# nju-ee/MODE-2022

Measured on AMD Instinct MI355X. Metric: ERP stereo pairs/sec (512x1024, 192 disp) fwd+bwd, higher is better.
Workload: dtype fp32 storage/accumulate; products: 2xfp16 split (22-bit, per-tensor 2^k scale, 3 MFMAs) in the stride-1 3x3x3 / spherical / 3x3 layers incl. gradients (DESIGN 3u/3v); 3xbf16 split (24-bit, 6 MFMAs) in the stride-2 / transposed 3x3x3 layers and the polar spherical tiles (3j-3l); fp32 MFMA in the 32->; 1 GPU; ModeDisparity(192,Sphere,1024x512 Cassini) fwd+bwd+Adam step, batch 2/GPU (BASELINE configs[2]); global_batch=2, conv_arith=bf16x6, init=recipe state, seed 1 (tests/golden/recipe.py), parallelism=dp1

## Files before the change

### include/mode_hip.h

```cpp
#ifndef MODE_HIP_H_
#define MODE_HIP_H_

#include <stddef.h>
#include <stdint.h>

#ifdef __cplusplus
extern "C" {
#endif

typedef void* mode_stream_t;

enum {
  MODE_OK = 0,
  MODE_ERR_BAD_ARG = -1,
  MODE_ERR_UNSUPPORTED = -2,
  MODE_ERR_WORKSPACE = -3
};

typedef struct mode_bn_epilogue {
  const float* gamma;
  const float* beta;
  const float* mean;
  const float* var;
  float eps;
// ... 158 lines not shown

int mode_conv1x1_bwd_weight(const float* gy, const float* x, float* gw, float* workspace, int B, int Ci, int H, int W, int Co,
                            int stride, int accumulate, mode_stream_t stream);

size_t mode_conv_stem_wpack_bytes(int Ci, int Co);

int mode_conv_stem_fwd(const float* x, const float* w, float* y, float* wpack, int B, int Ci, int H, int W, int Co, mode_stream_t stream);

int mode_conv_stem_fwd_bn(const float* x, const float* w, const mode_bn_epilogue* bn, float* y, float* wpack, int B, int Ci, int H,
                          int W, int Co, mode_stream_t stream);

size_t mode_conv_stem_bwd_weight_workspace_bytes(int B, int Ci, int H, int W, int Co);

int mode_conv_stem_bwd_weight(const float* gy, const float* x, float* gw, float* workspace, int B, int Ci, int H, int W, int Co,
                              int accumulate, mode_stream_t stream);
size_t mode_conv2d_bwd_weight_workspace_bytes(int B, int Ci, int H, int W, int Co);
int mode_conv2d_bwd_weight(const float* gy, const float* x, float* gw, float* workspace, int B, int Ci, int H, int W, int Co,
                           int dilation, int accumulate, mode_stream_t stream);

size_t mode_conv3d_wpack_bytes(int Ci, int Co);

int mode_conv3d_fwd(const float* x, const float* w, float* y, float* wpack, int B, int Ci, int D, int H, int W, int Co,
                    int stride, mode_stream_t stream);

int mode_conv3d_bwd_data(const float* gy, const float* w, float* gx, float* wpack, int B, int Ci, int D, int H, int W,
                         int Co, int stride, mode_stream_t stream);

int mode_conv3d_fwd_bn(const float* x, const float* w, const mode_bn_epilogue* bn, float* y, float* wpack, int B, int Ci, int D,
                       int H, int W, int Co, int stride, mode_stream_t stream);

int mode_deconv3d_fwd_bn(const float* x, const float* w, const mode_bn_epilogue* bn, float* y, float* wpack, int B, int Cin, int D,
                         int H, int W, int Cout, mode_stream_t stream);

int mode_conv3d_split_supported(int Ci, int Co, int stride, int which );
int mode_conv3d_split_shape_supported(int Ci, int Co, int D, int H, int W, int stride, int which);
int mode_conv3d_fwd_s2_split(const float* x, const float* w, const mode_bn_epilogue* bn ,
                             float* y, float* wpack, int B, int Ci, int D, int H, int W, int Co, mode_stream_t stream);
int mode_conv3d_fwd_s2_split_amax(const float* x, const float* w, const mode_bn_epilogue* bn, float* y, float* out_absmax, float* wpack, int B,
                                  int Ci, int D, int H, int W, int Co, mode_stream_t stream);

int mode_deconv3d_split_supported(int Cin, int Cout);
int mode_deconv3d_fwd_split(const float* x, const float* w, float* y, float* wpack, int B, int Cin, int D, int H, int W, int Cout,
                            mode_stream_t stream);
int mode_abs_max(const float* x, long long n, float* out_device_buffer, mode_stream_t stream);
int mode_abs_max_batch(const float* const* device_ptrs, const long long* device_sizes, int n, float* out, mode_stream_t stream);
int mode_conv3d_fwd_split_f16(const float* x, const float* w, const float* amax_x, const float* amax_w, float* y, float* wpack, int B, int Ci,
                              int D, int H, int W, int Co, mode_stream_t stream);
int mode_conv3d_bwd_data_split_f16(const float* gy, const float* w, const float* amax_g, const float* amax_w, const float* acc, float* gx,
                                   float* wpack, int B, int Ci, int D, int H, int W, int Co, mode_stream_t stream);
int mode_conv3d_fwd_split_f16_bn(const float* x, const float* w, const float* amax_x, const mode_bn_epilogue* bn, float* y, float* amax_y,
                                 float* wpack, int B, int Ci, int D, int H, int W, int Co, mode_stream_t stream);
int mode_conv3d_bwd_weight_split_f16(const float* gy, const float* x, const float* amax_g, const float* amax_x, float* gw, float* workspace,
                                     int B, int Ci, int D, int H, int W, int Co, int accumulate, mode_stream_t stream);
int mode_conv3d_bwd_data_split_acc_supported(int Ci, int Co, int stride);
int mode_conv3d_bwd_data_split_acc(const float* gy, const float* w, const float* acc, float* gx, float* wpack, int B, int Ci, int D, int H,
                                   int W, int Co, int stride, mode_stream_t stream);
int mode_deconv3d_split_bn_supported(int Cin, int Cout);
int mode_deconv3d_fwd_split_bn(const float* x, const float* w, const mode_bn_epilogue* bn, float* y, float* wpack, int B, int Cin, int D,
                               int H, int W, int Cout, mode_stream_t stream);
int mode_deconv3d_fwd_split_bn_amax(const float* x, const float* w, const mode_bn_epilogue* bn, float* y, float* out_absmax ,
                                    float* wpack, int B, int Cin, int D, int H, int W, int Cout, mode_stream_t stream);
int mode_conv3d_bwd_data_s2_split(const float* gy, const float* w, float* gx, float* wpack, int B, int Ci, int D, int H, int W, int Co,
                                  mode_stream_t stream);
int mode_conv3d_bwd_weight_s2_split(const float* gy, const float* x, float* gw, float* workspace, int B, int Ci, int D, int H, int W,
                                    int Co, int accumulate, mode_stream_t stream);

int mode_conv3d_fwd_split(const float* x, const float* w, const mode_bn_epilogue* bn, float* y, float* wpack, int B, int Ci, int D,
                          int H, int W, int Co, mode_stream_t stream);
int mode_conv3d_bwd_data_split(const float* gy, const float* w, float* gx, float* wpack, int B, int Ci, int D, int H, int W, int Co,
                               mode_stream_t stream);
int mode_conv3d_bwd_weight_split(const float* gy, const float* x, float* gw, float* workspace, int B, int Ci, int D, int H, int W,
                                 int Co, int accumulate, mode_stream_t stream);

int mode_conv2d_split_supported(int Ci, int Co, int dilation, int which );
int mode_conv2d_split_shape_supported(int Ci, int Co, int H, int W, int dilation, int which );
int mode_conv2d_fwd_split(const float* x, const float* w, const mode_bn_epilogue* bn, float* y, float* wpack, int B, int Ci, int H, int W,
                          int Co, int dilation, mode_stream_t stream);
int mode_conv2d_bwd_data_split(const float* gy, const float* w, float* gx, float* wpack, int B, int Ci, int H, int W, int Co, int dilation,
                               mode_stream_t stream);
int mode_conv2d_bwd_data_split_acc(const float* gy, const float* w, const float* acc, float* gx, float* wpack, int B, int Ci, int H, int W,
                                   int Co, int dilation, mode_stream_t stream);
int mode_conv2d_fwd_split_f16(const float* x, const float* w, const float* amax_x, const float* amax_w, float* y, float* wpack, int B, int Ci,
                              int H, int W, int Co, int dilation, mode_stream_t stream);
int mode_conv2d_bwd_data_split_f16(const float* gy, const float* w, const float* amax_g, const float* amax_w, const float* acc, float* gx,
                                   float* wpack, int B, int Ci, int H, int W, int Co, int dilation, mode_stream_t stream);
int mode_conv2d_fwd_split_f16_bn(const float* x, const float* w, const float* amax_x, const mode_bn_epilogue* bn, float* y, float* amax_y,
                                 float* wpack, int B, int Ci, int H, int W, int Co, int dilation, mode_stream_t stream);
int mode_conv2d_bwd_weight_split(const float* gy, const float* x, float* gw, float* workspace, int B, int Ci, int H, int W, int Co,
                                 int dilation, int accumulate, mode_stream_t stream);
int mode_conv2d_bwd_weight_split_f16(const float* gy, const float* x, const float* amax_g, const float* amax_x, float* gw, float* workspace,
                                     int B, int Ci, int H, int W, int Co, int dilation, int accumulate, mode_stream_t stream);

size_t mode_conv3d_bwd_weight_workspace_bytes(int B, int Ci, int D, int H, int W, int Co, int stride);

int mode_conv3d_bwd_weight(const float* gy, const float* x, float* gw, float* workspace, int B, int Ci, int D, int H,
                           int W, int Co, int stride, int accumulate, mode_stream_t stream);

int mode_deconv3d_fwd(const float* x, const float* w, float* y, float* wpack, int B, int Cin, int D, int H, int W,
                      int Cout, mode_stream_t stream);

int mode_head_fwd(const float* logits, float* pred, float* conf, int B, int D4, int H4, int W4, int D, int H, int W,
                  mode_stream_t stream);

size_t mode_head_bwd_workspace_bytes(int B, int D4, int H, int W);

int mode_head_bwd(const float* logits, const float* gpred, float* glogits, float* workspace, int B, int D4, int H4,
// ... 203 lines not shown
```

### mode-2022_amd/csrc/bn_act.hip

```cpp
#include "bn_internal.h"
#include <cstdlib>

namespace {

constexpr int NT = 256;
constexpr int NW = NT / 64;

__device__ __forceinline__ float wave_sum(float v) {
#pragma unroll
  for (int off = 32; off > 0; off >>= 1) v += __shfl_down(v, off, 64);
  return v;
}

__device__ __forceinline__ void block_sum2(float& a, float& b, float* sh ) {
  a = wave_sum(a);
  b = wave_sum(b);
  const int wave = threadIdx.x >> 6, lane = threadIdx.x & 63;
  if (lane == 0) {
    sh[wave] = a;
    sh[NW + wave] = b;
  }
  __syncthreads();
  if (threadIdx.x == 0) {
    a = sh[0];
    b = sh[NW];
#pragma unroll
    for (int w = 1; w < NW; ++w) {
      a += sh[w];
      b += sh[NW + w];
    }
  }
}

__global__ __launch_bounds__(NT) void bn_stats_kernel(const float* __restrict__ y, float* __restrict__ partial, int B, int C,
                                                      long long S, int nsplit, unsigned* __restrict__ zero) {
  __shared__ float sh[2 * NW];
  const int c = blockIdx.y, split = blockIdx.x;
  const int Bg = B / gridDim.z, b0 = blockIdx.z * Bg;
  const long long prow = (long long)blockIdx.z * C + c;
  if (zero && blockIdx.x == 0 && blockIdx.y == 0 && blockIdx.z == 0)
    for (int i = threadIdx.x; i < MODE_BN_ABSMAX_FLOATS; i += NT) zero[i] = 0u;
  const long long S4 = (S & 3) ? 0 : (S >> 2);
  const float K = y[((long long)b0 * C + c) * S];
  float s0 = 0.f, s1 = 0.f;
  for (int b = b0; b < b0 + Bg; ++b) {
    const float4* p = reinterpret_cast<const float4*>(y + ((long long)b * C + c) * S);
    auto acc1 = [&](const float4& v) {
      const float dx = v.x - K, dy = v.y - K, dz = v.z - K, dw = v.w - K;
      s0 += (dx + dy) + (dz + dw);
      s1 += (dx * dx + dy * dy) + (dz * dz + dw * dw);
    };
    const long long st = (long long)nsplit * NT;
    long long i = (long long)split * NT + threadIdx.x;
    for (; i + 3 * st < S4; i += 4 * st) {
      const float4 v0 = p[i], v1 = p[i + st], v2 = p[i + 2 * st], v3 = p[i + 3 * st];
      acc1(v0);
      acc1(v1);
      acc1(v2);
      acc1(v3);
    }
    for (; i < S4; i += st) acc1(p[i]);
    {
      const float* q = y + ((long long)b * C + c) * S;
      for (long long i = (S4 << 2) + (long long)split * NT + threadIdx.x; i < S; i += (long long)nsplit * NT) {
        const float dq = q[i] - K;
        s0 += dq;
        s1 += dq * dq;
      }
    }
  }
  block_sum2(s0, s1, sh);
  if (threadIdx.x == 0) {
    partial[(prow * nsplit + split) * 2] = s0;
    partial[(prow * nsplit + split) * 2 + 1] = s1;
  }
}

__device__ __forceinline__ void reduce_partials(const float* __restrict__ partial, int c, int nsplit, double& s0, double& s1,
                                                double* shd ) {
  double a = 0.0, b = 0.0;
  for (int i = threadIdx.x; i < nsplit; i += NT) {
    const float2 v = reinterpret_cast<const float2*>(partial)[(long long)c * nsplit + i];
    a += (double)v.x;
    b += (double)v.y;
  }
#pragma unroll
  for (int off = 32; off > 0; off >>= 1) {
    a += __shfl_down(a, off, 64);
    b += __shfl_down(b, off, 64);
  }
  const int wave = threadIdx.x >> 6, lane = threadIdx.x & 63;
  if (lane == 0) {
    shd[wave] = a;
    shd[NW + wave] = b;
  }
  __syncthreads();
  s0 = shd[0];
  s1 = shd[NW];
#pragma unroll
  for (int w = 1; w < NW; ++w) {
    s0 += shd[w];
    s1 += shd[NW + w];
  }
  __syncthreads();
}

struct BnCoefArgs {
  const float* partial;
  const float* gamma;
  const float* beta;
  float* running_mean;
  float* running_var;
  long long* num_batches_tracked;
  float* save_mean;
  float* save_invstd;
  float* save_scale;
  float* save_shift;
  float momentum, eps;
  int nsplit;
  double count;
  int groups;
  int Bg;
  const float* pivot;
  unsigned* amax;
};

template <bool RELU, bool ADD, bool TRAIN, bool AMAX = false>
// ... 344 lines not shown
                                      float* save_mean, float* save_invstd, float* save_scale, float* save_shift, float* workspace, int B,
                                      int C, long long S, int groups, float* out_absmax, mode_stream_t stream) {
  return bn_train_fwd_impl(y, add, gamma, beta, running_mean, running_var, num_batches_tracked, momentum, eps, relu, out, save_mean,
                           save_invstd, save_scale, save_shift, workspace, B, C, S, groups, 0, out_absmax, stream);
}

static int check_nsplit(int nsplit) {
  MODE_REQUIRE(nsplit > 0 && nsplit <= 1023, MODE_ERR_BAD_ARG, "mode_bn_train_fwd_prestats: %d partial pairs per channel (1..1023)", nsplit);
  return MODE_OK;
}

extern "C" int mode_bn_train_fwd_prestats(const float* y, const float* add, const float* gamma, const float* beta, float* running_mean,
                                          float* running_var, long long* num_batches_tracked, float momentum, float eps, int relu,
                                          float* out, float* save_mean, float* save_invstd, float* save_scale, float* save_shift,
                                          float* workspace, int nsplit, int B, int C, long long S, mode_stream_t stream) {
  int rc = check_nsplit(nsplit);
  if (rc != MODE_OK) return rc;
  return bn_train_fwd_impl(y, add, gamma, beta, running_mean, running_var, num_batches_tracked, momentum, eps, relu, out, save_mean,
                           save_invstd, save_scale, save_shift, workspace, B, C, S, 1, nsplit, nullptr, stream);
}

extern "C" int mode_bn_train_fwd_prestats_amax(const float* y, const float* add, const float* gamma, const float* beta, float* running_mean,
                                               float* running_var, long long* num_batches_tracked, float momentum, float eps, int relu,
                                               float* out, float* save_mean, float* save_invstd, float* save_scale, float* save_shift,
                                               float* workspace, int nsplit, int B, int C, long long S, float* out_absmax,
                                               mode_stream_t stream) {
  int rc = check_nsplit(nsplit);
  if (rc != MODE_OK) return rc;
  return bn_train_fwd_impl(y, add, gamma, beta, running_mean, running_var, num_batches_tracked, momentum, eps, relu, out, save_mean,
                           save_invstd, save_scale, save_shift, workspace, B, C, S, 1, nsplit, out_absmax, stream);
}

static int bn_train_fwd_impl(const float* y, const float* add, const float* gamma, const float* beta, float* running_mean,
                             float* running_var, long long* num_batches_tracked, float momentum, float eps, int relu, float* out,
                             float* save_mean, float* save_invstd, float* save_scale, float* save_shift, float* workspace, int B,
                             int C, long long S, int groups, int prestats, float* amax, mode_stream_t stream) {
  int rc = check_bn(B, C, S, "mode_bn_train_fwd");
  if (rc != MODE_OK) return rc;
  MODE_REQUIRE(B > 0, MODE_ERR_BAD_ARG, "mode_bn_train_fwd: empty batch has no statistics");
  MODE_REQUIRE(y && gamma && beta && out && save_mean && save_invstd && workspace, MODE_ERR_BAD_ARG, "mode_bn_train_fwd: null pointer");
  MODE_REQUIRE(aligned_rows(y, S) && aligned_rows(out, S) && (!add || aligned_rows(add, S)) && aligned16(workspace), MODE_ERR_UNSUPPORTED,
               "mode_bn_train_fwd: unaligned buffer");
  MODE_REQUIRE((running_mean == nullptr) == (running_var == nullptr), MODE_ERR_BAD_ARG, "mode_bn_train_fwd: running stats must come in pairs");
  MODE_REQUIRE((save_scale == nullptr) == (save_shift == nullptr), MODE_ERR_BAD_ARG, "mode_bn_train_fwd: save_scale / save_shift come in pairs");
  MODE_REQUIRE(groups >= 1 && B % groups == 0, MODE_ERR_BAD_ARG, "mode_bn_train_fwd: batch %d not divisible into %d groups", B, groups);
  MODE_REQUIRE(out != y, MODE_ERR_BAD_ARG, "mode_bn_train_fwd: in-place operation (out == y) is not supported");
  hipStream_t st = mode::as_stream(stream);
  if (amax && prestats > 0) {
    rc = mode::absmax_begin(amax, st, "mode_bn_train_fwd");
    if (rc != MODE_OK) return rc;
  }
  const int nsplit = prestats > 0 ? prestats : pick_nsplit(C * groups, S);
  if (prestats <= 0)
    hipLaunchKernelGGL(bn_stats_kernel, dim3(nsplit, C, groups), dim3(NT), 0, st, y, workspace, B, C, S, nsplit, reinterpret_cast<unsigned*>(amax));
  BnCoefArgs k{workspace, gamma, beta, running_mean, running_var, num_batches_tracked, save_mean, save_invstd, save_scale, save_shift,
               momentum, eps, nsplit,
               (double)(B / groups) * (double)S, groups, B / groups, prestats > 0 ? workspace + 2LL * C * nsplit : nullptr,
               reinterpret_cast<unsigned*>(amax)};
  const int BC = B * C;
  const char* who = "mode_bn_train_fwd";
  if (amax) {
    if (relu)
      rc = add ? launch_apply(bn_apply_kernel<true, true, true, true>, BC, S, st, who, y, add, k, out, C, S)
               : launch_apply(bn_apply_kernel<true, false, true, true>, BC, S, st, who, y, y, k, out, C, S);
    else
      rc = add ? launch_apply(bn_apply_kernel<false, true, true, true>, BC, S, st, who, y, add, k, out, C, S)
               : launch_apply(bn_apply_kernel<false, false, true, true>, BC, S, st, who, y, y, k, out, C, S);
    return rc;
  }
  if (relu) {
    if (add) return launch_apply(bn_apply_kernel<true, true, true>, BC, S, st, who, y, add, k, out, C, S);
    return launch_apply(bn_apply_kernel<true, false, true>, BC, S, st, who, y, y, k, out, C, S);
  }
  if (add) return launch_apply(bn_apply_kernel<false, true, true>, BC, S, st, who, y, add, k, out, C, S);
  return launch_apply(bn_apply_kernel<false, false, true>, BC, S, st, who, y, y, k, out, C, S);
}

namespace {
__global__ __launch_bounds__(NT) void bn_finalize_kernel(const float* __restrict__ y, BnCoefArgs k, int C, long long S) {
  __shared__ double shd[2 * NW];
  const int c = blockIdx.x;
  double s0, s1;
  reduce_partials(k.partial, c, k.nsplit, s0, s1, shd);
  if (threadIdx.x != 0) return;
  const double dm = s0 / k.count;
  const double mean = (double)y[(long long)c * S] + dm;
  double var = s1 / k.count - dm * dm;
  if (var < 0.0) var = 0.0;
  const double invstd = 1.0 / sqrt(var + (double)k.eps);
  const double sc = (double)k.gamma[c] * invstd;
  k.save_mean[c] = (float)mean;
  k.save_invstd[c] = (float)invstd;
  k.save_scale[c] = (float)sc;
  k.save_shift[c] = (float)((double)k.beta[c] - mean * sc);
  if (k.running_mean) {
    const double unbiased = k.count > 1.0 ? var * k.count / (k.count - 1.0) : var;
    k.running_mean[c] = (float)((1.0 - k.momentum) * (double)k.running_mean[c] + k.momentum * mean);
    k.running_var[c] = (float)((1.0 - k.momentum) * (double)k.running_var[c] + k.momentum * unbiased);
  }
  if (c == 0 && k.num_batches_tracked) *k.num_batches_tracked += 1;
}
}

int mode::bn_train_coefficients(const float* y, const float* gamma, const float* beta, float* running_mean, float* running_var,
                                long long* num_batches_tracked, float momentum, float eps, float* save_mean, float* save_invstd,
                                float* save_scale, float* save_shift, float* workspace, int B, int C, long long S, hipStream_t st,
                                const char* who) {
  int rc = ::check_bn(B, C, S, who);
  if (rc != MODE_OK) return rc;
  MODE_REQUIRE(B > 0, MODE_ERR_BAD_ARG, "%s: empty batch has no statistics", who);
  MODE_REQUIRE(y && gamma && beta && save_mean && save_invstd && save_scale && save_shift && workspace, MODE_ERR_BAD_ARG, "%s: null pointer", who);
  MODE_REQUIRE(aligned_rows(y, S) && aligned16(workspace), MODE_ERR_UNSUPPORTED, "%s: unaligned buffer", who);
  MODE_REQUIRE((running_mean == nullptr) == (running_var == nullptr), MODE_ERR_BAD_ARG, "%s: running stats must come in pairs", who);
  const int nsplit = pick_nsplit(C, S);
  hipLaunchKernelGGL(bn_stats_kernel, dim3(nsplit, C, 1), dim3(NT), 0, st, y, workspace, B, C, S, nsplit, (unsigned*)nullptr);
  BnCoefArgs k{workspace, gamma, beta, running_mean, running_var, num_batches_tracked, save_mean, save_invstd, save_scale, save_shift,
               momentum, eps, nsplit, (double)B * (double)S, 1, B, nullptr};
  hipLaunchKernelGGL(bn_finalize_kernel, dim3(C), dim3(NT), 0, st, y, k, C, S);
  return mode::check_launch(who);
}

extern "C" int mode_bn_eval_fwd(const float* y, const float* add, const float* gamma, const float* beta, const float* running_mean,
                                const float* running_var, float eps, int relu, float* out, int B, int C, long long S,
                                mode_stream_t stream) {
  int rc = check_bn(B, C, S, "mode_bn_eval_fwd");
  if (rc != MODE_OK) return rc;
  if (B == 0) return MODE_OK;
  MODE_REQUIRE(y && gamma && beta && running_mean && running_var && out, MODE_ERR_BAD_ARG, "mode_bn_eval_fwd: null pointer");
  MODE_REQUIRE(aligned_rows(y, S) && aligned_rows(out, S) && (!add || aligned_rows(add, S)), MODE_ERR_UNSUPPORTED, "mode_bn_eval_fwd: unaligned buffer");
  hipStream_t st = mode::as_stream(stream);
  BnCoefArgs k{nullptr, gamma, beta, const_cast<float*>(running_mean), const_cast<float*>(running_var), nullptr, nullptr, nullptr, nullptr,
               nullptr, 0.f,
               eps, 0, 0.0, 1, 1, nullptr};
  const int BC = B * C;
  const char* who = "mode_bn_eval_fwd";
  if (relu) {
    if (add) return launch_apply(bn_apply_kernel<true, true, false>, BC, S, st, who, y, add, k, out, C, S);
    return launch_apply(bn_apply_kernel<true, false, false>, BC, S, st, who, y, y, k, out, C, S);
  }
  if (add) return launch_apply(bn_apply_kernel<false, true, false>, BC, S, st, who, y, add, k, out, C, S);
  return launch_apply(bn_apply_kernel<false, false, false>, BC, S, st, who, y, y, k, out, C, S);
}

extern "C" int mode_bn_train_bwd(const float* gout, const float* y, const float* out, const float* gamma, const float* save_mean,
                                 const float* save_invstd, const float* save_scale, const float* save_shift, int relu, float* gy,
                                 float* gadd, float* ggamma, float* gbeta, int accumulate, float* workspace, int B, int C, long long S,
                                 int groups, mode_stream_t stream) {
  return mode_bn_train_bwd_amax(gout, y, out, gamma, save_mean, save_invstd, save_scale, save_shift, relu, gy, gadd, ggamma, gbeta,
                                accumulate, workspace, B, C, S, groups, nullptr, stream);
}

extern "C" int mode_bn_train_bwd_amax(const float* gout, const float* y, const float* out, const float* gamma, const float* save_mean,
                                      const float* save_invstd, const float* save_scale, const float* save_shift, int relu, float* gy,
                                      float* gadd, float* ggamma, float* gbeta, int accumulate, float* workspace, int B, int C,
                                      long long S, int groups, float* gy_absmax, mode_stream_t stream) {
  float* amax = gy_absmax;
  int rc = check_bn(B, C, S, "mode_bn_train_bwd");
  if (rc != MODE_OK) return rc;
  MODE_REQUIRE(B > 0, MODE_ERR_BAD_ARG, "mode_bn_train_bwd: empty batch");
  MODE_REQUIRE(gout && y && gamma && save_mean && save_invstd && gy && ggamma && gbeta && workspace, MODE_ERR_BAD_ARG,
               "mode_bn_train_bwd: null pointer");
  MODE_REQUIRE((save_scale == nullptr) == (save_shift == nullptr), MODE_ERR_BAD_ARG, "mode_bn_train_bwd: save_scale / save_shift come in pairs");
  MODE_REQUIRE(!relu || out || save_scale, MODE_ERR_BAD_ARG,
               "mode_bn_train_bwd: the ReLU mask needs the forward output, or (no residual add) the forward's scale / shift");
  MODE_REQUIRE(aligned_rows(gout, S) && aligned_rows(y, S) && aligned_rows(gy, S) && (!out || aligned_rows(out, S)) &&
                   (!gadd || aligned_rows(gadd, S)) && aligned16(workspace),
               MODE_ERR_UNSUPPORTED, "mode_bn_train_bwd: unaligned buffer");
  MODE_REQUIRE(groups >= 1 && B % groups == 0, MODE_ERR_BAD_ARG, "mode_bn_train_bwd: batch %d not divisible into %d groups", B, groups);
  if (gadd) {
    const long long n = (long long)B * C * S;
    auto overlaps = [&](const float* p) { return p && p < gadd + n && gadd < p + n; };
// ... 79 lines not shown
```

### mode-2022_amd/csrc/conv3d.hip

```cpp
#include "common.h"
#include <cstdlib>

#include "conv3d_internal.h"
#include "bn_internal.h"

namespace {

typedef float f32x16 __attribute__((ext_vector_type(16)));

constexpr int NT = 256;
constexpr int CCH = 8;

struct CDims {
  int B, Ci, Co, D, H, W;
  int Do, Ho, Wo;
  int nWt, nHt, nDt;
  int MT, NCHUNK;
  int ntiles;
};

__device__ __forceinline__ f32x16 mfma32(float a, float b, f32x16 c) {
  return __builtin_amdgcn_mfma_f32_32x32x2f32(a, b, c, 0, 0, 0);
}

// ... 554 lines not shown
extern "C" int mode_conv3d_fwd_split_stats_partials(void) { return mode::conv3d_split_stat_partials(); }

extern "C" int mode_conv3d_fwd_split_stats(const float* x, const float* w, float* y, float* wpack, float* stats, int B, int Ci, int D, int H,
                                           int W, int Co, mode_stream_t stream) {
  const char* who = "mode_conv3d_fwd_split_stats";
  int rc = check_split_args(x, w, y, wpack, B, Ci, D, H, W, Co, 1, 0, who);
  if (rc != MODE_OK) return rc;
  MODE_REQUIRE(stats, MODE_ERR_WORKSPACE, "%s: statistics workspace required", who);
  MODE_REQUIRE(B > 0, MODE_ERR_BAD_ARG, "%s: empty batch has no statistics", who);
  return mode::conv3d_s1_split(x, w, y, wpack, B, Ci, Co, D, H, W, 0, mode::as_stream(stream), who, nullptr, stats);
}

extern "C" int mode_conv3d_fwd_s2_split_amax(const float* x, const float* w, const mode_bn_epilogue* bn, float* y, float* out_absmax, float* wpack,
                                             int B, int Ci, int D, int H, int W, int Co, mode_stream_t stream) {
  const char* who = "mode_conv3d_fwd_s2_split";
  int rc = check_split_args(x, w, y, wpack, B, Ci, D, H, W, Co, 2, 0, who);
  if (rc == MODE_OK && bn) rc = mode::check_bn(bn, who);
  if (rc != MODE_OK) return rc;
  MODE_REQUIRE(!out_absmax || bn, MODE_ERR_BAD_ARG, "%s: the output maximum comes out of the eval epilogue (bn is NULL)", who);
  if (B == 0) return out_absmax ? mode::absmax_begin(out_absmax, mode::as_stream(stream), who) : MODE_OK;
  return mode::conv3d_s2_split(x, w, y, wpack, B, Ci, Co, D, H, W, mode::as_stream(stream), who, bn, out_absmax);
}

extern "C" int mode_conv3d_fwd_s2_split(const float* x, const float* w, const mode_bn_epilogue* bn, float* y, float* wpack, int B, int Ci,
                                        int D, int H, int W, int Co, mode_stream_t stream) {
  return mode_conv3d_fwd_s2_split_amax(x, w, bn, y, nullptr, wpack, B, Ci, D, H, W, Co, stream);
}

extern "C" int mode_conv3d_bwd_data_s2_split(const float* gy, const float* w, float* gx, float* wpack, int B, int Ci, int D, int H, int W,
                                             int Co, mode_stream_t stream) {
  const char* who = "mode_conv3d_bwd_data_s2_split";
  int rc = check_split_args(gy, w, gx, wpack, B, Ci, D, H, W, Co, 2, 1, who);
  if (rc != MODE_OK || B == 0) return rc;
  return mode::deconv3d_split(gy, w, gx, wpack, B, Co, Ci, D / 2, H / 2, W / 2, mode::as_stream(stream), who);
}

extern "C" int mode_abs_max(const float* x, long long n, float* out, mode_stream_t stream) {
  return mode::abs_max(x, n, out, mode::as_stream(stream), "mode_abs_max");
}

extern "C" int mode_abs_max_batch(const float* const* device_ptrs, const long long* device_sizes, int n, float* out, mode_stream_t stream) {
  return mode::abs_max_batch(device_ptrs, device_sizes, n, out, mode::as_stream(stream), "mode_abs_max_batch");
}

extern "C" int mode_conv3d_fwd_split_f16(const float* x, const float* w, const float* amax_x, const float* amax_w, float* y, float* wpack, int B,
                                         int Ci, int D, int H, int W, int Co, mode_stream_t stream) {
  const char* who = "mode_conv3d_fwd_split_f16";
  int rc = check_split_args(x, w, y, wpack, B, Ci, D, H, W, Co, 1, 0, who);
  if (rc != MODE_OK || B == 0) return rc;
  MODE_REQUIRE(amax_x && amax_w, MODE_ERR_BAD_ARG, "%s: null operand maximum", who);
  return mode::conv3d_s1_split(x, w, y, wpack, B, Ci, Co, D, H, W, 0, mode::as_stream(stream), who, nullptr, nullptr, nullptr, amax_x, amax_w);
}

extern "C" int mode_conv3d_fwd_split_f16_bn(const float* x, const float* w, const float* amax_x, const mode_bn_epilogue* bn, float* y,
                                            float* amax_y, float* wpack, int B, int Ci, int D, int H, int W, int Co, mode_stream_t stream) {
  const char* who = "mode_conv3d_fwd_split_f16_bn";
  int rc = check_split_args(x, w, y, wpack, B, Ci, D, H, W, Co, 1, 0, who);
  if (rc == MODE_OK) {
    MODE_REQUIRE(bn, MODE_ERR_BAD_ARG, "%s: null BatchNorm epilogue", who);
    rc = mode::check_bn(bn, who);
  }
  if (rc != MODE_OK) return rc;
  MODE_REQUIRE(amax_x && amax_y, MODE_ERR_BAD_ARG, "%s: null maximum buffer", who);
  if (B == 0) return mode::absmax_begin(amax_y, mode::as_stream(stream), who);
  return mode::conv3d_s1_split(x, w, y, wpack, B, Ci, Co, D, H, W, 0, mode::as_stream(stream), who, bn, nullptr, nullptr, amax_x, nullptr, amax_y);
}

extern "C" int mode_conv3d_bwd_data_split_f16(const float* gy, const float* w, const float* amax_g, const float* amax_w, const float* acc, float* gx,
                                              float* wpack, int B, int Ci, int D, int H, int W, int Co, mode_stream_t stream) {
  const char* who = "mode_conv3d_bwd_data_split_f16";
  int rc = check_split_args(gy, w, gx, wpack, B, Ci, D, H, W, Co, 1, 1, who);
  if (rc != MODE_OK || B == 0) return rc;
  MODE_REQUIRE(amax_g && amax_w && acc != gx, MODE_ERR_BAD_ARG, "%s: null operand maximum, or acc is the output tensor", who);
  return mode::conv3d_s1_split(gy, w, gx, wpack, B, Co, Ci, D, H, W, 1, mode::as_stream(stream), who, nullptr, nullptr, acc, amax_g, amax_w);
}

extern "C" int mode_conv3d_bwd_data_split_acc_supported(int Ci, int Co, int stride) {
  if (Ci <= 0 || Co <= 0) return 0;
  if (stride == 1) return mode::conv3d_split_supported(Co, Ci) ? 1 : 0;
  return (stride == 2 && mode::deconv3d_split_bn_supported(Co, Ci)) ? 1 : 0;
}

extern "C" int mode_conv3d_bwd_data_split_acc(const float* gy, const float* w, const float* acc, float* gx, float* wpack, int B, int Ci, int D,
                                              int H, int W, int Co, int stride, mode_stream_t stream) {
  const char* who = "mode_conv3d_bwd_data_split_acc";
  MODE_REQUIRE(stride == 1 || stride == 2, MODE_ERR_UNSUPPORTED, "%s: stride %d not implemented", who, stride);
  int rc = check_split_args(gy, w, gx, wpack, B, Ci, D, H, W, Co, stride, 1, who);
  if (rc != MODE_OK || B == 0) return rc;
  MODE_REQUIRE(acc && acc != gx, MODE_ERR_BAD_ARG, "%s: acc must be a tensor of gx's shape that is not gx", who);
  if (stride == 1) return mode::conv3d_s1_split(gy, w, gx, wpack, B, Co, Ci, D, H, W, 1, mode::as_stream(stream), who, nullptr, nullptr, acc);
  return mode::deconv3d_split(gy, w, gx, wpack, B, Co, Ci, D / 2, H / 2, W / 2, mode::as_stream(stream), who, nullptr, acc);
}

extern "C" int mode_deconv3d_split_supported(int Cin, int Cout) { return mode::deconv3d_split_supported(Cin, Cout) ? 1 : 0; }

extern "C" int mode_deconv3d_fwd_split(const float* x, const float* w, float* y, float* wpack, int B, int Cin, int D, int H, int W, int Cout,
                                       mode_stream_t stream) {
  const char* who = "mode_deconv3d_fwd_split";
  int rc = check_deconv_split_args(x, w, y, wpack, B, Cin, D, H, W, Cout, who);
  if (rc != MODE_OK || B == 0) return rc;
  return mode::deconv3d_split(x, w, y, wpack, B, Cin, Cout, D, H, W, mode::as_stream(stream), who);
}

extern "C" int mode_deconv3d_split_bn_supported(int Cin, int Cout) { return mode::deconv3d_split_bn_supported(Cin, Cout) ? 1 : 0; }

extern "C" int mode_deconv3d_fwd_split_bn_amax(const float* x, const float* w, const mode_bn_epilogue* bn, float* y, float* out_absmax,
// ... 586 lines not shown
  if (B == 0) {
    if (!accumulate) return mode::zero_floats(gw, (size_t)Co * Ci * 27, st, "mode_conv3d_bwd_weight");
    return MODE_OK;
  }
  if (Co == 1 && stride == 1)
    return mode::conv3d_co1_bwd_weight(gy, x, gw, workspace, B, Ci, D, H, W, accumulate, st, "mode_conv3d_bwd_weight");
  WDims d;
  make_wdims(d, B, Ci, D, H, W, Co, stride);
  if (stride == 1) {
    const size_t lds = WGeom<1, WTH1>::LDS;
    if ((long long)std::max(Ci, Co) * D * H * W < (1ll << 29)) {
      rc = mode::allow_lds(conv3d_bwd_weight_ring_kernel, lds, "mode_conv3d_bwd_weight");
      if (rc != MODE_OK) return rc;
      int ring_dc = D;
      while (ring_dc > 6 && (long long)B * d.nHt * d.nWt * mode::cdiv(D, ring_dc) < 2ll * d.S) ring_dc = mode::cdiv(ring_dc, 2);
      static const char* dc_env = getenv("MODE_RING_DC");
      if (dc_env && atoi(dc_env) > 0) ring_dc = atoi(dc_env);
      const int nDc = mode::cdiv(D, ring_dc);
      const int units = B * d.nHt * d.nWt * nDc;
      if (d.S > units) d.S = units;
      hipLaunchKernelGGL(conv3d_bwd_weight_ring_kernel, dim3(d.S, d.MTo, d.MTc), dim3(NT), lds, st, gy, x, workspace, d, nDc, units,
                         ring_dc);
    } else {
      rc = mode::allow_lds(conv3d_bwd_weight_kernel<1, WTH1>, lds, "mode_conv3d_bwd_weight");
      if (rc != MODE_OK) return rc;
      hipLaunchKernelGGL((conv3d_bwd_weight_kernel<1, WTH1>), dim3(d.S, d.MTo, d.MTc), dim3(NT), lds, st, gy, x, workspace, d);
    }
  } else {
    const size_t lds = WGeom<2, WTH2>::LDS;
    if (std::max((long long)Ci * D * H * W, (long long)Co * d.Do * d.Ho * d.Wo) < (1ll << 29)) {
      if (d.MTo >= 2) {
        const size_t lds2 = lds + (size_t)32 * WGeom<2, WTH2>::GPLANE * sizeof(float);
        rc = mode::allow_lds(conv3d_bwd_weight_s2_kernel<2>, lds2, "mode_conv3d_bwd_weight");
        if (rc != MODE_OK) return rc;
        hipLaunchKernelGGL(conv3d_bwd_weight_s2_kernel<2>, dim3(d.S, mode::cdiv(d.MTo, 2), d.MTc), dim3(2 * NT), lds2, st, gy, x, workspace, d);
      } else {
        rc = mode::allow_lds(conv3d_bwd_weight_s2_kernel<1>, lds, "mode_conv3d_bwd_weight");
        if (rc != MODE_OK) return rc;
        hipLaunchKernelGGL(conv3d_bwd_weight_s2_kernel<1>, dim3(d.S, d.MTo, d.MTc), dim3(NT), lds, st, gy, x, workspace, d);
      }
    } else {
      rc = mode::allow_lds(conv3d_bwd_weight_kernel<2, WTH2>, lds, "mode_conv3d_bwd_weight");
      if (rc != MODE_OK) return rc;
      hipLaunchKernelGGL((conv3d_bwd_weight_kernel<2, WTH2>), dim3(d.S, d.MTo, d.MTc), dim3(NT), lds, st, gy, x, workspace, d);
    }
  }
  rc = mode::check_launch("mode_conv3d_bwd_weight");
  if (rc != MODE_OK) return rc;
  hipLaunchKernelGGL(reduce_gw3d, dim3(mode::cdiv((long long)d.MTo * d.MTc * 27 * 1024, 32)), dim3(256), 0, st, workspace, gw, d, accumulate);
  return mode::check_launch("mode_conv3d_bwd_weight(reduce)");
}

static int bwd_weight_split(const float* gy, const float* x, const float* amax_g, const float* amax_x, float* gw, float* workspace, int B, int Ci,
                            int D, int H, int W, int Co, int accumulate, mode_stream_t stream, const char* who);

extern "C" int mode_conv3d_bwd_weight_split(const float* gy, const float* x, float* gw, float* workspace, int B, int Ci, int D, int H,
                                            int W, int Co, int accumulate, mode_stream_t stream) {
  return bwd_weight_split(gy, x, nullptr, nullptr, gw, workspace, B, Ci, D, H, W, Co, accumulate, stream, "mode_conv3d_bwd_weight_split");
}

extern "C" int mode_conv3d_bwd_weight_split_f16(const float* gy, const float* x, const float* amax_g, const float* amax_x, float* gw, float* workspace,
                                                int B, int Ci, int D, int H, int W, int Co, int accumulate, mode_stream_t stream) {
  MODE_REQUIRE(amax_g && amax_x, MODE_ERR_BAD_ARG, "mode_conv3d_bwd_weight_split_f16: null operand maximum");
  return bwd_weight_split(gy, x, amax_g, amax_x, gw, workspace, B, Ci, D, H, W, Co, accumulate, stream, "mode_conv3d_bwd_weight_split_f16");
}

static int bwd_weight_split(const float* gy, const float* x, const float* amax_g, const float* amax_x, float* gw, float* workspace, int B, int Ci,
                            int D, int H, int W, int Co, int accumulate, mode_stream_t stream, const char* who) {
  int rc = check_split_args(gy, x, gw, workspace, B, Ci, D, H, W, Co, 1, 2, who);
  if (rc != MODE_OK) return rc;
  hipStream_t st = mode::as_stream(stream);
  if (B == 0) {
    if (!accumulate) return mode::zero_floats(gw, (size_t)Co * Ci * 27, st, "mode_conv3d_bwd_weight");
    return MODE_OK;
  }
  WDims d;
  make_wdims(d, B, Ci, D, H, W, Co, 1);
  mode::WgradSplitDims q;
  q.Ci = Ci; q.Co = Co; q.D = D; q.H = H; q.W = W;
  q.nWt = d.nWt; q.nHt = d.nHt; q.MTo = d.MTo; q.MTc = d.MTc;
  int S = mode::cdiv(kNumCU, d.MTo * d.MTc);
  int ring_dc = D;
  while (ring_dc > 6 && (long long)B * d.nHt * d.nWt * mode::cdiv(D, ring_dc) < 2ll * S) ring_dc = mode::cdiv(ring_dc, 2);
  q.ring_dc = ring_dc;
  q.nDc = mode::cdiv(D, ring_dc);
  q.units = B * d.nHt * d.nWt * q.nDc;
  if (S > q.units) S = q.units;
  q.S = d.S = S;
  rc = mode::conv3d_bww_split_launch(gy, x, workspace, q, st, who, amax_g, amax_x);
  if (rc != MODE_OK) return rc;
  hipLaunchKernelGGL(reduce_gw3d, dim3(mode::cdiv((long long)d.MTo * d.MTc * 27 * 1024, 32)), dim3(256), 0, st, workspace, gw, d, accumulate);
  return mode::check_launch("mode_conv3d_bwd_weight_split(reduce)");
}

extern "C" int mode_conv3d_bwd_weight_s2_split(const float* gy, const float* x, float* gw, float* workspace, int B, int Ci, int D, int H,
                                               int W, int Co, int accumulate, mode_stream_t stream) {
  const char* who = "mode_conv3d_bwd_weight_s2_split";
  int rc = check_split_args(gy, x, gw, workspace, B, Ci, D, H, W, Co, 2, 2, who);
  if (rc != MODE_OK) return rc;
  hipStream_t st = mode::as_stream(stream);
  if (B == 0) {
    if (!accumulate) return mode::zero_floats(gw, (size_t)Co * Ci * 27, st, "mode_conv3d_bwd_weight");
    return MODE_OK;
  }
  WDims d;
  make_wdims(d, B, Ci, D, H, W, Co, 2);
  mode::WgradS2SplitDims q;
  q.Ci = Ci; q.Co = Co; q.D = D; q.H = H; q.W = W; q.Do = d.Do; q.Ho = d.Ho; q.Wo = d.Wo;
  q.nWt = mode::cdiv(d.Wo, 16); q.MTo = d.MTo; q.MTc = d.MTc;
  int S = std::max(1, kNumCU / (mode::cdiv(d.MTo, 2) * d.MTc));
  int ring_dc = d.Do;
  while (ring_dc > 3 && (long long)B * d.Ho * q.nWt * mode::cdiv(d.Do, ring_dc) < 2ll * S) ring_dc = mode::cdiv(ring_dc, 2);
  q.ring_dc = ring_dc;
  q.nDc = mode::cdiv(d.Do, ring_dc);
  q.units = B * d.Ho * q.nWt * q.nDc;
  q.S = std::min(std::min(S, q.units), d.S);
  d.S = q.S;
  rc = mode::conv3d_bww_s2_split_launch(gy, x, workspace, q, st, who);
  if (rc != MODE_OK) return rc;
  hipLaunchKernelGGL(reduce_gw3d, dim3(mode::cdiv((long long)d.MTo * d.MTc * 27 * 1024, 32)), dim3(256), 0, st, workspace, gw, d, accumulate);
  return mode::check_launch("mode_conv3d_bwd_weight_s2_split(reduce)");
}

extern "C" int mode_deconv3d_fwd(const float* x, const float* w, float* y, float* wpack, int B, int Cin, int D, int H, int W,
                                 int Cout, mode_stream_t stream) {
  int rc = check_conv_args(x, w, y, wpack, B, Cin, D, H, W, Cout, 1, "mode_deconv3d_fwd");
  if (rc != MODE_OK || B == 0) return rc;
  MODE_REQUIRE((long long)Cout * D * H * W * 8 < (1ll << 31), MODE_ERR_UNSUPPORTED, "mode_deconv3d_fwd: output sample too large");
  return deconv3d(x, w, y, wpack, B, Cin, Cout, D, H, W, mode::as_stream(stream), "mode_deconv3d_fwd");
}

extern "C" int mode_deconv3d_fwd_bn(const float* x, const float* w, const mode_bn_epilogue* bn, float* y, float* wpack, int B, int Cin,
                                    int D, int H, int W, int Cout, mode_stream_t stream) {
  const char* who = "mode_deconv3d_fwd_bn";
  int rc = check_conv_args(x, w, y, wpack, B, Cin, D, H, W, Cout, 1, who);
  if (rc == MODE_OK) rc = mode::check_bn(bn, who);
  if (rc != MODE_OK || B == 0) return rc;
  MODE_REQUIRE((long long)Cout * D * H * W * 8 < (1ll << 31), MODE_ERR_UNSUPPORTED, "%s: output sample too large", who);
  return deconv3d(x, w, y, wpack, B, Cin, Cout, D, H, W, mode::as_stream(stream), who, bn);
}
```

### mode-2022_amd/csrc/conv3d_internal.h

```cpp
#pragma once
#include "common.h"
#include "size_contracts.h"

namespace mode {

int conv3d_co1_fwd(const float* x, const float* w, float* y, int B, int Ci, int D, int H, int W, hipStream_t st, const char* who);

int conv3d_co1_fwd_small(const float* x, const float* w, float* y, int B, int Ci, int D, int H, int W, hipStream_t st, const char* who);

int conv3d_co1_bwd_data(const float* gy, const float* w, float* gx, int B, int Ci, int D, int H, int W, hipStream_t st, const char* who);

size_t conv3d_co1_bwd_weight_workspace_floats(int B, int Ci, int D, int H, int W);
int conv3d_co1_bwd_weight(const float* gy, const float* x, float* gw, float* workspace, int B, int Ci, int D, int H, int W,
                          int accumulate, hipStream_t st, const char* who);

bool conv3d_split_supported(int K, int rows);
size_t conv3d_split_wpack_floats(int K, int rows);
int conv3d_split_stat_partials();
int conv3d_s1_split(const float* x, const float* w, float* y, float* wpack, int B, int K, int rows, int D, int H, int W, int flip,
                    hipStream_t st, const char* who, const mode_bn_epilogue* bn, float* stats = nullptr, const float* acc_in = nullptr,
                    const float* amax_x = nullptr, const float* amax_w = nullptr, float* amax_y = nullptr);

int abs_max(const float* x, long long n, float* out, hipStream_t st, const char* who);
int abs_max_batch(const float* const* ptrs, const long long* sizes, int n, float* out, hipStream_t st, const char* who);

bool conv3d_s2_split_supported(int K, int rows);
size_t conv3d_s2_split_wpack_floats(int K, int rows);
int conv3d_s2_split(const float* x, const float* w, float* y, float* wpack, int B, int K, int rows, int D, int H, int W, hipStream_t st,
                    const char* who, const mode_bn_epilogue* bn = nullptr, float* amax_y = nullptr);

bool deconv3d_split_supported(int K, int Co);
bool deconv3d_split_bn_supported(int K, int Co);
size_t deconv3d_split_wpack_floats(int K, int Co);
int deconv3d_split(const float* x, const float* w, float* y, float* wpack, int B, int K, int Co, int D, int H, int W, hipStream_t st,
                   const char* who, const mode_bn_epilogue* bn = nullptr, const float* acc_in = nullptr, float* amax_y = nullptr);

struct WgradSplitDims {
  int Ci, Co, D, H, W;
  int nWt, nHt, nDc, ring_dc, units;
  int S, MTo, MTc;
};
int conv3d_bww_split_launch(const float* gy, const float* x, float* part, const WgradSplitDims& d, hipStream_t st, const char* who,
                            const float* amax_g = nullptr, const float* amax_x = nullptr);

struct WgradS2SplitDims {
  int Ci, Co, D, H, W, Do, Ho, Wo;
  int nWt, nDc, ring_dc, units;
  int S, MTo, MTc;
};
int conv3d_bww_s2_split_launch(const float* gy, const float* x, float* part, const WgradS2SplitDims& d, hipStream_t st, const char* who);

bool conv2d_split_supported(int K, int rows, int dilation);
size_t conv2d_split_wpack_floats(int K, int rows);
int conv2d_split_run(const float* x, const float* w, float* y, float* wpack, int B, int K, int rows, int H, int W, int dilation, int flip,
                     hipStream_t st, const char* who, const mode_bn_epilogue* bn, const float* acc_in = nullptr,
                     const float* amax_x = nullptr, const float* amax_w = nullptr, float* amax_y = nullptr);

struct Wgrad2SplitDims {
  int Ci, Co, H, W;
  int nWt, nGroups, run_groups, nRun, units;
  int S, MTo, MTc;
};
int conv2d_bww_split_launch(const float* gy, const float* x, float* part, const Wgrad2SplitDims& d, int dilation, hipStream_t st,
                            const char* who, const float* amax_g = nullptr, const float* amax_x = nullptr);

}
```

### mode-2022_amd/csrc/conv3d_split.hip

```cpp
#include "common.h"

#include "bn_internal.h"
#include "conv3d_internal.h"
#include "split_arith.h"

namespace {

using namespace mode::split;

#ifndef MODE_SPLIT_NT
#define MODE_SPLIT_NT 256
#endif
constexpr int NT = MODE_SPLIT_NT;
constexpr int TD = 2, ID = TD + 2, IW = 34;
template <int TH_>
struct Geo {
  static constexpr int TH = TH_, IH = TH_ + 2;
  static constexpr int ROWS = ID * IH;
  static constexpr int ITEMS = ROWS * IW;
  static constexpr int KIT = (ITEMS + NT - 1) / NT;
  static constexpr int PIECE = KIT * NT;
  static constexpr int R = TD * TH_ / (NT / 64);
  static constexpr int RB = R / 4;
};
// ... 30 lines not shown
  if (fold && blockIdx.x == 0) {
    float* shifts = reinterpret_cast<float*>(wp + total * NP);
    for (int o = threadIdx.x; o < rows; o += blockDim.x) shifts[o] = fold == 1 ? fold_shift(bn, o) : 0.f;
  }
  for (long long idx = (long long)blockIdx.x * blockDim.x + threadIdx.x; idx < total; idx += (long long)gridDim.x * blockDim.x) {
    const int lane = (int)(idx & 63);
    long long r = idx >> 6;
    const int pair = (int)(r % NPAIR);
    r /= NPAIR;
    const int ch = (int)(r % NCHUNK);
    const int m = (int)(r / NCHUNK);
    const int o = m * 32 + (lane & 31);
    const int tap = 2 * pair + (lane >> 5);
    float v[8];
#pragma unroll
    for (int j = 0; j < 8; ++j) {
      const int c = ch * 8 + j;
      v[j] = 0.f;
      if (o < rows && c < K && tap < 27)
        v[j] = flip == 0 ? w[((long long)o * K + c) * 27 + tap] : w[((long long)c * rows + o) * 27 + (26 - tap)];
      if (fold == 1 && o < rows) v[j] *= fold_scale(bn, o);
      if (F16) v[j] *= sw;
    }
    uint32_t q1[4], q2[4], q3[4];
#pragma unroll
    for (int j = 0; j < 4; ++j) split2<F16>(v[2 * j], v[2 * j + 1], q1[j], q2[j], q3[j]);
    uint4* dst = wp + (idx - lane) * NP + lane;
    dst[0] = make_uint4(q1[0], q1[1], q1[2], q1[3]);
    dst[64] = make_uint4(q2[0], q2[1], q2[2], q2[3]);
    if (NP == 3) dst[128] = make_uint4(q3[0], q3[1], q3[2], q3[3]);
  }
}

__host__ __device__ constexpr int tap_off(int tap, int IH) {
  return (tap / 9) * (IH * IW) + ((tap / 3) % 3) * IW + tap % 3;
}

__global__ __launch_bounds__(64) void first_voxel_kernel(const float* __restrict__ x, const float* __restrict__ w, float* __restrict__ pivot,
                                                         int K, int Co, int D, int H, int W) {
  const int o = blockIdx.x, lane = threadIdx.x;
  const long long HW = (long long)H * W, DHW = (long long)D * HW;
  float acc = 0.f;
  for (int item = lane; item < K * 8; item += 64) {
    const int c = item >> 3, t = item & 7;
    const int kd = 1 + (t >> 2), kh = 1 + ((t >> 1) & 1), kw = 1 + (t & 1);
    if (kd - 1 < D && kh - 1 < H && kw - 1 < W)
      acc = __builtin_fmaf(w[((long long)o * K + c) * 27 + kd * 9 + kh * 3 + kw], x[c * DHW + (kd - 1) * HW + (kh - 1) * W + (kw - 1)], acc);
  }
#pragma unroll
  for (int off = 32; off > 0; off >>= 1) acc += __shfl_xor(acc, off, 64);
  if (lane == 0) pivot[o] = acc;
}

template <int MT, int EPI, bool F16 = false, int TH_ = 8, bool AMAX = false>
__global__ __launch_bounds__(NT) void conv3d_split_kernel(const float* __restrict__ x, const uint4* __restrict__ wp,
                                                          float* __restrict__ y, SDims d, Epi epi, float* __restrict__ stats,
                                                          const float* __restrict__ stat_pivot, const float* __restrict__ amax_x,
                                                          const float* __restrict__ amax_w, unsigned* __restrict__ amax_y) {
  constexpr int NP = Arith<F16>::NP, NTERM = Arith<F16>::NTERM, BUF = buf_of<F16, TH_>();
  using Ge = Geo<TH_>;
  constexpr int TH = Ge::TH, IH = Ge::IH, ITEMS = Ge::ITEMS, KIT = Ge::KIT, PIECE = Ge::PIECE, R = Ge::R, RB = Ge::RB;
  static_assert(EPI == 0 || EPI == 1 || TH_ == 8, "the tall tile exists for the plain store and the shift epilogue (a residual's values do not fit)");
  const float sx = F16 ? f16_scale_of(mode::absmax_load(amax_x)) : 1.f;
  const float unscale = F16 ? (1.f / sx) * (1.f / f16_scale_of(mode::absmax_load(amax_w))) : 1.f;
  extern __shared__ __attribute__((aligned(16))) uint4 sm[];
  const int tid = threadIdx.x, wave = tid >> 6, lane = tid & 63;
  d.o0 += 32 * MT * (int)blockIdx.y;
  wp += (long long)blockIdx.y * MT * d.NCHUNK * NPAIR * (64 * NP);

  const int nwx = gridDim.x / kNumXCD;
  const int xcd = blockIdx.x % kNumXCD, slot = blockIdx.x / kNumXCD;
  const int q = d.ntiles / kNumXCD, rr = d.ntiles % kNumXCD;
  const int t_begin = xcd < rr ? xcd * (q + 1) : rr * (q + 1) + (xcd - rr) * q;
  const int t_count = xcd < rr ? q + 1 : q;
  const int mine = slot < t_count ? (t_count - slot + nwx - 1) / nwx : 0;
  const int G = mine * d.NCHUNK;

  const long long HW = (long long)d.H * d.W;
  const long long DHW = (long long)d.D * HW;

  auto tile_of = [&](int k, int& b, int& d0, int& h0, int& w0) {
    int t = t_begin + slot + k * nwx;
    w0 = (t % d.nWt) * 32;
    t /= d.nWt;
    h0 = (t % d.nHt) * TH;
    t /= d.nHt;
    d0 = (t % d.nDt) * TD;
    b = t / d.nDt;
  };

  int pdz[KIT], phy[KIT], pwi[KIT], poff[KIT];
#pragma unroll
  for (int k = 0; k < KIT; ++k) {
    const int item = min(tid + k * NT, ITEMS - 1);
    const int row = item / IW;
    pwi[k] = item - row * IW;
    pdz[k] = row / IH;
    phy[k] = row - pdz[k] * IH;
    poff[k] = pdz[k] * (int)HW + phy[k] * d.W + pwi[k];
  }
  float raw[KIT][8];
  int jw, jh, jd, jb, sw, sh, sd, sb, s_ch = 0;
  {
    int t = nwx;
    jw = t % d.nWt;
    t /= d.nWt;
    jh = t % d.nHt;
    t /= d.nHt;
    jd = t % d.nDt;
    jb = t / d.nDt;
    t = t_begin + slot;
    sw = t % d.nWt;
    t /= d.nWt;
    sh = t % d.nHt;
    t /= d.nHt;
    sd = t % d.nDt;
    sb = t / d.nDt;
  }
  unsigned soff[8];
#pragma unroll
  for (int c = 0; c < 8; ++c) soff[c] = (unsigned)c * (unsigned)DHW * 4u;
  __amdgpu_buffer_rsrc_t st_rs = buf_rsrc(x, 0);
  int st_base = 0, st_d0 = 0, st_h0 = 0, st_w0 = 0;
  auto stage_advance = [&](int step) {
    s_ch += step;
    const int wrap = s_ch >= d.NCHUNK ? 1 : 0;
    s_ch = wrap ? 0 : s_ch;
    sw += wrap ? jw : 0;
    int c = sw >= d.nWt ? 1 : 0;
    sw -= c ? d.nWt : 0;
    sh += (wrap ? jh : 0) + c;
    c = sh >= d.nHt ? 1 : 0;
    sh -= c ? d.nHt : 0;
    sd += (wrap ? jd : 0) + c;
    c = sd >= d.nDt ? 1 : 0;
    sd -= c ? d.nDt : 0;
    sb += (wrap ? jb : 0) + c;
  };
  auto stage_begin = [&]() {
    st_d0 = sd * TD;
    st_h0 = sh * TH;
    st_w0 = sw * 32;
    st_rs = buf_rsrc(x + ((long long)sb * d.K + s_ch * 8) * DHW, (unsigned)DHW * 32u);
    st_base = (st_d0 - 1) * (int)HW + (st_h0 - 1) * d.W + (st_w0 - 1);
  };
  auto stage_load = [&](int k) {
    const unsigned ok = (unsigned)((unsigned)(st_d0 + pdz[k] - 1) < (unsigned)d.D) & (unsigned)((unsigned)(st_h0 + phy[k] - 1) < (unsigned)d.H) &
                        (unsigned)((unsigned)(st_w0 + pwi[k] - 1) < (unsigned)d.W);
    const unsigned off = ok ? (unsigned)(st_base + poff[k]) * 4u : kBufOOB;
#pragma unroll
    for (int c = 0; c < 8; ++c) raw[k][c] = buf_load_f32(st_rs, off, soff[c]);
  };
  uint32_t sq[3][4];
  auto stage_commit = [&](int buf, int k, int h) {
#pragma unroll
    for (int j = 2 * h; j < 2 * h + 2; ++j) {
      float v0 = raw[k][2 * j], v1 = raw[k][2 * j + 1];
      if (F16) {
        v0 *= sx;
        v1 *= sx;
      }
      split2<F16>(v0, v1, sq[0][j], sq[1][j], sq[2][j]);
    }
    if (h == 1) {
      uint4* dst = sm + buf * BUF + tid + k * NT;
#pragma unroll
      for (int p = 0; p < NP; ++p) dst[p * PIECE] = make_uint4(sq[p][0], sq[p][1], sq[p][2], sq[p][3]);
    }
  };

  f32x16 acc[MT][R];
#pragma unroll
  for (int m = 0; m < MT; ++m)
#pragma unroll
    for (int r = 0; r < R; ++r) acc[m][r] = (f32x16){0};
  int rowpos[R];
#pragma unroll
  for (int r = 0; r < R; ++r) {
    const int row = wave * R + r;
    rowpos[r] = (row / TH) * (IH * IW) + (row % TH) * IW + (lane & 31);
  }
  const int half = lane >> 5;
  float shiftv[MT][16], addv[MT][R][16];
  float st0[MT][16], st1[MT][16], stK[MT][16];
  if (EPI == 3) {
#pragma unroll
    for (int m = 0; m < MT; ++m)
#pragma unroll
      for (int qq = 0; qq < 16; ++qq) {
        st0[m][qq] = st1[m][qq] = 0.f;
        stK[m][qq] = stat_pivot ? stat_pivot[min(d.o0 + m * 32 + (qq & 3) + 8 * (qq >> 2) + 4 * half, d.Co - 1)] : 0.f;
      }
  }
  unsigned out_mag = 0;
  const float relu_floor = (EPI == 1 || EPI == 2) && epi.relu ? 0.f : -__builtin_inff();
  if (EPI == 1 || EPI == 2) {
#pragma unroll
    for (int m = 0; m < MT; ++m)
#pragma unroll
      for (int qq = 0; qq < 16; ++qq) shiftv[m][qq] = epi.shift[min(d.o0 + m * 32 + (qq & 3) + 8 * (qq >> 2) + 4 * half, d.Co - 1)];
  }
  unsigned ep_off[R], ep_chan[MT][16];
  int ep_b = 0;
  auto ep_tile = [&](int k) {
    int b, d0, h0, w0;
    tile_of(k, b, d0, h0, w0);
    ep_b = __builtin_amdgcn_readfirstlane(b);
#pragma unroll
    for (int r = 0; r < R; ++r) {
      const int row = wave * R + r;
      const int gd = d0 + row / TH, gh = h0 + row % TH, gw = w0 + (lane & 31);
// ... 52 lines not shown
#pragma unroll
    for (int r = 0; r < 4; ++r)
#pragma unroll
      for (int p = 0; p < NP; ++p) bq[0][r][p] = src[p * PIECE + rowpos[r] + (half ? tap_off(1, IH) : tap_off(0, IH))];
#pragma unroll
    for (int idx = 0; idx < NPAIR * RB; ++idx) {
      const int pair = idx / RB, rb = idx % RB;
      if (idx + 1 < NPAIR * RB) {
        const int npair = (idx + 1) / RB, nrb = (idx + 1) % RB;
        const int t0 = 2 * npair, t1 = t0 + 1 < 27 ? t0 + 1 : 26;
        const int toff = half ? tap_off(t1, IH) : tap_off(t0, IH);
#pragma unroll
        for (int r = 0; r < 4; ++r)
#pragma unroll
          for (int p = 0; p < NP; ++p) bq[(idx + 1) & 1][r][p] = src[p * PIECE + rowpos[4 * nrb + r] + toff];
      }
      if (rb == 0) {
        if (pair + WAHEAD < NPAIR)
          load_a((pair + WAHEAD) % 7, ch, pair + WAHEAD);
        else
          load_a((pair + WAHEAD) % 7, ch_next, pair + WAHEAD - NPAIR);
        if (pair < KIT) stage_load(pair);
      }
      if (EPI == 2 && pair >= NPAIR - 2 * R) {
        const int r = (pair - (NPAIR - 2 * R)) / 2;
#pragma unroll
        for (int m = 0; m < MT; ++m)
#pragma unroll
          for (int qq = 8 * (pair & 1); qq < 8 * (pair & 1) + 8; ++qq) addv[m][r][qq] = ep_base[ep_cur[r] + ep_chan[m][qq]];
      }
      if (pair >= NPAIR - KIT) {
        if (RB == 1 || rb == 0) stage_commit((g + 1) & 1, pair - (NPAIR - KIT), 0);
        if (RB == 1 || rb == 1) stage_commit((g + 1) & 1, pair - (NPAIR - KIT), 1);
      }
#define MODE_SPLIT_TERM(PA, PB)                                                      \
  _Pragma("unroll") for (int m = 0; m < MT; ++m) _Pragma("unroll") for (int r = 0; r < 4; ++r) \
      acc[m][4 * rb + r] = mfma_split<F16>(aring[pair % 7][m][PA], bq[idx & 1][r][PB], acc[m][4 * rb + r]);
      if constexpr (F16) {
        MODE_SPLIT_TERM(1, 0)
        MODE_SPLIT_TERM(0, 1)
        MODE_SPLIT_TERM(0, 0)
      } else {
        MODE_SPLIT_TERM(2, 0)
        MODE_SPLIT_TERM(0, 2)
        MODE_SPLIT_TERM(1, 1)
        MODE_SPLIT_TERM(1, 0)
        MODE_SPLIT_TERM(0, 1)
        MODE_SPLIT_TERM(0, 0)
      }
#undef MODE_SPLIT_TERM
#pragma unroll
      for (int i = 0; i < MT * 4 * NTERM; ++i) {
        __builtin_amdgcn_sched_group_barrier(0x008, 1, 0);
        __builtin_amdgcn_sched_group_barrier(0x002, 3, 0);
        if (F16) {
          __builtin_amdgcn_sched_group_barrier(0x080, 1, 0);
          __builtin_amdgcn_sched_group_barrier(0x020, 1, 0);
        } else {
          __builtin_amdgcn_sched_group_barrier(0x100, 1, 0);
        }
      }
      __builtin_amdgcn_sched_barrier(0);
    }
    if (ch == d.NCHUNK - 1) {
      int b, d0, h0, w0;
      tile_of(k_tile, b, d0, h0, w0);
      float* yb = y + (long long)b * d.Co * DHW;
      const int gw = w0 + (lane & 31);
#pragma unroll
      for (int r = 0; r < R; ++r) {
        const int row = wave * R + r;
        const int gd = d0 + row / TH, gh = h0 + row % TH;
        if (gd < d.D && gh < d.H && gw < d.W) {
          const long long sp = gd * HW + (long long)gh * d.W + gw;
#pragma unroll
          for (int m = 0; m < MT; ++m)
#pragma unroll
            for (int qq = 0; qq < 16; ++qq) {
              const int o = d.o0 + m * 32 + (qq & 3) + 8 * (qq >> 2) + 4 * half;
              if (o < d.Co) {
                const long long idx = o * DHW + sp;
                float v = acc[m][r][qq];
                if (F16) v *= unscale;
                if (EPI == 1 || EPI == 2) v += shiftv[m][qq];
                if (EPI == 2) v += addv[m][r][qq];
                if (EPI == 3) {
                  const float dv = v - stK[m][qq];
                  st0[m][qq] += dv;
                  st1[m][qq] = __builtin_fmaf(dv, dv, st1[m][qq]);
                }
                const float vo = ((EPI == 1 || EPI == 2) && v < relu_floor) ? relu_floor : v;
                if (AMAX) out_mag = max(out_mag, mode::absmax_mag(vo));
                yb[idx] = vo;
              }
            }
        }
#pragma unroll
        for (int m = 0; m < MT; ++m) acc[m][r] = (f32x16){0};
      }
      ++k_tile;
      if (EPI == 2) ep_tile(min(k_tile, max(mine - 1, 0)));
    }
    ch = ch_next;
    lds_barrier();
  }
  if (AMAX) {
    __syncthreads();
    mode::absmax_block_commit(out_mag, amax_y, reinterpret_cast<unsigned*>(sm));
  }
  if (EPI == 3) {
    float* red = reinterpret_cast<float*>(sm);
    __syncthreads();
#pragma unroll
    for (int m = 0; m < MT; ++m)
#pragma unroll
      for (int qq = 0; qq < 16; ++qq) {
        float a = st0[m][qq], b = st1[m][qq];
#pragma unroll
        for (int off = 16; off > 0; off >>= 1) {
          a += __shfl_xor(a, off, 64);
          b += __shfl_xor(b, off, 64);
        }
        if ((lane & 31) == 0) {
          const int c = m * 32 + (qq & 3) + 8 * (qq >> 2) + 4 * half;
          red[(wave * MT * 32 + c) * 2] = a;
          red[(wave * MT * 32 + c) * 2 + 1] = b;
        }
      }
    __syncthreads();
    if (tid < MT * 32) {
      const int o = d.o0 + tid;
      if (o < d.Co) {
        float a = 0.f, b = 0.f;
#pragma unroll
        for (int wv = 0; wv < NT / 64; ++wv) {
          a += red[(wv * MT * 32 + tid) * 2];
          b += red[(wv * MT * 32 + tid) * 2 + 1];
        }
        stats[((long long)o * gridDim.x + blockIdx.x) * 2] = a;
        stats[((long long)o * gridDim.x + blockIdx.x) * 2 + 1] = b;
      }
    }
  }
}

template <int MT>
int launch_split(const float* x, const float* wpack, float* y, SDims d, int nblocks, hipStream_t st, const char* who, Epi epi,
                 float* stats = nullptr, const float* stat_pivot = nullptr, const float* amax_x = nullptr, const float* amax_w = nullptr,
                 float* amax_y = nullptr) {
  const uint4* wp = reinterpret_cast<const uint4*>(wpack);
  const int grid = kNumCU;
#define MODE_SPLIT_LAUNCH_TH(EPIV, F16V, THV, AMAXV, STATS, PIVOT)                                                           \
  {                                                                                                                          \
    int rc = mode::allow_lds(conv3d_split_kernel<MT, EPIV, F16V, THV, AMAXV>, lds_bytes<F16V, THV>(), who);                  \
    if (rc != MODE_OK) return rc;                                                                                            \
    hipLaunchKernelGGL((conv3d_split_kernel<MT, EPIV, F16V, THV, AMAXV>), dim3(grid, nblocks), dim3(NT), (lds_bytes<F16V, THV>()), st, x, wp, \
                       y, d, epi, STATS, PIVOT, amax_x, amax_w, reinterpret_cast<unsigned*>(amax_y));                        \
    return mode::check_launch(who);                                                                                          \
  }
#define MODE_SPLIT_LAUNCH(EPIV, F16V, STATS, PIVOT) MODE_SPLIT_LAUNCH_TH(EPIV, F16V, 8, false, STATS, PIVOT)
  if (amax_x && amax_y) {
    MODE_REQUIRE(!stats && epi.shift, MODE_ERR_BAD_ARG, "%s: the output maximum belongs to the eval epilogues", who);
    if (epi.add) MODE_SPLIT_LAUNCH_TH(2, true, 8, true, nullptr, nullptr)
    if (d.TH == 16) MODE_SPLIT_LAUNCH_TH(1, true, 16, true, nullptr, nullptr)
    MODE_SPLIT_LAUNCH_TH(1, true, 8, true, nullptr, nullptr)
  }
  if (amax_x) {
    MODE_REQUIRE(!stats && (!epi.shift || epi.add), MODE_ERR_UNSUPPORTED, "%s: the fp16 arithmetic has no BatchNorm epilogues", who);
    if (epi.shift && epi.add) MODE_SPLIT_LAUNCH(2, true, nullptr, nullptr)
    if (d.TH == 16) MODE_SPLIT_LAUNCH_TH(0, true, 16, false, nullptr, nullptr)
    MODE_SPLIT_LAUNCH(0, true, nullptr, nullptr)
  }
  if (stats) MODE_SPLIT_LAUNCH(3, false, stats, stat_pivot)
  if (epi.shift && epi.add) MODE_SPLIT_LAUNCH(2, false, nullptr, nullptr)
  if (epi.shift) MODE_SPLIT_LAUNCH(1, false, nullptr, nullptr)
  MODE_SPLIT_LAUNCH(0, false, nullptr, nullptr)
#undef MODE_SPLIT_LAUNCH
#undef MODE_SPLIT_LAUNCH_TH
}

__device__ __forceinline__ unsigned finite_mag(unsigned bits) {
  const unsigned v = bits & 0x7fffffffu;
  return v < 0x7f800000u ? v : 0u;
}
__global__ __launch_bounds__(256) void abs_max_kernel(const float* __restrict__ x, long long n, unsigned* __restrict__ out) {
  unsigned m = 0;
  const long long n4 = n >> 2, stride = (long long)gridDim.x * blockDim.x;
  const uint4* x4 = reinterpret_cast<const uint4*>(x);
  long long i = (long long)blockIdx.x * blockDim.x + threadIdx.x;
  for (; i + 3 * stride < n4; i += 4 * stride) {
    const uint4 v0 = x4[i], v1 = x4[i + stride], v2 = x4[i + 2 * stride], v3 = x4[i + 3 * stride];
    m = max(max(m, finite_mag(v0.x)), max(max(finite_mag(v0.y), finite_mag(v0.z)), finite_mag(v0.w)));
    m = max(max(m, finite_mag(v1.x)), max(max(finite_mag(v1.y), finite_mag(v1.z)), finite_mag(v1.w)));
    m = max(max(m, finite_mag(v2.x)), max(max(finite_mag(v2.y), finite_mag(v2.z)), finite_mag(v2.w)));
    m = max(max(m, finite_mag(v3.x)), max(max(finite_mag(v3.y), finite_mag(v3.z)), finite_mag(v3.w)));
  }
  for (; i < n4; i += stride) {
    const uint4 v = x4[i];
    m = max(max(m, finite_mag(v.x)), max(max(finite_mag(v.y), finite_mag(v.z)), finite_mag(v.w)));
  }
  for (long long i = (n4 << 2) + (long long)blockIdx.x * blockDim.x + threadIdx.x; i < n; i += stride)
    m = max(m, finite_mag(__builtin_bit_cast(unsigned, x[i])));
#pragma unroll
  for (int off = 32; off > 0; off >>= 1) m = max(m, (unsigned)__shfl_xor((int)m, off, 64));
  __shared__ unsigned sh[4];
  mode::absmax_block_commit(m, out, sh);
}

__global__ __launch_bounds__(1024) void abs_max_batch_kernel(const float* const* __restrict__ ptrs, const long long* __restrict__ sizes,
                                                             unsigned* __restrict__ out) {
  const int j = blockIdx.x;
  const float* x = ptrs[j];
  const long long n = sizes[j];
  unsigned m = 0;
  long long i = threadIdx.x;
  for (; i + 3072 < n; i += 4096) {
    const float a = x[i], b = x[i + 1024], c = x[i + 2048], e = x[i + 3072];
    m = max(max(m, finite_mag(__builtin_bit_cast(unsigned, a))), finite_mag(__builtin_bit_cast(unsigned, b)));
    m = max(max(m, finite_mag(__builtin_bit_cast(unsigned, c))), finite_mag(__builtin_bit_cast(unsigned, e)));
  }
  for (; i < n; i += 1024) m = max(m, finite_mag(__builtin_bit_cast(unsigned, x[i])));
#pragma unroll
  for (int off = 32; off > 0; off >>= 1) m = max(m, (unsigned)__shfl_xor((int)m, off, 64));
  __shared__ unsigned sh[16];
  if ((threadIdx.x & 63) == 0) sh[threadIdx.x >> 6] = m;
  unsigned* o = out + (long long)j * MODE_BN_ABSMAX_FLOATS;
  for (int k = threadIdx.x + 1; k < MODE_BN_ABSMAX_FLOATS; k += 1024) o[k] = 0u;
  __syncthreads();
  if (threadIdx.x == 0) {
    unsigned r = 0;
#pragma unroll
// ... 2 lines not shown
  }
}

__global__ __launch_bounds__(1024) void abs_max_folded_kernel(const float* __restrict__ w, mode_bn_epilogue bn, int rows, int n,
                                                              unsigned* __restrict__ out) {
  unsigned m = 0;
  for (int i = threadIdx.x; i < rows * n; i += 1024) m = max(m, finite_mag(__builtin_bit_cast(unsigned, w[i] * fold_scale(bn, i / n))));
#pragma unroll
  for (int off = 32; off > 0; off >>= 1) m = max(m, (unsigned)__shfl_xor((int)m, off, 64));
  __shared__ unsigned sh[16];
  if ((threadIdx.x & 63) == 0) sh[threadIdx.x >> 6] = m;
  for (int k = threadIdx.x + 1; k < MODE_BN_ABSMAX_FLOATS; k += 1024) out[k] = 0u;
  __syncthreads();
  if (threadIdx.x == 0) {
    unsigned r = 0;
#pragma unroll
    for (int k = 0; k < 16; ++k) r = max(r, sh[k]);
    out[0] = r;
  }
}

}

namespace mode {

int abs_max_batch(const float* const* ptrs, const long long* sizes, int n, float* out, hipStream_t st, const char* who) {
  MODE_REQUIRE(n >= 0, MODE_ERR_BAD_ARG, "%s: negative count", who);
  if (n == 0) return MODE_OK;
  MODE_REQUIRE(ptrs && sizes && out, MODE_ERR_BAD_ARG, "%s: null pointer", who);
  hipLaunchKernelGGL(abs_max_batch_kernel, dim3(n), dim3(1024), 0, st, ptrs, sizes, reinterpret_cast<unsigned*>(out));
  return mode::check_launch(who);
}

int abs_max(const float* x, long long n, float* out, hipStream_t st, const char* who) {
  MODE_REQUIRE(n >= 0 && out && (n == 0 || x), MODE_ERR_BAD_ARG, "%s: bad argument", who);
  MODE_REQUIRE((reinterpret_cast<size_t>(x) & 15) == 0, MODE_ERR_BAD_ARG, "%s: the tensor must be 16-byte aligned", who);
  int rc = mode::fill_words(out, 0u, MODE_BN_ABSMAX_FLOATS, st, who);
  if (rc != MODE_OK || n == 0) return rc;
  const int blocks = (int)std::min<long long>(cdiv(n, 256 * 16), 16 * kNumCU);
  hipLaunchKernelGGL(abs_max_kernel, dim3(std::max(blocks, 1)), dim3(256), 0, st, x, n, reinterpret_cast<unsigned*>(out));
  return mode::check_launch(who);
}

size_t conv3d_split_wpack_floats(int K, int rows) {
  return (size_t)cdiv(rows, 32) * cdiv(K, 8) * NPAIR * 3 * 64 * 4 + 32 * (size_t)cdiv(rows, 32);
}

bool conv3d_split_supported(int K, int rows) { return rows > 1 && rows <= 64 && K % 8 == 0; }

int conv3d_split_stat_partials() { return kNumCU; }

int conv3d_s1_split(const float* x, const float* w, float* y, float* wpack, int B, int K, int rows, int D, int H, int W, int flip,
                    hipStream_t st, const char* who, const mode_bn_epilogue* bn, float* stats, const float* acc_in, const float* amax_x,
                    const float* amax_w, float* amax_y) {
  const float* absmax = amax_x;
  const bool eval16 = absmax && bn;
  MODE_REQUIRE(eval16 ? (!amax_w && amax_y && !stats && !acc_in) : ((amax_x == nullptr) == (amax_w == nullptr) && !amax_y), MODE_ERR_BAD_ARG,
               "%s: both operand maxima, or neither (eval epilogue: the input's and the output's)", who);
  MODE_REQUIRE(!(acc_in && (bn || stats)), MODE_ERR_BAD_ARG, "%s: the accumulate form takes no BatchNorm epilogue and no statistics", who);
  MODE_REQUIRE(!(absmax && stats), MODE_ERR_UNSUPPORTED, "%s: the fp16 arithmetic has no statistics epilogue", who);
  SDims d;
  d.B = B; d.K = K; d.Co = rows; d.D = D; d.H = H; d.W = W;
  d.MT = cdiv(rows, 32);
  d.NCHUNK = cdiv(K, 8);
  MODE_REQUIRE(conv3d_split_supported(K, rows), MODE_ERR_UNSUPPORTED, "%s: %d output / %d reduction channels not supported by the split kernel", who,
               rows, K);
  MODE_REQUIRE(conv3d_s1_split_fits(rows, (long long)D * H * W), MODE_ERR_UNSUPPORTED,
               "%s: volume beyond the 32-bit offsets of the split kernel (8 planes of 2^31 bytes or more, or an output sample of 2^31 elements)", who);
  static const char* tall_env = getenv("MODE_SPLIT_TALL");
  const bool tall_ok = !tall_env || tall_env[0] != '0';
  d.TH = 8;
  if (absmax && !acc_in && !(bn && bn->add) && H % 16 == 0 && (long long)B * cdiv(D, TD) * (H / 8) * cdiv(W, 32) >= 4ll * kNumCU && tall_ok)
    d.TH = 16;
  d.nWt = cdiv(W, 32);
  d.nHt = cdiv(H, d.TH);
  d.nDt = cdiv(D, TD);
  d.ntiles = B * d.nDt * d.nHt * d.nWt;
  const long long npack = (long long)d.MT * d.NCHUNK * NPAIR * 64;
  const int NP = absmax ? 2 : 3;
  if (eval16) {
    float* wmax = wpack + npack * NP * 4 + 32 * d.MT;
    static_assert(NPAIR * 64 * 4 >= MODE_BN_ABSMAX_FLOATS + 64, "the folded weights' maximum does not fit behind the shifts");
    if (mode::pack_needed()) {
      hipLaunchKernelGGL(abs_max_folded_kernel, dim3(1), dim3(1024), 0, st, w, *bn, rows, K * 27, reinterpret_cast<unsigned*>(wmax));
      hipLaunchKernelGGL(pack_w3d_split<true>, dim3(cdiv(npack, 256)), dim3(256), 0, st, w, reinterpret_cast<uint4*>(wpack), rows, K, d.MT, d.NCHUNK,
                         flip, 1, *bn, wmax);
    }
    int rc = mode::absmax_begin(amax_y, st, who);
    if (rc != MODE_OK) return rc;
    d.o0 = 0;
    return launch_split<1>(x, wpack, y, d, d.MT, st, who, make_epi(bn, wpack + npack * NP * 4), nullptr, nullptr, amax_x, wmax, amax_y);
  }
  if (mode::pack_needed()) {
    if (absmax)
      hipLaunchKernelGGL(pack_w3d_split<true>, dim3(cdiv(npack, 256)), dim3(256), 0, st, w, reinterpret_cast<uint4*>(wpack), rows, K, d.MT, d.NCHUNK,
                         flip, acc_in ? 2 : 0, mode_bn_epilogue(), amax_w);
    else
      hipLaunchKernelGGL(pack_w3d_split<false>, dim3(cdiv(npack, 256)), dim3(256), 0, st, w, reinterpret_cast<uint4*>(wpack), rows, K, d.MT, d.NCHUNK,
                         flip, bn ? 1 : acc_in ? 2 : 0, bn ? *bn : mode_bn_epilogue(), nullptr);
  }
  Epi epi = make_epi(bn, wpack + npack * NP * 4);
  if (acc_in) {
    epi.shift = wpack + npack * NP * 4;
    epi.add = acc_in;
    epi.relu = 0;
  }
  d.o0 = 0;
  if (stats && !bn) {
    float* pivot = stats + 2LL * rows * conv3d_split_stat_partials();
    hipLaunchKernelGGL(first_voxel_kernel, dim3(rows), dim3(64), 0, st, x, w, pivot, K, rows, D, H, W);
    return launch_split<1>(x, wpack, y, d, d.MT, st, who, epi, stats, pivot);
  }
  return launch_split<1>(x, wpack, y, d, d.MT, st, who, epi, nullptr, nullptr, amax_x, amax_w);
}

}
```

### mode-2022_amd/csrc/conv3d_split_wgrad.hip

```cpp
#include "common.h"

#include "bn_internal.h"
#include "conv3d_internal.h"
#include "split_arith.h"

namespace {

using namespace mode::split;

constexpr int NT = 256;
constexpr int WTH = 2, XR = WTH + 2;
constexpr int XROWP = 40;
constexpr int XPLANE = XR * XROWP;
constexpr int XPIECE = 4 * XPLANE;
constexpr int XCS = 3 * XPIECE + 8;
constexpr int GPIECE = WTH * 32;
constexpr int GCS = 3 * GPIECE + 8;
constexpr int GBUF = 32 * GCS;
constexpr int XALL = 32 * XCS;
constexpr size_t LDS_BYTES = (size_t)(XALL + 2 * GBUF) * 2;
constexpr int XIT = (32 * XR * 17 + NT - 1) / NT;
constexpr int GIT = 32 * WTH * 16 / NT;

template <bool F16>
__device__ __forceinline__ void split2(float a, float b, uint32_t& p1, uint32_t& p2, uint32_t& p3) {
  if constexpr (F16) {
    split2_f16_subfma(a, b, p1, p2);
    p3 = 0;
  } else {
    split3_bf16_subfma(a, b, p1, p2, p3);
  }
}

template <bool F16>
__global__ __launch_bounds__(NT) void conv3d_bww_split_kernel(const float* __restrict__ gy, const float* __restrict__ x,
                                                              float* __restrict__ part, mode::WgradSplitDims d,
                                                              const float* __restrict__ amax_g, const float* __restrict__ amax_x) {
  constexpr int NP = Arith<F16>::NP;
  const float sg = F16 ? f16_scale_of(mode::absmax_load(amax_g)) : 1.f, sx = F16 ? f16_scale_of(mode::absmax_load(amax_x)) : 1.f;
  const float unscale = F16 ? (1.f / sg) * (1.f / sx) : 1.f;
  extern __shared__ __attribute__((aligned(16))) uint16_t lds[];
  uint16_t* xl = lds;
  uint16_t* gl = lds + XALL;
  const int s = blockIdx.x, ob = blockIdx.y, cb = blockIdx.z;
  const int tid = threadIdx.x, wave = tid >> 6, lane = tid & 63, half = lane >> 5;
  const int HWi = d.H * d.W, DHWi = d.D * HWi;

  int tkd[7], tkh[7];
#pragma unroll
  for (int t = 0; t < 6; ++t) {
    const int g = wave + 4 * (t / 3);
    tkd[t] = g / 3;
    tkh[t] = g % 3;
  }
  tkd[6] = 2;
  tkh[6] = 2;
  const int kw6 = min(wave, 2);
  const uint32_t sel6 = kw6 == 0 ? 0x03020100u : kw6 == 1 ? 0x05040302u : 0x07060504u;

  f32x16 acc[7], acs[7];
#pragma unroll
  for (int t = 0; t < 7; ++t) {
    acc[t] = (f32x16){0};
    acs[t] = (f32x16){0};
  }

  int x_c[XIT], x_row[XIT], x_wp[XIT], g_o[GIT], g_row[GIT], g_wp[GIT];
#pragma unroll
  for (int k = 0; k < XIT; ++k) {
    const int item = min(tid + k * NT, 32 * XR * 17 - 1);
    x_wp[k] = item % 17;
    x_row[k] = (item / 17) % XR;
    x_c[k] = item / (17 * XR);
  }
#pragma unroll
  for (int k = 0; k < GIT; ++k) {
    const int item = tid + k * NT;
    g_wp[k] = item % 16;
    g_row[k] = (item / 16) % WTH;
    g_o[k] = item / (16 * WTH);
  }

  float xr[XIT][2], gr[GIT][2];
  unsigned xo0[XIT], xo1[XIT], go0[GIT], go1[GIT];
  int xdst[XIT], gdst[GIT];
#pragma unroll
  for (int k = 0; k < XIT; ++k) xdst[k] = x_c[k] * XCS + x_row[k] * XROWP + 2 * x_wp[k];
#pragma unroll
  for (int k = 0; k < GIT; ++k) gdst[k] = g_o[k] * GCS + g_row[k] * 32 + 2 * g_wp[k];
  auto unit_begin = [&](int h0, int w0) {
#pragma unroll
    for (int k = 0; k < XIT; ++k) {
      const int gh = h0 - 1 + x_row[k], gw = w0 - 1 + 2 * x_wp[k];
      const unsigned rowok = (unsigned)((unsigned)gh < (unsigned)d.H) & (unsigned)(cb * 32 + x_c[k] < d.Ci);
      const unsigned base = 4u * (unsigned)(x_c[k] * DHWi + gh * d.W + gw);
      xo0[k] = (rowok & (unsigned)((unsigned)gw < (unsigned)d.W)) ? base : kBufOOB;
      xo1[k] = (rowok & (unsigned)((unsigned)(gw + 1) < (unsigned)d.W)) ? base + 4u : kBufOOB;
    }
#pragma unroll
    for (int k = 0; k < GIT; ++k) {
      const int gh = h0 + g_row[k], gw = w0 + 2 * g_wp[k];
      const unsigned rowok = (unsigned)(gh < d.H) & (unsigned)(ob * 32 + g_o[k] < d.Co);
      const unsigned base = 4u * (unsigned)(g_o[k] * DHWi + gh * d.W + gw);
      go0[k] = (rowok & (unsigned)(gw < d.W)) ? base : kBufOOB;
      go1[k] = (rowok & (unsigned)(gw + 1 < d.W)) ? base + 4u : kBufOOB;
    }
  };
  const unsigned block_bytes = 128u * (unsigned)DHWi;
  const float* xb = x;
  const float* gb = gy;
  auto load_x = [&](int k, int z) {
    const __amdgpu_buffer_rsrc_t rs = buf_rsrc(xb, (unsigned)z < (unsigned)d.D ? block_bytes : 0u);
    const unsigned zo = 4u * (unsigned)(min(max(z, 0), d.D - 1) * HWi);
    xr[k][0] = buf_load_f32(rs, xo0[k], zo);
    xr[k][1] = buf_load_f32(rs, xo1[k], zo);
  };
  auto commit_x = [&](int k, int z) {
    uint32_t p1, p2, p3;
    float v0 = xr[k][0], v1 = xr[k][1];
    if (F16) {
      v0 *= sx;
      v1 *= sx;
    }
    split2<F16>(v0, v1, p1, p2, p3);
    uint32_t* dst = reinterpret_cast<uint32_t*>(xl + xdst[k] + ((z + 4) & 3) * XPLANE);
    dst[0] = p1;
    dst[XPIECE / 2] = p2;
    if (!F16) dst[XPIECE] = p3;
  };
  auto load_g = [&](int k, int z) {
    const __amdgpu_buffer_rsrc_t rs = buf_rsrc(gb, z < d.D ? block_bytes : 0u);
    const unsigned zo = 4u * (unsigned)(min(z, d.D - 1) * HWi);
    gr[k][0] = buf_load_f32(rs, go0[k], zo);
    gr[k][1] = buf_load_f32(rs, go1[k], zo);
  };
  auto commit_g = [&](int k, int z) {
    uint32_t p1, p2, p3;
    float v0 = gr[k][0], v1 = gr[k][1];
    if (F16) {
      v0 *= sg;
      v1 *= sg;
    }
    split2<F16>(v0, v1, p1, p2, p3);
    uint32_t* dst = reinterpret_cast<uint32_t*>(gl + gdst[k] + (z & 1) * GBUF);
    dst[0] = p1;
    dst[GPIECE / 2] = p2;
    if (!F16) dst[GPIECE] = p3;
  };

  for (int u = xcd_remap(s, d.S); u < d.units; u += d.S) {
    int t = u;
    const int dc = t % d.nDc;
    t /= d.nDc;
    const int wt = t % d.nWt;
    t /= d.nWt;
    const int ht = t % d.nHt;
    const int b = t / d.nHt;
    unit_begin(ht * WTH, wt * 32);
    const int dlo = dc * d.ring_dc, dhi = min(d.D, dlo + d.ring_dc);
    xb = x + ((long long)b * d.Ci + cb * 32) * DHWi;
    gb = gy + ((long long)b * d.Co + ob * 32) * DHWi;

#pragma unroll 1
    for (int z = dlo - 1; z <= dlo + 1; ++z) {
#pragma unroll
      for (int k = 0; k < XIT; ++k) load_x(k, z);
#pragma unroll
      for (int k = 0; k < XIT; ++k) commit_x(k, z);
    }
#pragma unroll
    for (int k = 0; k < GIT; ++k) load_g(k, dlo);
#pragma unroll
    for (int k = 0; k < GIT; ++k) commit_g(k, dlo);
// ... 81 lines not shown
          }
        } else {
          MODE_SPLIT_TERM(acs, 2, 0)
          MODE_SPLIT_TERM(acs, 0, 2)
          MODE_SPLIT_TERM(acs, 1, 1)
          MODE_SPLIT_TERM(acs, 1, 0)
          MODE_SPLIT_TERM(acs, 0, 1)
          MODE_SPLIT_TERM(acc, 0, 0)
        }
#undef MODE_SPLIT_TERM
#pragma unroll
        for (int i = 0; i < (F16 ? 21 : 42); ++i) {
          __builtin_amdgcn_sched_group_barrier(0x008, 1, 0);
          if (F16) {
            if (ks < 2) {
              __builtin_amdgcn_sched_group_barrier(0x002, 3, 0);
              __builtin_amdgcn_sched_group_barrier(0x080, 1, 0);
              __builtin_amdgcn_sched_group_barrier(0x020, 1, 0);
            } else {
              __builtin_amdgcn_sched_group_barrier(0x002, 4, 0);
              __builtin_amdgcn_sched_group_barrier(0x080, 2, 0);
            }
          } else {
            __builtin_amdgcn_sched_group_barrier(0x002, 5, 0);
            __builtin_amdgcn_sched_group_barrier(0x100, 1, 0);
            __builtin_amdgcn_sched_group_barrier(0x200, 1, 0);
          }
        }
        __builtin_amdgcn_sched_barrier(0);
      }
      lds_barrier();
    }
  }

  float* pb = part + (((long long)s * d.MTo + ob) * d.MTc + cb) * (27 * 1024);
#pragma unroll
  for (int t7 = 0; t7 < 7; ++t7) {
    const int tap = t7 < 6 ? 3 * (wave + 4 * (t7 / 3)) + t7 % 3 : 24 + wave;
    if (tap < 27) {
#pragma unroll
      for (int q = 0; q < 16; ++q) {
        const int i = (q & 3) + 8 * (q >> 2) + 4 * half;
        pb[tap * 1024 + i * 32 + (lane & 31)] = F16 ? (acc[t7][q] + acs[t7][q]) * unscale : acc[t7][q] + acs[t7][q];
      }
    }
  }
}

}

namespace mode {

int conv3d_bww_split_launch(const float* gy, const float* x, float* part, const WgradSplitDims& d, hipStream_t st, const char* who,
                            const float* amax_g, const float* amax_x) {
  if (amax_g) {
    int rc = allow_lds(conv3d_bww_split_kernel<true>, LDS_BYTES, who);
    if (rc != MODE_OK) return rc;
    hipLaunchKernelGGL(conv3d_bww_split_kernel<true>, dim3(d.S, d.MTo, d.MTc), dim3(NT), LDS_BYTES, st, gy, x, part, d, amax_g, amax_x);
    return check_launch(who);
  }
  int rc = allow_lds(conv3d_bww_split_kernel<false>, LDS_BYTES, who);
  if (rc != MODE_OK) return rc;
  hipLaunchKernelGGL(conv3d_bww_split_kernel<false>, dim3(d.S, d.MTo, d.MTc), dim3(NT), LDS_BYTES, st, gy, x, part, d, nullptr, nullptr);
  return check_launch(who);
}

}
```

### mode-2022_amd/csrc/split_arith.h

```cpp
#pragma once
#ifdef __HIPCC__
#include <hip/hip_runtime.h>

#include <cstdint>

namespace mode {
namespace split {

typedef float f32x2 __attribute__((ext_vector_type(2)));
typedef float f32x16 __attribute__((ext_vector_type(16)));
typedef __bf16 bf16x2 __attribute__((ext_vector_type(2)));
typedef __bf16 bf16x8 __attribute__((ext_vector_type(8)));
typedef _Float16 f16x2 __attribute__((ext_vector_type(2)));
typedef _Float16 f16x8 __attribute__((ext_vector_type(8)));

template <bool F16> struct Arith {
  static constexpr int NP = F16 ? 2 : 3;
  static constexpr int NTERM = F16 ? 3 : 6;
};

__device__ __forceinline__ uint32_t pack2(float a, float b) {
  const f32x2 v = {a, b};
  return __builtin_bit_cast(uint32_t, __builtin_convertvector(v, bf16x2));
}
// ... 7 lines not shown
  return p;
}
__device__ __forceinline__ void split3_bf16_pinned(float a, float b, uint32_t& p1, uint32_t& p2, uint32_t& p3) {
  p1 = split_step_bf16_pinned(a, b);
  p2 = split_step_bf16_pinned(a, b);
  p3 = pack2(a, b);
}

__device__ __forceinline__ void split3_bf16_subfma(float a, float b, uint32_t& p1, uint32_t& p2, uint32_t& p3) {
  p1 = pack2(a, b);
  const float ra = a - __builtin_bit_cast(float, p1 << 16), rb = __builtin_fmaf(-1.f, __builtin_bit_cast(float, p1 & 0xffff0000u), b);
  p2 = pack2(ra, rb);
  const float sa = ra - __builtin_bit_cast(float, p2 << 16), sb = __builtin_fmaf(-1.f, __builtin_bit_cast(float, p2 & 0xffff0000u), rb);
  p3 = pack2(sa, sb);
}


__device__ __forceinline__ void split2_f16_subfma(float a, float b, uint32_t& p1, uint32_t& p2) {
  const f32x2 v = {a, b};
  const f16x2 h1 = __builtin_convertvector(v, f16x2);
  p1 = __builtin_bit_cast(uint32_t, h1);
  const f32x2 r = {a - (float)h1[0], __builtin_fmaf(-1.f, (float)h1[1], b)};
  p2 = __builtin_bit_cast(uint32_t, __builtin_convertvector(r, f16x2));
}

__device__ __forceinline__ void split2_f16_pinned(float a, float b, uint32_t& p1, uint32_t& p2) {
  const f32x2 v = {a, b};
  const f16x2 h1 = __builtin_convertvector(v, f16x2);
  p1 = __builtin_bit_cast(uint32_t, h1);
  float ra = a - (float)h1[0], rb = b - (float)h1[1];
  asm("" : "+v"(ra), "+v"(rb));
  const f32x2 r = {ra, rb};
  p2 = __builtin_bit_cast(uint32_t, __builtin_convertvector(r, f16x2));
}

__device__ __forceinline__ void split2_f16_mix(float a, float b, uint32_t& p1, uint32_t& p2) {
  const f32x2 v = {a, b};
  const f16x2 h1 = __builtin_convertvector(v, f16x2);
  p1 = __builtin_bit_cast(uint32_t, h1);
  float ra, rb;
  asm("v_fma_mix_f32 %0, 1.0, %3, -%2 op_sel_hi:[0,0,1]\n\t"
      "v_fma_mix_f32 %1, 1.0, %4, -%2 op_sel:[0,0,1] op_sel_hi:[0,0,1]"
      : "=&v"(ra), "=&v"(rb)
      : "v"(p1), "v"(a), "v"(b));
  const f32x2 r = {ra, rb};
  p2 = __builtin_bit_cast(uint32_t, __builtin_convertvector(r, f16x2));
}

__device__ __forceinline__ float f16_scale_of(float m) {
  const unsigned e = min(max((__builtin_bit_cast(unsigned, m) >> 23) & 0xffu, 64u), 254u);
  return m == 0.f ? 1.f : __builtin_bit_cast(float, (268u - e) << 23);
}

__device__ __forceinline__ f32x16 mfma_bf16(uint4 a, uint4 b, f32x16 c) {
  return __builtin_amdgcn_mfma_f32_32x32x16_bf16(__builtin_bit_cast(bf16x8, a), __builtin_bit_cast(bf16x8, b), c, 0, 0, 0);
}
__device__ __forceinline__ f32x16 mfma_f16(uint4 a, uint4 b, f32x16 c) {
  return __builtin_amdgcn_mfma_f32_32x32x16_f16(__builtin_bit_cast(f16x8, a), __builtin_bit_cast(f16x8, b), c, 0, 0, 0);
}
template <bool F16>
__device__ __forceinline__ f32x16 mfma_split(uint4 a, uint4 b, f32x16 c) {
  if constexpr (F16)
    return mfma_f16(a, b, c);
  else
    return mfma_bf16(a, b, c);
}

__device__ __forceinline__ void lds_barrier() { asm volatile("s_waitcnt lgkmcnt(0)\n\ts_barrier" ::: "memory"); }

}
}
#endif
```

### mode-2022_amd/mode_hip/__init__.py

```python
import ctypes
import os
import threading

import torch

HERE = os.path.dirname(os.path.abspath(__file__))
LIB_PATH = os.path.join(HERE, 'libmode_hip.so')

_c_int = ctypes.c_int
_c_ptr = ctypes.c_void_p
_c_size = ctypes.c_size_t

SIGNATURES = {
    'mode_hip_abi_version': (_c_int, []),
    'mode_last_error': (ctypes.c_char_p, []),
    'mode_debug_poison': (_c_int, [ctypes.c_uint, _c_ptr]),
    'mode_weight_pack_reuse': (_c_int, [_c_int]),
    'mode_sum_n': (_c_int, [_c_ptr] * 5 + [ctypes.c_longlong, _c_ptr]),
    'mode_conv3d_fwd_split_stats_partials': (_c_int, []),
    'mode_conv3d_fwd_split_stats': (_c_int, [_c_ptr] * 5 + [_c_int] * 6 + [_c_ptr]),
    'mode_bn_train_fwd_prestats': (_c_int, [_c_ptr] * 7 + [ctypes.c_float] * 2 + [_c_int] + [_c_ptr] * 6 + [_c_int] * 3 +
                                   [ctypes.c_longlong, _c_ptr]),
    'mode_sphere_conv_wpack_bytes': (_c_size, [_c_int] * 5),
    'mode_sphere_conv_fwd': (_c_int, [_c_ptr] * 5 + [_c_int] * 12 + [_c_ptr]),
# ... 34 lines not shown
    'mode_cost_volume_bwd': (_c_int, [_c_ptr] * 3 + [_c_int] * 5 + [_c_ptr]),
    'mode_conv2d_wpack_bytes': (_c_size, [_c_int] * 2),
    'mode_conv2d_fwd': (_c_int, [_c_ptr] * 4 + [_c_int] * 6 + [_c_ptr]),
    'mode_conv2d_fwd_bn': (_c_int, [_c_ptr] * 5 + [_c_int] * 6 + [_c_ptr]),
    'mode_zero_insert2': (_c_int, [_c_ptr] * 2 + [ctypes.c_longlong] + [_c_int] * 2 + [_c_ptr]),
    'mode_conv2d_bwd_data': (_c_int, [_c_ptr] * 4 + [_c_int] * 6 + [_c_ptr]),
    'mode_conv2d_bwd_weight_workspace_bytes': (_c_size, [_c_int] * 5),
    'mode_conv2d_bwd_weight': (_c_int, [_c_ptr] * 4 + [_c_int] * 7 + [_c_ptr]),
    'mode_conv1x1_wpack_bytes': (_c_size, [_c_int] * 2),
    'mode_conv1x1_fwd': (_c_int, [_c_ptr] * 4 + [_c_int] * 6 + [_c_ptr]),
    'mode_conv1x1_fwd_bn': (_c_int, [_c_ptr] * 5 + [_c_int] * 6 + [_c_ptr]),
    'mode_conv1x1_bwd_data': (_c_int, [_c_ptr] * 4 + [_c_int] * 6 + [_c_ptr]),
    'mode_conv1x1_bwd_weight_workspace_bytes': (_c_size, [_c_int] * 6),
    'mode_conv1x1_bwd_weight': (_c_int, [_c_ptr] * 4 + [_c_int] * 7 + [_c_ptr]),
    'mode_conv_stem_wpack_bytes': (_c_size, [_c_int] * 2),
    'mode_conv_stem_fwd': (_c_int, [_c_ptr] * 4 + [_c_int] * 5 + [_c_ptr]),
    'mode_conv_stem_fwd_bn': (_c_int, [_c_ptr] * 5 + [_c_int] * 5 + [_c_ptr]),
    'mode_conv_stem_bwd_weight_workspace_bytes': (_c_size, [_c_int] * 5),
    'mode_conv_stem_bwd_weight': (_c_int, [_c_ptr] * 4 + [_c_int] * 6 + [_c_ptr]),
    'mode_cost_conv_assemble_fwd': (_c_int, [_c_ptr] * 3 + [_c_int] * 5 + [_c_ptr]),
    'mode_cost_conv_assemble_fwd_bn': (_c_int, [_c_ptr] * 4 + [_c_int] * 5 + [_c_ptr]),
    'mode_cost_conv_assemble_fwd_bn_amax': (_c_int, [_c_ptr] * 5 + [_c_int] * 5 + [_c_ptr]),
    'mode_cost_conv_assemble_bwd': (_c_int, [_c_ptr] * 3 + [_c_int] * 5 + [_c_ptr]),
    'mode_conv3d_wpack_bytes': (_c_size, [_c_int] * 2),
    'mode_conv3d_fwd': (_c_int, [_c_ptr] * 4 + [_c_int] * 7 + [_c_ptr]),
    'mode_conv3d_fwd_bn': (_c_int, [_c_ptr] * 5 + [_c_int] * 7 + [_c_ptr]),
    'mode_deconv3d_fwd_bn': (_c_int, [_c_ptr] * 5 + [_c_int] * 6 + [_c_ptr]),
    'mode_conv3d_bwd_data': (_c_int, [_c_ptr] * 4 + [_c_int] * 7 + [_c_ptr]),
    'mode_conv2d_split_supported': (_c_int, [_c_int] * 4),
    'mode_conv2d_split_shape_supported': (_c_int, [_c_int] * 6),
    'mode_conv2d_fwd_split': (_c_int, [_c_ptr] * 5 + [_c_int] * 6 + [_c_ptr]),
    'mode_conv2d_bwd_data_split': (_c_int, [_c_ptr] * 4 + [_c_int] * 6 + [_c_ptr]),
    'mode_conv2d_bwd_data_split_acc': (_c_int, [_c_ptr] * 5 + [_c_int] * 6 + [_c_ptr]),
    'mode_conv2d_fwd_split_f16': (_c_int, [_c_ptr] * 6 + [_c_int] * 6 + [_c_ptr]),
    'mode_conv2d_fwd_split_f16_bn': (_c_int, [_c_ptr] * 7 + [_c_int] * 6 + [_c_ptr]),
    'mode_conv2d_bwd_data_split_f16': (_c_int, [_c_ptr] * 7 + [_c_int] * 6 + [_c_ptr]),
    'mode_conv2d_bwd_weight_split': (_c_int, [_c_ptr] * 4 + [_c_int] * 7 + [_c_ptr]),
    'mode_conv2d_bwd_weight_split_f16': (_c_int, [_c_ptr] * 6 + [_c_int] * 7 + [_c_ptr]),
    'mode_conv3d_split_supported': (_c_int, [_c_int] * 4),
    'mode_conv3d_split_shape_supported': (_c_int, [_c_int] * 7),
    'mode_conv3d_fwd_split': (_c_int, [_c_ptr] * 5 + [_c_int] * 6 + [_c_ptr]),
    'mode_conv3d_fwd_s2_split': (_c_int, [_c_ptr] * 5 + [_c_int] * 6 + [_c_ptr]),
    'mode_conv3d_fwd_s2_split_amax': (_c_int, [_c_ptr] * 6 + [_c_int] * 6 + [_c_ptr]),
    'mode_deconv3d_split_supported': (_c_int, [_c_int] * 2),
    'mode_deconv3d_fwd_split': (_c_int, [_c_ptr] * 4 + [_c_int] * 6 + [_c_ptr]),
    'mode_deconv3d_split_bn_supported': (_c_int, [_c_int] * 2),
    'mode_conv3d_bwd_data_split_acc_supported': (_c_int, [_c_int] * 3),
    'mode_abs_max': (_c_int, [_c_ptr, ctypes.c_longlong, _c_ptr, _c_ptr]),
    'mode_abs_max_batch': (_c_int, [_c_ptr, _c_ptr, _c_int, _c_ptr, _c_ptr]),
    'mode_conv3d_fwd_split_f16': (_c_int, [_c_ptr] * 6 + [_c_int] * 6 + [_c_ptr]),
    'mode_conv3d_fwd_split_f16_bn': (_c_int, [_c_ptr] * 7 + [_c_int] * 6 + [_c_ptr]),
    'mode_conv3d_bwd_data_split_f16': (_c_int, [_c_ptr] * 7 + [_c_int] * 6 + [_c_ptr]),
    'mode_conv3d_bwd_weight_split_f16': (_c_int, [_c_ptr] * 6 + [_c_int] * 7 + [_c_ptr]),
    'mode_conv3d_bwd_data_split_acc': (_c_int, [_c_ptr] * 5 + [_c_int] * 7 + [_c_ptr]),
    'mode_deconv3d_fwd_split_bn': (_c_int, [_c_ptr] * 5 + [_c_int] * 6 + [_c_ptr]),
    'mode_deconv3d_fwd_split_bn_amax': (_c_int, [_c_ptr] * 6 + [_c_int] * 6 + [_c_ptr]),
    'mode_conv3d_bwd_data_s2_split': (_c_int, [_c_ptr] * 4 + [_c_int] * 6 + [_c_ptr]),
    'mode_conv3d_bwd_data_split': (_c_int, [_c_ptr] * 4 + [_c_int] * 6 + [_c_ptr]),
    'mode_conv3d_bwd_weight_split': (_c_int, [_c_ptr] * 4 + [_c_int] * 7 + [_c_ptr]),
    'mode_conv3d_bwd_weight_s2_split': (_c_int, [_c_ptr] * 4 + [_c_int] * 7 + [_c_ptr]),
    'mode_conv3d_bwd_weight_workspace_bytes': (_c_size, [_c_int] * 7),
    'mode_deconv3d_fwd': (_c_int, [_c_ptr] * 4 + [_c_int] * 6 + [_c_ptr]),
    'mode_conv3d_bwd_weight': (_c_int, [_c_ptr] * 4 + [_c_int] * 8 + [_c_ptr]),
    'mode_head_fwd': (_c_int, [_c_ptr] * 3 + [_c_int] * 7 + [_c_ptr]),
    'mode_head_bwd_workspace_bytes': (_c_size, [_c_int] * 4),
    'mode_head_bwd': (_c_int, [_c_ptr] * 4 + [_c_int] * 7 + [_c_ptr]),
    'mode_head_bwd_conf': (_c_int, [_c_ptr] * 7 + [_c_int] * 7 + [_c_ptr]),
    'mode_smooth_l1_workspace_bytes': (_c_size, [ctypes.c_longlong]),
    'mode_smooth_l1_masked': (_c_int, [_c_ptr] * 4 + [ctypes.c_float] * 3 + [_c_ptr] * 3 + [ctypes.c_longlong, _c_ptr]),
    'mode_head_loss_supported': (_c_int, [_c_int] * 7),
    'mode_head_bwd_loss': (_c_int, [_c_ptr] * 3 + [ctypes.c_float] + [_c_ptr] * 3 + [_c_int] * 7 + [_c_ptr]),
    'mode_disp2depth': (_c_int, [_c_ptr] * 2 + [_c_int] * 2 + [ctypes.c_float, _c_ptr]),
    'mode_grid_sample_border': (_c_int, [_c_ptr] * 3 + [_c_int] * 7 + [_c_ptr]),
    'mode_depth_view_trans_workspace_bytes': (_c_size, [_c_int] * 2),
    'mode_depth_view_trans': (_c_int, [_c_ptr] * 8 + [_c_int] * 2 + [_c_ptr]),
    'mode_depth_view_project': (_c_int, [_c_ptr] * 6 + [_c_int] * 2 + [_c_ptr]),
    'mode_zbuffer': (_c_int, [_c_ptr] * 6 + [ctypes.c_longlong, _c_ptr]),
    'mode_multiview_handoff_workspace_bytes': (_c_size, [_c_int] * 3),
    'mode_multiview_handoff': (_c_int, [_c_ptr] * 2 + [_c_int] * 3 + [_c_ptr] * 4 + [_c_int] + [_c_ptr] * 3),
    'mode_multiview_handoff_bwd': (_c_int, [_c_ptr] * 3 + [_c_int] * 3 + [_c_ptr] * 6 + [_c_int] * 2 + [_c_ptr] * 2),
    'mode_multiview_handoff_bwd_full': (_c_int, [_c_ptr] * 3 + [_c_int] * 3 + [_c_ptr] * 6 + [_c_int] * 2 + [_c_ptr] * 3),
    'mode_classif_workspace_bytes': (_c_size, [_c_int] * 5),
    'mode_classif_train_fwd': (_c_int, [_c_ptr] * 6 + [ctypes.c_float] * 2 + [_c_ptr] * 8 + [_c_int] * 5 + [_c_ptr]),
    'mode_classif_train_bwd': (_c_int, [_c_ptr] * 13 + [_c_int] + [_c_ptr] + [_c_int] * 5 + [_c_ptr]),
    'mode_bn_workspace_bytes': (_c_size, [_c_int]),
    'mode_bn_train_fwd': (_c_int, [_c_ptr] * 7 + [ctypes.c_float] * 2 + [_c_int] + [_c_ptr] * 6 + [_c_int] * 2 +
                          [ctypes.c_longlong, _c_int, _c_ptr]),
    'mode_bn_eval_fwd': (_c_int, [_c_ptr] * 6 + [ctypes.c_float, _c_int] + [_c_ptr] + [_c_int] * 2 + [ctypes.c_longlong, _c_ptr]),
    'mode_bn_train_bwd': (_c_int, [_c_ptr] * 8 + [_c_int] + [_c_ptr] * 4 + [_c_int] + [_c_ptr] + [_c_int] * 2 +
                          [ctypes.c_longlong, _c_int, _c_ptr]),
    'mode_bn_train_fwd_amax': (_c_int, [_c_ptr] * 7 + [ctypes.c_float] * 2 + [_c_int] + [_c_ptr] * 6 + [_c_int] * 2 +
                               [ctypes.c_longlong, _c_int, _c_ptr, _c_ptr]),
    'mode_bn_train_fwd_prestats_amax': (_c_int, [_c_ptr] * 7 + [ctypes.c_float] * 2 + [_c_int] + [_c_ptr] * 6 + [_c_int] * 3 +
                                        [ctypes.c_longlong, _c_ptr, _c_ptr]),
    'mode_bn_train_bwd_amax': (_c_int, [_c_ptr] * 8 + [_c_int] + [_c_ptr] * 4 + [_c_int] + [_c_ptr] + [_c_int] * 2 +
                               [ctypes.c_longlong, _c_int, _c_ptr, _c_ptr]),
    'mode_classif_train_bwd_amax': (_c_int, [_c_ptr] * 13 + [_c_int] + [_c_ptr] + [_c_int] * 5 + [_c_ptr, _c_ptr]),
    'mode_maxpool2x2_fwd': (_c_int, [_c_ptr] * 2 + [ctypes.c_longlong, _c_int, _c_int, _c_ptr]),
    'mode_maxpool2x2_bwd': (_c_int, [_c_ptr] * 3 + [ctypes.c_longlong, _c_int, _c_int, _c_ptr]),
    'mode_depth_to_space2': (_c_int, [_c_ptr] * 4 + [_c_int] * 5 + [_c_ptr]),
    'mode_space_to_depth2': (_c_int, [_c_ptr] * 2 + [_c_int] * 4 + [_c_ptr]),
    'mode_conv1x1_sigmoid_fwd': (_c_int, [_c_ptr] * 4 + [_c_int] * 2 + [ctypes.c_longlong, _c_ptr]),
    'mode_conv1x1_sigmoid_bwd_workspace_bytes': (_c_size, [_c_int, ctypes.c_longlong]),
    'mode_conv1x1_sigmoid_bwd': (_c_int, [_c_ptr] * 7 + [_c_int] + [_c_ptr] + [_c_int] * 2 + [ctypes.c_longlong, _c_ptr]),
    'mode_masked_metrics_workspace_bytes': (_c_size, [ctypes.c_longlong]),
    'mode_masked_metrics': (_c_int, [_c_ptr] * 3 + [ctypes.c_longlong] + [_c_ptr] * 2 + [_c_size] + [_c_ptr] * 2),
# ... 92 lines not shown
```

### mode-2022_amd/mode_hip/functional.py

```python
import collections
import ctypes
import threading

import torch

from . import METRICS_COUNT, METRICS_MAX_THRESHOLDS, BnEpilogue, MetricsParams, check, lib, profiling, ptr, require_f32c, require_gpu, stream_of


def _stream_capturing():
  return torch.cuda.is_initialized() and torch.cuda.is_current_stream_capturing()


class _LRU(object):
  capturing = staticmethod(_stream_capturing)

  def __init__(self, maxsize):
    self.maxsize = maxsize
    self.d = collections.OrderedDict()
    self.pinned = {}

  def _touch(self, key):
    if key in self.pinned:
      return self.pinned[key]
    value = self.d[key]
# ... 1905 lines not shown
_bn_tls = threading.local()


def known_abs_max(t):
  tag = getattr(t, '_mode_amax', None)
  return tag[0] if tag is not None and tag[1] == t._version and tag[2] == t.data_ptr() else None


class BnActFunction(torch.autograd.Function):

  @staticmethod
  def forward(ctx, y, add, gamma, beta, running_mean, running_var, momentum, eps, relu, num_batches_tracked=None, groups=1, prestats_ws=None,
              add_carrier=None):
    ctx.add_carrier = add_carrier
    require_gpu(y, add, gamma, beta)
    y = y.contiguous()
    add = add.contiguous() if add is not None else None
    require_f32c(y, gamma, beta)
    B, C, S = _bcs(y)
    out = torch.empty_like(y)
    if B % groups:
      raise RuntimeError('BatchNorm statistics groups: batch %d is not divisible by %d' % (B, groups))
    mean = torch.empty(groups * C, dtype=torch.float32, device=y.device)
    invstd = torch.empty_like(mean)
    from_y = bool(relu) and add is None
    coef = torch.empty((2, groups * C), dtype=torch.float32, device=y.device) if from_y else None
    nbytes = 4 * y.numel() * (3 + (1 if add is not None else 0))
    with torch.cuda.device_of(y), profiling.region(_tag_bn('bn_train_fwd', y), nbytes, 0, y.device):
      common = (ptr(y), ptr(add) if add is not None else None, ptr(gamma), ptr(beta), ptr(running_mean) if running_mean is not None else None,
                ptr(running_var) if running_var is not None else None, ptr(num_batches_tracked) if num_batches_tracked is not None else None,
                float(momentum), float(eps), int(relu), ptr(out), ptr(mean), ptr(invstd), ptr(coef[0]) if from_y else None,
                ptr(coef[1]) if from_y else None)
      _bn_tls.out_amax = out_amax = None
      if CONV_ARITH == 'bf16x6' and ((CONV3D_S1_F16 and y.dim() == 5) or (SPHERE_FWD_F16 and y.dim() == 4 and C % 16 == 0)):
        _bn_tls.out_amax = out_amax = torch.empty(BN_ABSMAX_FLOATS, dtype=torch.float32, device=y.device)
      if prestats_ws is not None:
        if groups != 1:
          raise RuntimeError('BatchNorm with precomputed statistics takes one statistics group')
        check(lib().mode_bn_train_fwd_prestats_amax(*common, ptr(prestats_ws), lib().mode_conv3d_fwd_split_stats_partials(), B, C, S,
                                                    ptr(out_amax) if out_amax is not None else None, stream_of(y)),
              'mode_bn_train_fwd_prestats_amax')
      else:
        ws = _bn_ws(C * groups, y.device)
        check(lib().mode_bn_train_fwd_amax(*common, ptr(ws), B, C, S, groups, ptr(out_amax) if out_amax is not None else None, stream_of(y)),
              'mode_bn_train_fwd_amax')
    _written_by_kernel(running_mean, running_var, num_batches_tracked)
    ctx.save_for_backward(y, out if (relu and not from_y) else None, gamma, beta, mean, invstd, coef)
    ctx.relu, ctx.has_add, ctx.groups = bool(relu), add is not None, groups
    return out

  @staticmethod
  def backward(ctx, gout):
    y, out, gamma, beta, mean, invstd, coef = ctx.saved_tensors
    gout = gout.contiguous()
    B, C, S = _bcs(y)
    gy = torch.empty_like(y)
    need_gadd = ctx.has_add and ctx.relu and ctx.needs_input_grad[1]
    gadd = torch.empty_like(y) if need_gadd else None
    sink_g, sink_b = grad_sink(gamma), grad_sink(beta)
    fused = sink_g is not None and sink_b is not None and ctx.needs_input_grad[2] and ctx.needs_input_grad[3]
    ggamma = sink_g if fused else torch.empty_like(gamma)
    gbeta = sink_b if fused else torch.empty_like(gamma)
    if need_gadd and out is not None:
      nbytes = 4 * y.numel() * 7
    else:
      nbytes = 4 * y.numel() * (2 * (2 + (1 if out is not None else 0)) + 1 + (1 if need_gadd else 0))
    gy_amax = None
    if CONV_ARITH == 'bf16x6' and ((CONV3D_S1_F16 and y.dim() == 5) or (SPHERE_BWD_F16 and y.dim() == 4 and C % 16 == 0)):
      gy_amax = torch.empty(BN_ABSMAX_FLOATS, dtype=torch.float32, device=y.device)
    with torch.cuda.device_of(y), profiling.region(_tag_bn('bn_train_bwd', y), nbytes, 0, y.device):
      ws = _bn_ws(C * ctx.groups, y.device)
      check(lib().mode_bn_train_bwd_amax(ptr(gout), ptr(y), ptr(out) if out is not None else None, ptr(gamma), ptr(mean), ptr(invstd),
                                         ptr(coef[0]) if coef is not None else None, ptr(coef[1]) if coef is not None else None, int(ctx.relu),
                                         ptr(gy), ptr(gadd) if gadd is not None else None, ptr(ggamma), ptr(gbeta),
                                         int(fused), ptr(ws), B, C, S, ctx.groups, ptr(gy_amax) if gy_amax is not None else None,
                                         stream_of(y)), 'mode_bn_train_bwd_amax')
    if gy_amax is not None:
      gy._mode_amax = (gy_amax, gy._version, gy.data_ptr())
    if fused:
      ggamma = gbeta = None
    if ctx.has_add and not ctx.relu:
      gadd = gout
    if gadd is not None and ctx.add_carrier is not None:
      prev = ctx.add_carrier.take(ctx)
      if prev is not None:
        gadd = gadd + prev
      elif ctx.add_carrier.leave(gadd, ctx):
        gadd = None
    return gy, gadd, ggamma, gbeta, None, None, None, None, None, None, None, None, None


def bn_eval(y, add, gamma, beta, running_mean, running_var, eps, relu):
  require_gpu(y, add, gamma, beta, running_mean, running_var)
  y = y.contiguous()
  add = add.contiguous() if add is not None else None
  require_f32c(y, gamma, beta, running_mean, running_var)
  B, C, S = _bcs(y)
  out = torch.empty_like(y)
  nbytes = 4 * y.numel() * (2 + (1 if add is not None else 0))
  with torch.cuda.device_of(y), profiling.region('bn_eval_fwd', nbytes, 0, y.device):
    check(lib().mode_bn_eval_fwd(ptr(y), ptr(add) if add is not None else None, ptr(gamma), ptr(beta), ptr(running_mean),
                                 ptr(running_var), float(eps), int(relu), ptr(out), B, C, S, stream_of(y)), 'mode_bn_eval_fwd')
  return out


def bn_act(bn, y, add=None, relu=False, groups=1, add_carrier=None):
  use_batch_stats = bn.training or bn.running_mean is None
  if use_batch_stats:
    momentum = bn.momentum
    update = bn.training and bn.track_running_stats
    nbt = bn.num_batches_tracked if update else None
    if groups > 1 and momentum is None:
      raise NotImplementedError('grouped BatchNorm statistics need a fixed momentum')
    if nbt is not None and (momentum is None or not (nbt.is_cuda and nbt.dtype == torch.int64)):
      nbt.add_(groups)
      if momentum is None:
        momentum = 1.0 / float(nbt)
      nbt = None
    if add_carrier is not None:
      add_carrier.arm(add is not None and add.requires_grad and torch.is_grad_enabled())
    out = BnActFunction.apply(y, add, bn.weight, bn.bias, bn.running_mean if update else None, bn.running_var if update else None,
                              momentum if momentum is not None else 0.0, bn.eps, relu, nbt, groups, None, add_carrier)
    am = getattr(_bn_tls, 'out_amax', None)
    if am is not None:
      _bn_tls.out_amax = None
      out._mode_amax = (am, out._version, out.data_ptr())
    return out
  if torch.is_grad_enabled() and (y.requires_grad or bn.weight.requires_grad):
    out = torch.nn.functional.batch_norm(y, bn.running_mean, bn.running_var, bn.weight, bn.bias, False, 0.0, bn.eps)
    out = out + add if add is not None else out
    return torch.relu(out) if relu else out
  return bn_eval(y, add, bn.weight, bn.bias, bn.running_mean, bn.running_var, bn.eps, relu)


CLASSIF_FUSED = True


def classif_fused_supported(y, bn, conv):
  return (CLASSIF_FUSED and y.is_cuda and y.dtype == torch.float32 and y.dim() == 5 and y.shape[0] > 0 and y.shape[1] <= 32 and
          bn.training and bn.momentum is not None and bn.weight is not None and bn.bias is not None and
          type(conv) is torch.nn.Conv3d and conv.out_channels == 1 and conv.in_channels == y.shape[1] and conv.bias is None and
          tuple(conv.kernel_size) == (3, 3, 3) and tuple(conv.stride) == (1, 1, 1) and tuple(conv.padding) == (1, 1, 1) and
          tuple(conv.dilation) == (1, 1, 1) and conv.groups == 1 and conv.padding_mode == 'zeros' and
          y.shape[1] * y.shape[2] * y.shape[3] * y.shape[4] < 2**30)


class ClassifHeadFunction(torch.autograd.Function):

  @staticmethod
  def forward(ctx, y, w, gamma, beta, add, running_mean, running_var, momentum, eps, num_batches_tracked):
    require_gpu(y, w, gamma, beta, add)
    y, w = y.contiguous(), w.contiguous()
    add = add.contiguous() if add is not None else None
    require_f32c(y, w, gamma, beta)
    B, C, D, H, W = y.shape
    cost = torch.empty((B, 1, D, H, W), dtype=y.dtype, device=y.device)
    if add is not None:
      require_f32c(add)
      if tuple(add.shape) != tuple(cost.shape):
        raise RuntimeError('classifier head: residual %s does not match the output %s' % (tuple(add.shape), tuple(cost.shape)))
    saved = torch.empty((4, C), dtype=torch.float32, device=y.device)
    with torch.cuda.device_of(y), profiling.region(_tag3('classif_fwd', C, 1, 1, D, H, W), 4 * (2 * y.numel() + cost.numel() * (2 if add is not None else 1)),
                                                   2 * cost.numel() * C * 27, y.device):
      ws = torch.empty(max(lib().mode_classif_workspace_bytes(B, C, D, H, W) // 4, 1), dtype=torch.float32, device=y.device)
      check(lib().mode_classif_train_fwd(ptr(y), ptr(gamma), ptr(beta), ptr(running_mean) if running_mean is not None else None,
                                         ptr(running_var) if running_var is not None else None,
                                         ptr(num_batches_tracked) if num_batches_tracked is not None else None, float(momentum), float(eps),
                                         ptr(w), ptr(add) if add is not None else None, ptr(cost), ptr(saved[0]), ptr(saved[1]), ptr(saved[2]),
                                         ptr(saved[3]), ptr(ws), B, C, D, H, W, stream_of(y)), 'mode_classif_train_fwd')
    _written_by_kernel(running_mean, running_var, num_batches_tracked)
    ctx.save_for_backward(y, w, gamma, beta, saved)
    ctx.has_add = add is not None
    return cost

  @staticmethod
  def backward(ctx, gcost):
    y, w, gamma, beta, saved = ctx.saved_tensors
    gcost = gcost.contiguous()
    B, C, D, H, W = y.shape
    gy = torch.empty_like(y)
    sink_w = grad_sink(w) if ctx.needs_input_grad[1] else None
    sink_g, sink_b = grad_sink(gamma), grad_sink(beta)
    fused = sink_w is not None and sink_g is not None and sink_b is not None and ctx.needs_input_grad[2] and ctx.needs_input_grad[3]
    gw = sink_w if fused else torch.empty_like(w)
    ggamma = sink_g if fused else torch.empty_like(gamma)
# ... 597 lines not shown
```

### mode-2022_amd/models/mode_disparity.py

```python
from __future__ import print_function

import math

import torch
import torch.nn as nn
import torch.nn.functional as F

from mode_hip import functional as HF

from . import stage3d
from .submodule import convbn_3d, feature_extraction, sphere_feature_extraction


class hourglass(nn.Module):

  def __init__(self, inplanes):
    super(hourglass, self).__init__()
    c2 = inplanes * 2
    self.conv1 = nn.Sequential(convbn_3d(inplanes, c2, kernel_size=3, stride=2, pad=1), nn.ReLU(inplace=True))
    self.conv2 = convbn_3d(c2, c2, kernel_size=3, stride=1, pad=1)
    self.conv3 = nn.Sequential(convbn_3d(c2, c2, kernel_size=3, stride=2, pad=1), nn.ReLU(inplace=True))
    self.conv4 = nn.Sequential(convbn_3d(c2, c2, kernel_size=3, stride=1, pad=1), nn.ReLU(inplace=True))
    self.conv5 = nn.Sequential(nn.ConvTranspose3d(c2, c2, kernel_size=3, padding=1, output_padding=1, stride=2, bias=False),
                               nn.BatchNorm3d(c2))
    self.conv6 = nn.Sequential(nn.ConvTranspose3d(c2, inplanes, kernel_size=3, padding=1, output_padding=1, stride=2, bias=False),
                               nn.BatchNorm3d(inplanes))

  def forward(self, x, presqu, postsqu, *, residual=None, pre_consumers=1, x_carrier=None):
    out = stage3d.conv_bn(self.conv1[0], x, relu=True) if x_carrier is None else stage3d.conv_bn(self.conv1[0], x, relu=True, x_carrier=x_carrier)
    pre = stage3d.conv_bn(self.conv2, out, relu=True, add=postsqu)
    inner = 1 + (1 if presqu is None else 0)
    alias = HF.fan_out(pre, inner + pre_consumers) if inner + pre_consumers > 2 else (pre,) * (inner + pre_consumers)
    out = stage3d.conv_bn(self.conv3[0], alias[0], relu=True)
    out = stage3d.conv_bn(self.conv4[0], out, relu=True)
    post = stage3d.conv_bn(self.conv5, out, relu=True, add=presqu if presqu is not None else alias[1])
    out = stage3d.conv_bn(self.conv6, post, add=residual)
    return out, (alias[inner] if pre_consumers == 1 else tuple(alias[inner:])), post


def _cumulative_bn(module):
  return any(isinstance(m, nn.modules.batchnorm._BatchNorm) and m.momentum is None for m in module.modules())


class ModeDisparity(nn.Module):
  pair_extractor = True
  fold_cost_volume = True

  def __init__(self, maxdisp, conv='Sphere', in_height=1024, in_width=512, sphereType='Cassini', out_conf=False):
    super(ModeDisparity, self).__init__()
    print("MODE stereo matching network!")
    self.maxdisp = maxdisp
    self.out_conf = out_conf
    if conv == 'Regular':
      self.feature_extraction = feature_extraction()
      print("using Regular feature extraction!")
    elif conv == 'Sphere':
      self.feature_extraction = sphere_feature_extraction(in_height, in_width, sphereType)
      print("using Spherical feature extraction!")
    else:
      raise NotImplementedError("Convolution Type must be Regular or Sphere!")

    relu = lambda: nn.ReLU(inplace=True)
    self.dres0 = nn.Sequential(convbn_3d(64, 32, 3, 1, 1), relu(), convbn_3d(32, 32, 3, 1, 1), relu())
    self.dres1 = nn.Sequential(convbn_3d(32, 32, 3, 1, 1), relu(), convbn_3d(32, 32, 3, 1, 1))
    self.dres2 = hourglass(32)
    self.dres3 = hourglass(32)
    self.dres4 = hourglass(32)
    for i in (1, 2, 3):
      setattr(self, 'classif%d' % i,
              nn.Sequential(convbn_3d(32, 32, 3, 1, 1), relu(), nn.Conv3d(32, 1, kernel_size=3, padding=1, stride=1, bias=False)))
    self._psmnet_init()

  def _psmnet_init(self):
    for m in self.modules():
      if isinstance(m, (nn.Conv2d, nn.Conv3d)):
        n = m.out_channels
        for k in m.kernel_size:
          n *= k
        m.weight.data.normal_(0, math.sqrt(2. / n))
      elif isinstance(m, (nn.BatchNorm2d, nn.BatchNorm3d)):
        m.weight.data.fill_(1)
        m.bias.data.zero_()
      elif isinstance(m, nn.Linear):
        m.bias.data.zero_()

  def forward(self, left, right):
    cost1, cost2, cost3 = self._logits(left, right)
    size = (self.maxdisp, left.size(2), left.size(3))
    if self.training:
      return stage3d.head(cost1, size), stage3d.head(cost2, size), stage3d.head(cost3, size)
    if self.out_conf:
      return stage3d.head(cost3, size, with_confidence=True)
    return stage3d.head(cost3, size)

  def forward_loss(self, left, right, disp_true, count=None, weights=(0.5, 0.7, 1.0)):
    if not self.training:
      raise RuntimeError('forward_loss() is the training step; call the module itself for inference')
    costs = self._logits(left, right)
    size = (self.maxdisp, left.size(2), left.size(3))
    gt = disp_true.reshape(left.size(0), 1, left.size(2), left.size(3))
    if count is None:
      count = (~torch.isnan(gt)).sum().to(torch.float32).clamp(min=1)
    if HF.head_loss_supported(costs[0], size):
      return HF.head_loss(costs, size, gt, count.reciprocal(), weights)
    preds = tuple(stage3d.head(c, size) for c in costs)
    mask = ~torch.isnan(gt)
    gt0 = torch.nan_to_num(gt)
    loss = 0
    for wgt, o in zip(weights, preds):
      per = F.smooth_l1_loss(o, gt0, reduction='none')
      loss = loss + wgt * torch.where(mask, per, torch.zeros((), dtype=per.dtype, device=per.device)).sum() / count
    return loss, tuple(p.detach() for p in preds)

  def _logits(self, left, right):
    if left.is_cuda:
      with HF.weight_maxima(self):
        return self._logits_body(left, right)
    return self._logits_body(left, right)

  def _logits_body(self, left, right):
    if self.pair_extractor and left.shape == right.shape and not _cumulative_bn(self.feature_extraction):
      with stage3d.bn_groups(2):
        fea = self.feature_extraction(torch.cat((left, right), 0))
      ref_fea, tgt_fea = fea[:left.shape[0]], fea[left.shape[0]:]
    else:
      ref_fea = self.feature_extraction(left)
      tgt_fea = self.feature_extraction(right)

    conv0 = self.dres0[0][0]
    if (self.fold_cost_volume and ref_fea.is_cuda and conv0.bias is None and tuple(conv0.kernel_size) == (3, 3, 3) and
        tuple(conv0.stride) == (1, 1, 1) and tuple(conv0.padding) == (1, 1, 1) and conv0.in_channels == 2 * ref_fea.shape[1] and
        HF.cost_conv_supported(ref_fea, self.maxdisp // 4, conv0.out_channels)):
      if HF.bn_foldable(self.dres0[0][1]):
        cost0 = HF.cost_conv_bn_eval(ref_fea, tgt_fea, conv0.weight, self.maxdisp // 4, self.dres0[0][1], relu=True)
      else:
        y0 = HF.cost_conv(ref_fea, tgt_fea, conv0.weight, self.maxdisp // 4)
        cost0 = stage3d.bn_act(self.dres0[0][1], y0, None, True)
    else:
      cost = HF.cost_volume(ref_fea, tgt_fea, self.maxdisp // 4)
      cost0 = stage3d.conv_bn(self.dres0[0], cost, relu=True)
    cost0 = stage3d.conv_bn(self.dres0[2], cost0, relu=True)
    car = HF.grad_carrier(cost0)
    if car is None:
      t = stage3d.conv_bn(self.dres1[0], cost0, relu=True)
      cost0 = stage3d.conv_bn(self.dres1[2], t, add=cost0)
    else:
      t = stage3d.conv_bn(self.dres1[0], cost0, relu=True, x_carrier=car)
      cost0 = stage3d.conv_bn(self.dres1[2], t, add=cost0, add_carrier=car)

    c0 = HF.fan_out(cost0, 4)
    out1, pre1, post1 = self.dres2(c0[0], None, None, residual=c0[1], pre_consumers=2)
    car1 = HF.grad_carrier(out1)
    kw1 = {} if car1 is None else {'x_carrier': car1}
    out2, pre2, post2 = self.dres3(out1, pre1[0], post1, residual=c0[2], **kw1)
    car2 = HF.grad_carrier(out2)
    kw2 = {} if car2 is None else {'x_carrier': car2}
    out3, pre3, post3 = self.dres4(out2, pre1[1], post2, residual=c0[3], **kw2)

    cost1 = stage3d.classify(self.classif1, out1, **kw1)
    cost2 = stage3d.classify(self.classif2, out2, add=cost1, **kw2)
    cost3 = stage3d.classify(self.classif3, out3, add=cost2)
    return cost1, cost2, cost3
```

### mode-2022_amd/models/stage3d.py

```python
import contextlib
import threading

import torch
import torch.nn as nn
import torch.nn.functional as F

from mode_hip import functional as HF



def _hip_kind(conv, x):
  if conv.kernel_size != (3, 3, 3) or conv.padding != (1, 1, 1) or conv.dilation != (1, 1, 1) or \
      conv.groups != 1 or conv.bias is not None or conv.in_channels > 64 or conv.out_channels > 64:
    return None
  if type(conv) is nn.Conv3d:
    if conv.stride == (1, 1, 1):
      return 'conv1'
    if conv.stride == (2, 2, 2) and all(s % 2 == 0 for s in x.shape[2:]):
      return 'conv2'
  if type(conv) is nn.ConvTranspose3d and conv.stride == (2, 2, 2) and conv.output_padding == (1, 1, 1):
    return 'deconv'
  return None


def conv3(conv, x, carrier=None):
  if not x.is_cuda:
    raise NotImplementedError('Only support cuda tensor!')
  kind = _hip_kind(conv, x)
  if kind == 'conv1':
    return HF.conv3d(x, conv.weight, 1, carrier)
  if kind == 'conv2':
    return HF.conv3d(x, conv.weight, 2, carrier)
  if kind == 'deconv':
    return HF.deconv3d(x, conv.weight)
  if type(conv) is nn.Conv2d and conv.kernel_size == (3, 3) and conv.stride == (1, 1) and conv.groups == 1 and \
      conv.bias is None and conv.padding == conv.dilation and conv.dilation in ((1, 1), (2, 2)) and conv.padding_mode == 'zeros' and \
      x.dtype == torch.float32 and x.is_cuda:
    if torch.is_grad_enabled() and (conv.weight.requires_grad or x.requires_grad):
      if HF.conv2d_wgrad_supported(x, conv.weight):
        return HF.conv2d_3x3(x.contiguous(), conv.weight, conv.dilation[0], carrier)
    elif HF._conv2d_own(x, conv.weight):
      return HF.conv2d_fwd(x.contiguous(), conv.weight.detach().contiguous(), conv.dilation[0])
  if type(conv) is nn.Conv2d and HF.conv2d_3x3_s2_supported(x, conv) and torch.is_grad_enabled() and (conv.weight.requires_grad or x.requires_grad):
    return HF.conv2d_3x3_s2(x, conv)
  if type(conv) is nn.Conv2d and HF.conv_stem_supported(x, conv):
    return HF.conv_stem(x, conv)
  if type(conv) is nn.Conv2d and HF.conv1x1_supported(x, conv):
    return HF.conv1x1(x, conv)
  if type(conv) is nn.Conv2d and HF.conv2d_tabled_supported(x, conv):
    return HF.conv2d_tabled(x, conv)
  return conv(x)


def conv_bn(seq, x, relu=False, add=None, x_carrier=None, add_carrier=None):
  conv, bn = seq[0], seq[1]
  if x.is_cuda and x.dtype == torch.float32 and HF.bn_foldable(bn):
    y = _conv_bn_folded(conv, bn, x, add, relu)
    if y is not None:
      return y
  if (x.is_cuda and bn.training and current_bn_groups() == 1 and _hip_kind(conv, x) == 'conv1' and conv.out_channels > 1 and
      torch.is_grad_enabled() and HF.conv3d_stats_supported(x, conv.weight, bn)):
    return HF.conv3d_bn_train(x, conv.weight, bn, add, relu)
  y = conv3(conv, x) if x_carrier is None else conv3(conv, x, x_carrier)
  return bn_act(bn, y, add, relu) if add_carrier is None else bn_act(bn, y, add, relu, add_carrier)


def _conv_bn_folded(conv, bn, x, add, relu):
  kind = _hip_kind(conv, x)
  if kind == 'conv1' and conv.out_channels > 1:
    return HF.conv3d_bn_eval(x, conv.weight, bn, 1, add, relu)
  if kind == 'conv2':
    return HF.conv3d_bn_eval(x, conv.weight, bn, 2, add, relu)
  if kind == 'deconv':
    return HF.deconv3d_bn_eval(x, conv.weight, bn, add, relu)
  if hasattr(conv, 'forward_bn'):
    return conv.forward_bn(x, bn, add, relu)
  if type(conv) is nn.Conv2d and conv.groups == 1 and conv.bias is None and conv.padding_mode == 'zeros':
    if conv.kernel_size == (3, 3) and conv.stride == (1, 1) and conv.padding == conv.dilation and conv.dilation in ((1, 1), (2, 2)) and \
        HF._conv2d_own(x, conv.weight):
      return HF.conv2d_bn_eval(x, conv.weight, bn, conv.dilation[0], add, relu)
    if HF.conv_stem_supported(x, conv):
      return HF.conv_stem_fwd(x, conv.weight, bn, add, relu)
    if HF.conv1x1_supported(x, conv):
      return HF.conv1x1_fwd(x, conv.weight, conv.stride[0], bn, add, relu)
    if HF.conv2d_tabled_supported(x, conv):
      return HF.conv2d_tabled_bn_eval(x, conv, bn, add, relu)
  return None


_tls = threading.local()


def current_bn_groups():
  return getattr(_tls, 'bn_groups', 1)


@contextlib.contextmanager
def bn_groups(n):
  prev = current_bn_groups()
  _tls.bn_groups = n
  try:
    yield
  finally:
    _tls.bn_groups = prev


def bn_act(bn, y, add=None, relu=False, add_carrier=None):
  if not y.is_cuda:
    raise NotImplementedError('Only support cuda tensor!')
  if not HF.bn_supported(y):
    return bn_act_torch(bn, y, add, relu)
  return HF.bn_act(bn, y, add, relu, groups=current_bn_groups() if bn.training else 1, add_carrier=add_carrier)


def bn_act_torch(bn, y, add=None, relu=False, add_carrier=None):
  groups = current_bn_groups()
  if groups > 1 and bn.training:
    y = torch.cat([bn(part) for part in y.chunk(groups, 0)], 0)
  else:
    y = bn(y)
  if add is not None:
    y = y + add
  return F.relu(y, inplace=True) if relu else y


def classify(seq, x, *, add=None, x_carrier=None):
  conv0, bn = seq[0][0], seq[0][1]
  if (x.is_cuda and bn.training and torch.is_grad_enabled() and current_bn_groups() == 1 and _hip_kind(conv0, x) == 'conv1' and
      conv0.out_channels > 1):
    y = conv3(conv0, x) if x_carrier is None else conv3(conv0, x, x_carrier)
    if HF.classif_fused_supported(y, bn, seq[2]):
      return HF.classif_head_train(y, bn, seq[2], add)
    cost = conv3(seq[2], bn_act(bn, y, None, True))
  else:
    cost = conv3(seq[2], conv_bn(seq[0], x, relu=True) if x_carrier is None else conv_bn(seq[0], x, relu=True, x_carrier=x_carrier))
  return cost if add is None else cost + add


def head(cost, size, with_confidence=False):
  if not cost.is_cuda:
    raise NotImplementedError('Only support cuda tensor!')
  if with_confidence:
    return HF.head_fwd(cost, size, with_confidence=True)
  return HF.head(cost, size)
```

Before: 38.05 pairs/s.

## Defer BN+ReLU into the next conv3d prologue in training hourglass layers

Adds a deferred-activation path: after a conv whose BN+ReLU output only feeds another stride-1 3x3x3 conv, the raw conv output is kept and BN statistics, scale/shift and the activation's abs-max are computed in one stats pass that also tracks per-channel min/max. The next conv's forward and weight-gradient kernels apply scale/shift/ReLU in their input prologue, so the normalized activation tensor is never written or re-read. Backward recomputes the BN-ReLU gradient from the saved pre-activation. This trades materialisation traffic for extra per-element work in the conv prologues and more kernel variants.

```diff
diff --git a/include/mode_hip.h b/include/mode_hip.h
--- a/include/mode_hip.h
+++ b/include/mode_hip.h
@@ -234,6 +234,17 @@
                                  float* wpack, int B, int Ci, int D, int H, int W, int Co, mode_stream_t stream);
 int mode_conv3d_bwd_weight_split_f16(const float* gy, const float* x, const float* amax_g, const float* amax_x, float* gw, float* workspace,
                                      int B, int Ci, int D, int H, int W, int Co, int accumulate, mode_stream_t stream);
+size_t mode_bn_coef_amax_workspace_bytes(int C);
+int mode_bn_train_coef_amax(const float* y, const float* gamma, const float* beta, float* running_mean, float* running_var,
+                            long long* num_batches_tracked, float momentum, float eps, float* save_mean, float* save_invstd, float* scale,
+                            float* shift, float* act_absmax, float* workspace, int B, int C, long long S, int groups, mode_stream_t stream);
+int mode_conv3d_bnrelu_prologue_supported(int Ci, int Co, int D, int H, int W);
+int mode_conv3d_fwd_split_f16_bnrelu(const float* x, const float* scale, const float* shift, const float* w, const float* amax_a,
+                                     const float* amax_w, float* y, float* wpack, int B, int Ci, int D, int H, int W, int Co,
+                                     mode_stream_t stream);
+int mode_conv3d_bwd_weight_split_f16_bnrelu(const float* gy, const float* x, const float* scale, const float* shift, const float* amax_g,
+                                            const float* amax_a, float* gw, float* workspace, int B, int Ci, int D, int H, int W, int Co,
+                                            int accumulate, mode_stream_t stream);
 int mode_conv3d_bwd_data_split_acc_supported(int Ci, int Co, int stride);
 int mode_conv3d_bwd_data_split_acc(const float* gy, const float* w, const float* acc, float* gx, float* wpack, int B, int Ci, int D, int H,
                                    int W, int Co, int stride, mode_stream_t stream);
diff --git a/mode-2022_amd/csrc/bn_act.hip b/mode-2022_amd/csrc/bn_act.hip
--- a/mode-2022_amd/csrc/bn_act.hip
+++ b/mode-2022_amd/csrc/bn_act.hip
@@ -32,9 +32,17 @@
   }
 }
 
+template <bool MINMAX = false>
 __global__ __launch_bounds__(NT) void bn_stats_kernel(const float* __restrict__ y, float* __restrict__ partial, int B, int C,
-                                                      long long S, int nsplit, unsigned* __restrict__ zero) {
+                                                      long long S, int nsplit, unsigned* __restrict__ zero,
+                                                      float* __restrict__ minmax = nullptr) {
   __shared__ float sh[2 * NW];
+  float lo = __builtin_inff(), hi = -__builtin_inff();
+  auto track = [&](float v) {
+    const bool finite = __builtin_fabsf(v) < __builtin_inff();
+    lo = finite ? fminf(lo, v) : lo;
+    hi = finite ? fmaxf(hi, v) : hi;
+  };
   const int c = blockIdx.y, split = blockIdx.x;
   const int Bg = B / gridDim.z, b0 = blockIdx.z * Bg;
   const long long prow = (long long)blockIdx.z * C + c;
@@ -49,6 +57,9 @@
       const float dx = v.x - K, dy = v.y - K, dz = v.z - K, dw = v.w - K;
       s0 += (dx + dy) + (dz + dw);
       s1 += (dx * dx + dy * dy) + (dz * dz + dw * dw);
+      if (MINMAX) {
+        track(v.x); track(v.y); track(v.z); track(v.w);
+      }
     };
     const long long st = (long long)nsplit * NT;
     long long i = (long long)split * NT + threadIdx.x;
@@ -66,6 +77,7 @@
         const float dq = q[i] - K;
         s0 += dq;
         s1 += dq * dq;
+        if (MINMAX) track(q[i]);
       }
     }
   }
@@ -73,6 +85,29 @@
   if (threadIdx.x == 0) {
     partial[(prow * nsplit + split) * 2] = s0;
     partial[(prow * nsplit + split) * 2 + 1] = s1;
+  }
+  if (MINMAX) {
+#pragma unroll
+    for (int off = 32; off > 0; off >>= 1) {
+      lo = fminf(lo, __shfl_down(lo, off, 64));
+      hi = fmaxf(hi, __shfl_down(hi, off, 64));
+    }
+    __syncthreads();
+    const int wave = threadIdx.x >> 6;
+    if ((threadIdx.x & 63) == 0) {
+      sh[wave] = lo;
+      sh[NW + wave] = hi;
+    }
+    __syncthreads();
+    if (threadIdx.x == 0) {
+#pragma unroll
+      for (int w = 1; w < NW; ++w) {
+        lo = fminf(lo, sh[w]);
+        hi = fmaxf(hi, sh[NW + w]);
+      }
+      minmax[(prow * nsplit + split) * 2] = lo;
+      minmax[(prow * nsplit + split) * 2 + 1] = hi;
+    }
   }
 }
 
@@ -523,7 +558,8 @@
   }
   const int nsplit = prestats > 0 ? prestats : pick_nsplit(C * groups, S);
   if (prestats <= 0)
-    hipLaunchKernelGGL(bn_stats_kernel, dim3(nsplit, C, groups), dim3(NT), 0, st, y, workspace, B, C, S, nsplit, reinterpret_cast<unsigned*>(amax));
+    hipLaunchKernelGGL(bn_stats_kernel<false>, dim3(nsplit, C, groups), dim3(NT), 0, st, y, workspace, B, C, S, nsplit, reinterpret_cast<unsigned*>(amax),
+                       (float*)nullptr);
   BnCoefArgs k{workspace, gamma, beta, running_mean, running_var, num_batches_tracked, save_mean, save_invstd, save_scale, save_shift,
                momentum, eps, nsplit,
                (double)(B / groups) * (double)S, groups, B / groups, prestats > 0 ? workspace + 2LL * C * nsplit : nullptr,
@@ -584,10 +620,95 @@
   MODE_REQUIRE(aligned_rows(y, S) && aligned16(workspace), MODE_ERR_UNSUPPORTED, "%s: unaligned buffer", who);
   MODE_REQUIRE((running_mean == nullptr) == (running_var == nullptr), MODE_ERR_BAD_ARG, "%s: running stats must come in pairs", who);
   const int nsplit = pick_nsplit(C, S);
-  hipLaunchKernelGGL(bn_stats_kernel, dim3(nsplit, C, 1), dim3(NT), 0, st, y, workspace, B, C, S, nsplit, (unsigned*)nullptr);
+  hipLaunchKernelGGL(bn_stats_kernel<false>, dim3(nsplit, C, 1), dim3(NT), 0, st, y, workspace, B, C, S, nsplit, (unsigned*)nullptr, (float*)nullptr);
   BnCoefArgs k{workspace, gamma, beta, running_mean, running_var, num_batches_tracked, save_mean, save_invstd, save_scale, save_shift,
                momentum, eps, nsplit, (double)B * (double)S, 1, B, nullptr};
   hipLaunchKernelGGL(bn_finalize_kernel, dim3(C), dim3(NT), 0, st, y, k, C, S);
+  return mode::check_launch(who);
+}
+
+namespace {
+__global__ __launch_bounds__(NT) void bn_coef_amax_kernel(const float* __restrict__ y, BnCoefArgs k, const float* __restrict__ minmax, int C,
+                                                          long long S) {
+  __shared__ double shd[2 * NW];
+  __shared__ float shm[2 * NW];
+  const int c = blockIdx.x;
+  unsigned mag = 0;
+  for (int g = 0; g < k.groups; ++g) {
+    double s0, s1;
+    reduce_partials(k.partial, g * C + c, k.nsplit, s0, s1, shd);
+    float lo = __builtin_inff(), hi = -__builtin_inff();
+    for (int i = threadIdx.x; i < k.nsplit; i += NT) {
+      const float2 v = reinterpret_cast<const float2*>(minmax)[(long long)(g * C + c) * k.nsplit + i];
+      lo = fminf(lo, v.x);
+      hi = fmaxf(hi, v.y);
+    }
+#pragma unroll
+    for (int off = 32; off > 0; off >>= 1) {
+      lo = fminf(lo, __shfl_down(lo, off, 64));
+      hi = fmaxf(hi, __shfl_down(hi, off, 64));
+    }
+    if ((threadIdx.x & 63) == 0) {
+      shm[threadIdx.x >> 6] = lo;
+      shm[NW + (threadIdx.x >> 6)] = hi;
+    }
+    __syncthreads();
+    if (threadIdx.x == 0) {
+#pragma unroll
+      for (int w = 1; w < NW; ++w) {
+        lo = fminf(lo, shm[w]);
+        hi = fmaxf(hi, shm[NW + w]);
+      }
+      const double dm = s0 / k.count;
+      const double mean = (double)y[((long long)(g * k.Bg) * C + c) * S] + dm;
+      double var = s1 / k.count - dm * dm;
+      if (var < 0.0) var = 0.0;
+      const double invstd = 1.0 / sqrt(var + (double)k.eps);
+      const double sc = (double)k.gamma[c] * invstd;
+      const float fsc = (float)sc, fsh = (float)((double)k.beta[c] - mean * sc);
+      k.save_mean[g * C + c] = (float)mean;
+      k.save_invstd[g * C + c] = (float)invstd;
+      k.save_scale[g * C + c] = fsc;
+      k.save_shift[g * C + c] = fsh;
+      if (k.running_mean) {
+        const double unbiased = k.count > 1.0 ? var * k.count / (k.count - 1.0) : var;
+        k.running_mean[c] = (float)((1.0 - k.momentum) * (double)k.running_mean[c] + k.momentum * mean);
+        k.running_var[c] = (float)((1.0 - k.momentum) * (double)k.running_var[c] + k.momentum * unbiased);
+      }
+      if (lo <= hi)
+        mag = max(mag, max(mode::absmax_mag(relu_nan(__builtin_fmaf(lo, fsc, fsh))), mode::absmax_mag(relu_nan(__builtin_fmaf(hi, fsc, fsh)))));
+    }
+    __syncthreads();
+  }
+  if (threadIdx.x == 0) {
+    if (c == 0 && k.num_batches_tracked) *k.num_batches_tracked += k.groups;
+    if (mag) atomicMax(k.amax + 16 * (1 + c % mode::ABSMAX_SLOTS), mag);
+  }
+}
+}
+
+extern "C" size_t mode_bn_coef_amax_workspace_bytes(int C) { return 2 * mode_bn_workspace_bytes(C); }
+
+extern "C" int mode_bn_train_coef_amax(const float* y, const float* gamma, const float* beta, float* running_mean, float* running_var,
+                                       long long* num_batches_tracked, float momentum, float eps, float* save_mean, float* save_invstd,
+                                       float* scale, float* shift, float* act_absmax, float* workspace, int B, int C, long long S, int groups,
+                                       mode_stream_t stream) {
+  const char* who = "mode_bn_train_coef_amax";
+  int rc = check_bn(B, C, S, who);
+  if (rc != MODE_OK) return rc;
+  MODE_REQUIRE(B > 0, MODE_ERR_BAD_ARG, "%s: empty batch has no statistics", who);
+  MODE_REQUIRE(y && gamma && beta && save_mean && save_invstd && scale && shift && act_absmax && workspace, MODE_ERR_BAD_ARG, "%s: null pointer", who);
+  MODE_REQUIRE(aligned_rows(y, S) && aligned16(workspace), MODE_ERR_UNSUPPORTED, "%s: unaligned buffer", who);
+  MODE_REQUIRE((running_mean == nullptr) == (running_var == nullptr), MODE_ERR_BAD_ARG, "%s: running stats must come in pairs", who);
+  MODE_REQUIRE(groups >= 1 && B % groups == 0, MODE_ERR_BAD_ARG, "%s: batch %d not divisible into %d groups", who, B, groups);
+  hipStream_t st = mode::as_stream(stream);
+  const int nsplit = pick_nsplit(C * groups, S);
+  float* minmax = workspace + mode_bn_workspace_bytes(C * groups) / sizeof(float);
+  hipLaunchKernelGGL(bn_stats_kernel<true>, dim3(nsplit, C, groups), dim3(NT), 0, st, y, workspace, B, C, S, nsplit,
+                     reinterpret_cast<unsigned*>(act_absmax), minmax);
+  BnCoefArgs k{workspace, gamma, beta, running_mean, running_var, num_batches_tracked, save_mean, save_invstd, scale, shift,
+               momentum, eps, nsplit, (double)(B / groups) * (double)S, groups, B / groups, nullptr, reinterpret_cast<unsigned*>(act_absmax)};
+  hipLaunchKernelGGL(bn_coef_amax_kernel, dim3(C), dim3(NT), 0, st, y, k, minmax, C, S);
   return mode::check_launch(who);
 }
 
diff --git a/mode-2022_amd/csrc/conv3d.hip b/mode-2022_amd/csrc/conv3d.hip
--- a/mode-2022_amd/csrc/conv3d.hip
+++ b/mode-2022_amd/csrc/conv3d.hip
@@ -630,6 +630,22 @@
   return mode::conv3d_s1_split(x, w, y, wpack, B, Ci, Co, D, H, W, 0, mode::as_stream(stream), who, nullptr, nullptr, nullptr, amax_x, amax_w);
 }
 
+extern "C" int mode_conv3d_fwd_split_f16_bnrelu(const float* x, const float* scale, const float* shift, const float* w, const float* amax_a,
+                                                const float* amax_w, float* y, float* wpack, int B, int Ci, int D, int H, int W, int Co,
+                                                mode_stream_t stream) {
+  const char* who = "mode_conv3d_fwd_split_f16_bnrelu";
+  int rc = check_split_args(x, w, y, wpack, B, Ci, D, H, W, Co, 1, 0, who);
+  if (rc != MODE_OK || B == 0) return rc;
+  MODE_REQUIRE(amax_a && amax_w, MODE_ERR_BAD_ARG, "%s: null operand maximum", who);
+  MODE_REQUIRE(scale && shift, MODE_ERR_BAD_ARG, "%s: null BatchNorm coefficients", who);
+  return mode::conv3d_s1_split(x, w, y, wpack, B, Ci, Co, D, H, W, 0, mode::as_stream(stream), who, nullptr, nullptr, nullptr, amax_a, amax_w,
+                               nullptr, scale, shift);
+}
+
+extern "C" int mode_conv3d_bnrelu_prologue_supported(int Ci, int Co, int D, int H, int W) {
+  return (mode_conv3d_split_shape_supported(Ci, Co, D, H, W, 1, 0) == 1 && mode_conv3d_split_shape_supported(Ci, Co, D, H, W, 1, 2) == 1) ? 1 : 0;
+}
+
 extern "C" int mode_conv3d_fwd_split_f16_bn(const float* x, const float* w, const float* amax_x, const mode_bn_epilogue* bn, float* y,
                                             float* amax_y, float* wpack, int B, int Ci, int D, int H, int W, int Co, mode_stream_t stream) {
   const char* who = "mode_conv3d_fwd_split_f16_bn";
@@ -1322,7 +1338,8 @@
 }
 
 static int bwd_weight_split(const float* gy, const float* x, const float* amax_g, const float* amax_x, float* gw, float* workspace, int B, int Ci,
-                            int D, int H, int W, int Co, int accumulate, mode_stream_t stream, const char* who);
+                            int D, int H, int W, int Co, int accumulate, mode_stream_t stream, const char* who, const float* pro_scale = nullptr,
+                            const float* pro_shift = nullptr);
 
 extern "C" int mode_conv3d_bwd_weight_split(const float* gy, const float* x, float* gw, float* workspace, int B, int Ci, int D, int H,
                                             int W, int Co, int accumulate, mode_stream_t stream) {
@@ -1335,8 +1352,20 @@
   return bwd_weight_split(gy, x, amax_g, amax_x, gw, workspace, B, Ci, D, H, W, Co, accumulate, stream, "mode_conv3d_bwd_weight_split_f16");
 }
 
+extern "C" int mode_conv3d_bwd_weight_split_f16_bnrelu(const float* gy, const float* x, const float* scale, const float* shift,
+                                                       const float* amax_g, const float* amax_a, float* gw, float* workspace, int B, int Ci, int D,
+                                                       int H, int W, int Co, int accumulate, mode_stream_t stream) {
+  const char* who = "mode_conv3d_bwd_weight_split_f16_bnrelu";
+  int rc = check_split_args(gy, x, gw, workspace, B, Ci, D, H, W, Co, 1, 2, who);
+  if (rc != MODE_OK) return rc;
+  MODE_REQUIRE(amax_g && amax_a, MODE_ERR_BAD_ARG, "%s: null operand maximum", who);
+  MODE_REQUIRE(scale && shift, MODE_ERR_BAD_ARG, "%s: null BatchNorm coefficients", who);
+  return bwd_weight_split(gy, x, amax_g, amax_a, gw, workspace, B, Ci, D, H, W, Co, accumulate, stream, who, scale, shift);
+}
+
 static int bwd_weight_split(const float* gy, const float* x, const float* amax_g, const float* amax_x, float* gw, float* workspace, int B, int Ci,
-                            int D, int H, int W, int Co, int accumulate, mode_stream_t stream, const char* who) {
+                            int D, int H, int W, int Co, int accumulate, mode_stream_t stream, const char* who, const float* pro_scale,
+                            const float* pro_shift) {
   int rc = check_split_args(gy, x, gw, workspace, B, Ci, D, H, W, Co, 1, 2, who);
   if (rc != MODE_OK) return rc;
   hipStream_t st = mode::as_stream(stream);
@@ -1357,7 +1386,7 @@
   q.units = B * d.nHt * d.nWt * q.nDc;
   if (S > q.units) S = q.units;
   q.S = d.S = S;
-  rc = mode::conv3d_bww_split_launch(gy, x, workspace, q, st, who, amax_g, amax_x);
+  rc = mode::conv3d_bww_split_launch(gy, x, workspace, q, st, who, amax_g, amax_x, pro_scale, pro_shift);
   if (rc != MODE_OK) return rc;
   hipLaunchKernelGGL(reduce_gw3d, dim3(mode::cdiv((long long)d.MTo * d.MTc * 27 * 1024, 32)), dim3(256), 0, st, workspace, gw, d, accumulate);
   return mode::check_launch("mode_conv3d_bwd_weight_split(reduce)");
diff --git a/mode-2022_amd/csrc/conv3d_internal.h b/mode-2022_amd/csrc/conv3d_internal.h
--- a/mode-2022_amd/csrc/conv3d_internal.h
+++ b/mode-2022_amd/csrc/conv3d_internal.h
@@ -19,7 +19,8 @@
 int conv3d_split_stat_partials();
 int conv3d_s1_split(const float* x, const float* w, float* y, float* wpack, int B, int K, int rows, int D, int H, int W, int flip,
                     hipStream_t st, const char* who, const mode_bn_epilogue* bn, float* stats = nullptr, const float* acc_in = nullptr,
-                    const float* amax_x = nullptr, const float* amax_w = nullptr, float* amax_y = nullptr);
+                    const float* amax_x = nullptr, const float* amax_w = nullptr, float* amax_y = nullptr, const float* pro_scale = nullptr,
+                    const float* pro_shift = nullptr);
 
 int abs_max(const float* x, long long n, float* out, hipStream_t st, const char* who);
 int abs_max_batch(const float* const* ptrs, const long long* sizes, int n, float* out, hipStream_t st, const char* who);
@@ -41,7 +42,8 @@
   int S, MTo, MTc;
 };
 int conv3d_bww_split_launch(const float* gy, const float* x, float* part, const WgradSplitDims& d, hipStream_t st, const char* who,
-                            const float* amax_g = nullptr, const float* amax_x = nullptr);
+                            const float* amax_g = nullptr, const float* amax_x = nullptr,
+                            const float* pro_scale = nullptr, const float* pro_shift = nullptr);
 
 struct WgradS2SplitDims {
   int Ci, Co, D, H, W, Do, Ho, Wo;
diff --git a/mode-2022_amd/csrc/conv3d_split.hip b/mode-2022_amd/csrc/conv3d_split.hip
--- a/mode-2022_amd/csrc/conv3d_split.hip
+++ b/mode-2022_amd/csrc/conv3d_split.hip
@@ -106,11 +106,13 @@
   if (lane == 0) pivot[o] = acc;
 }
 
-template <int MT, int EPI, bool F16 = false, int TH_ = 8, bool AMAX = false>
+template <int MT, int EPI, bool F16 = false, int TH_ = 8, bool AMAX = false, bool PRO = false>
 __global__ __launch_bounds__(NT) void conv3d_split_kernel(const float* __restrict__ x, const uint4* __restrict__ wp,
                                                           float* __restrict__ y, SDims d, Epi epi, float* __restrict__ stats,
                                                           const float* __restrict__ stat_pivot, const float* __restrict__ amax_x,
-                                                          const float* __restrict__ amax_w, unsigned* __restrict__ amax_y) {
+                                                          const float* __restrict__ amax_w, unsigned* __restrict__ amax_y,
+                                                          const float* __restrict__ pro_scale, const float* __restrict__ pro_shift) {
+  static_assert(!PRO || (F16 && EPI == 0 && !AMAX), "the BatchNorm prologue exists for the training forward on two fp16 pieces");
   constexpr int NP = Arith<F16>::NP, NTERM = Arith<F16>::NTERM, BUF = buf_of<F16, TH_>();
   using Ge = Geo<TH_>;
   constexpr int TH = Ge::TH, IH = Ge::IH, ITEMS = Ge::ITEMS, KIT = Ge::KIT, PIECE = Ge::PIECE, R = Ge::R, RB = Ge::RB;
@@ -176,6 +178,8 @@
   for (int c = 0; c < 8; ++c) soff[c] = (unsigned)c * (unsigned)DHW * 4u;
   __amdgpu_buffer_rsrc_t st_rs = buf_rsrc(x, 0);
   int st_base = 0, st_d0 = 0, st_h0 = 0, st_w0 = 0;
+  float pro_sc[8], pro_sh[8], pro_s[KIT];
+  const float half_sx = 0.5f * sx;
   auto stage_advance = [&](int step) {
     s_ch += step;
     const int wrap = s_ch >= d.NCHUNK ? 1 : 0;
@@ -197,20 +201,32 @@
     st_w0 = sw * 32;
     st_rs = buf_rsrc(x + ((long long)sb * d.K + s_ch * 8) * DHW, (unsigned)DHW * 32u);
     st_base = (st_d0 - 1) * (int)HW + (st_h0 - 1) * d.W + (st_w0 - 1);
+    if (PRO) {
+#pragma unroll
+      for (int c = 0; c < 8; ++c) {
+        pro_sc[c] = pro_scale[s_ch * 8 + c];
+        pro_sh[c] = pro_shift[s_ch * 8 + c];
+      }
+    }
   };
   auto stage_load = [&](int k) {
     const unsigned ok = (unsigned)((unsigned)(st_d0 + pdz[k] - 1) < (unsigned)d.D) & (unsigned)((unsigned)(st_h0 + phy[k] - 1) < (unsigned)d.H) &
                         (unsigned)((unsigned)(st_w0 + pwi[k] - 1) < (unsigned)d.W);
     const unsigned off = ok ? (unsigned)(st_base + poff[k]) * 4u : kBufOOB;
+    if (PRO) pro_s[k] = ok ? half_sx : 0.f;
 #pragma unroll
     for (int c = 0; c < 8; ++c) raw[k][c] = buf_load_f32(st_rs, off, soff[c]);
   };
   uint32_t sq[3][4];
   auto stage_commit = [&](int buf, int k, int h) {
+    const float sxk = PRO ? pro_s[k] : sx;
 #pragma unroll
     for (int j = 2 * h; j < 2 * h + 2; ++j) {
       float v0 = raw[k][2 * j], v1 = raw[k][2 * j + 1];
-      if (F16) {
+      if (PRO) {
+        v0 = bnrelu_scaled(v0, pro_sc[2 * j], pro_sh[2 * j], sxk);
+        v1 = bnrelu_scaled(v1, pro_sc[2 * j + 1], pro_sh[2 * j + 1], sxk);
+      } else if (F16) {
         v0 *= sx;
         v1 *= sx;
       }
@@ -369,7 +385,11 @@
 #pragma unroll
       for (int i = 0; i < MT * 4 * NTERM; ++i) {
         __builtin_amdgcn_sched_group_barrier(0x008, 1, 0);
-        __builtin_amdgcn_sched_group_barrier(0x002, 3, 0);
+        if constexpr (PRO) {
+          __builtin_amdgcn_sched_group_barrier(0x002, 4, 0);
+        } else {
+          __builtin_amdgcn_sched_group_barrier(0x002, 3, 0);
+        }
         if (F16) {
           __builtin_amdgcn_sched_group_barrier(0x080, 1, 0);
           __builtin_amdgcn_sched_group_barrier(0x020, 1, 0);
@@ -464,17 +484,18 @@
 template <int MT>
 int launch_split(const float* x, const float* wpack, float* y, SDims d, int nblocks, hipStream_t st, const char* who, Epi epi,
                  float* stats = nullptr, const float* stat_pivot = nullptr, const float* amax_x = nullptr, const float* amax_w = nullptr,
-                 float* amax_y = nullptr) {
+                 float* amax_y = nullptr, const float* pro_scale = nullptr, const float* pro_shift = nullptr) {
   const uint4* wp = reinterpret_cast<const uint4*>(wpack);
   const int grid = kNumCU;
-#define MODE_SPLIT_LAUNCH_TH(EPIV, F16V, THV, AMAXV, STATS, PIVOT)                                                           \
+#define MODE_SPLIT_LAUNCH_PRO(EPIV, F16V, THV, AMAXV, PROV, STATS, PIVOT)                                                    \
   {                                                                                                                          \
-    int rc = mode::allow_lds(conv3d_split_kernel<MT, EPIV, F16V, THV, AMAXV>, lds_bytes<F16V, THV>(), who);                  \
+    int rc = mode::allow_lds(conv3d_split_kernel<MT, EPIV, F16V, THV, AMAXV, PROV>, lds_bytes<F16V, THV>(), who);            \
     if (rc != MODE_OK) return rc;                                                                                            \
-    hipLaunchKernelGGL((conv3d_split_kernel<MT, EPIV, F16V, THV, AMAXV>), dim3(grid, nblocks), dim3(NT), (lds_bytes<F16V, THV>()), st, x, wp, \
-                       y, d, epi, STATS, PIVOT, amax_x, amax_w, reinterpret_cast<unsigned*>(amax_y));                        \
+    hipLaunchKernelGGL((conv3d_split_kernel<MT, EPIV, F16V, THV, AMAXV, PROV>), dim3(grid, nblocks), dim3(NT), (lds_bytes<F16V, THV>()), st, \
+                       x, wp, y, d, epi, STATS, PIVOT, amax_x, amax_w, reinterpret_cast<unsigned*>(amax_y), pro_scale, pro_shift); \
     return mode::check_launch(who);                                                                                          \
   }
+#define MODE_SPLIT_LAUNCH_TH(EPIV, F16V, THV, AMAXV, STATS, PIVOT) MODE_SPLIT_LAUNCH_PRO(EPIV, F16V, THV, AMAXV, false, STATS, PIVOT)
 #define MODE_SPLIT_LAUNCH(EPIV, F16V, STATS, PIVOT) MODE_SPLIT_LAUNCH_TH(EPIV, F16V, 8, false, STATS, PIVOT)
   if (amax_x && amax_y) {
     MODE_REQUIRE(!stats && epi.shift, MODE_ERR_BAD_ARG, "%s: the output maximum belongs to the eval epilogues", who);
@@ -485,6 +506,10 @@
   if (amax_x) {
     MODE_REQUIRE(!stats && (!epi.shift || epi.add), MODE_ERR_UNSUPPORTED, "%s: the fp16 arithmetic has no BatchNorm epilogues", who);
     if (epi.shift && epi.add) MODE_SPLIT_LAUNCH(2, true, nullptr, nullptr)
+    if (pro_scale) {
+      if (d.TH == 16) MODE_SPLIT_LAUNCH_PRO(0, true, 16, false, true, nullptr, nullptr)
+      MODE_SPLIT_LAUNCH_PRO(0, true, 8, false, true, nullptr, nullptr)
+    }
     if (d.TH == 16) MODE_SPLIT_LAUNCH_TH(0, true, 16, false, nullptr, nullptr)
     MODE_SPLIT_LAUNCH(0, true, nullptr, nullptr)
   }
@@ -494,6 +519,7 @@
   MODE_SPLIT_LAUNCH(0, false, nullptr, nullptr)
 #undef MODE_SPLIT_LAUNCH
 #undef MODE_SPLIT_LAUNCH_TH
+#undef MODE_SPLIT_LAUNCH_PRO
 }
 
 __device__ __forceinline__ unsigned finite_mag(unsigned bits) {
@@ -602,8 +628,10 @@
 
 int conv3d_s1_split(const float* x, const float* w, float* y, float* wpack, int B, int K, int rows, int D, int H, int W, int flip,
                     hipStream_t st, const char* who, const mode_bn_epilogue* bn, float* stats, const float* acc_in, const float* amax_x,
-                    const float* amax_w, float* amax_y) {
+                    const float* amax_w, float* amax_y, const float* pro_scale, const float* pro_shift) {
   const float* absmax = amax_x;
+  MODE_REQUIRE((pro_scale == nullptr) == (pro_shift == nullptr) && (!pro_scale || (amax_x && amax_w && !bn && !stats && !acc_in && flip == 0)),
+               MODE_ERR_BAD_ARG, "%s: the BatchNorm prologue takes scale and shift, on the plain fp16 forward only", who);
   const bool eval16 = absmax && bn;
   MODE_REQUIRE(eval16 ? (!amax_w && amax_y && !stats && !acc_in) : ((amax_x == nullptr) == (amax_w == nullptr) && !amax_y), MODE_ERR_BAD_ARG,
                "%s: both operand maxima, or neither (eval epilogue: the input's and the output's)", who);
@@ -661,7 +689,7 @@
     hipLaunchKernelGGL(first_voxel_kernel, dim3(rows), dim3(64), 0, st, x, w, pivot, K, rows, D, H, W);
     return launch_split<1>(x, wpack, y, d, d.MT, st, who, epi, stats, pivot);
   }
-  return launch_split<1>(x, wpack, y, d, d.MT, st, who, epi, nullptr, nullptr, amax_x, amax_w);
-}
-
-}
+  return launch_split<1>(x, wpack, y, d, d.MT, st, who, epi, nullptr, nullptr, amax_x, amax_w, nullptr, pro_scale, pro_shift);
+}
+
+}
diff --git a/mode-2022_amd/csrc/conv3d_split_wgrad.hip b/mode-2022_amd/csrc/conv3d_split_wgrad.hip
--- a/mode-2022_amd/csrc/conv3d_split_wgrad.hip
+++ b/mode-2022_amd/csrc/conv3d_split_wgrad.hip
@@ -32,10 +32,12 @@
   }
 }
 
-template <bool F16>
+template <bool F16, bool PRO = false>
 __global__ __launch_bounds__(NT) void conv3d_bww_split_kernel(const float* __restrict__ gy, const float* __restrict__ x,
                                                               float* __restrict__ part, mode::WgradSplitDims d,
-                                                              const float* __restrict__ amax_g, const float* __restrict__ amax_x) {
+                                                              const float* __restrict__ amax_g, const float* __restrict__ amax_x,
+                                                              const float* __restrict__ pro_scale, const float* __restrict__ pro_shift) {
+  static_assert(!PRO || F16, "the BatchNorm prologue exists on two fp16 pieces");
   constexpr int NP = Arith<F16>::NP;
   const float sg = F16 ? f16_scale_of(mode::absmax_load(amax_g)) : 1.f, sx = F16 ? f16_scale_of(mode::absmax_load(amax_x)) : 1.f;
   const float unscale = F16 ? (1.f / sg) * (1.f / sx) : 1.f;
@@ -86,6 +88,15 @@
   int xdst[XIT], gdst[GIT];
 #pragma unroll
   for (int k = 0; k < XIT; ++k) xdst[k] = x_c[k] * XCS + x_row[k] * XROWP + 2 * x_wp[k];
+  float xsc[XIT], xsh[XIT];
+  if (PRO) {
+#pragma unroll
+    for (int k = 0; k < XIT; ++k) {
+      const int c = min(cb * 32 + x_c[k], d.Ci - 1);
+      xsc[k] = pro_scale[c];
+      xsh[k] = pro_shift[c];
+    }
+  }
 #pragma unroll
   for (int k = 0; k < GIT; ++k) gdst[k] = g_o[k] * GCS + g_row[k] * 32 + 2 * g_wp[k];
   auto unit_begin = [&](int h0, int w0) {
@@ -118,7 +129,11 @@
   auto commit_x = [&](int k, int z) {
     uint32_t p1, p2, p3;
     float v0 = xr[k][0], v1 = xr[k][1];
-    if (F16) {
+    if (PRO) {
+      const float sz = (unsigned)z < (unsigned)d.D ? 0.5f * sx : 0.f;
+      v0 = bnrelu_scaled(v0, xsc[k], xsh[k], xo0[k] != kBufOOB ? sz : 0.f);
+      v1 = bnrelu_scaled(v1, xsc[k], xsh[k], xo1[k] != kBufOOB ? sz : 0.f);
+    } else if (F16) {
       v0 *= sx;
       v1 *= sx;
     }
@@ -306,16 +321,27 @@
 namespace mode {
 
 int conv3d_bww_split_launch(const float* gy, const float* x, float* part, const WgradSplitDims& d, hipStream_t st, const char* who,
-                            const float* amax_g, const float* amax_x) {
+                            const float* amax_g, const float* amax_x, const float* pro_scale, const float* pro_shift) {
+  MODE_REQUIRE((pro_scale == nullptr) == (pro_shift == nullptr) && (!pro_scale || amax_g), MODE_ERR_BAD_ARG,
+               "%s: the BatchNorm prologue takes scale and shift, on the fp16 arithmetic only", who);
+  if (pro_scale) {
+    int rc = allow_lds(conv3d_bww_split_kernel<true, true>, LDS_BYTES, who);
+    if (rc != MODE_OK) return rc;
+    hipLaunchKernelGGL((conv3d_bww_split_kernel<true, true>), dim3(d.S, d.MTo, d.MTc), dim3(NT), LDS_BYTES, st, gy, x, part, d, amax_g, amax_x,
+                       pro_scale, pro_shift);
+    return check_launch(who);
+  }
   if (amax_g) {
     int rc = allow_lds(conv3d_bww_split_kernel<true>, LDS_BYTES, who);
     if (rc != MODE_OK) return rc;
-    hipLaunchKernelGGL(conv3d_bww_split_kernel<true>, dim3(d.S, d.MTo, d.MTc), dim3(NT), LDS_BYTES, st, gy, x, part, d, amax_g, amax_x);
+    hipLaunchKernelGGL(conv3d_bww_split_kernel<true>, dim3(d.S, d.MTo, d.MTc), dim3(NT), LDS_BYTES, st, gy, x, part, d, amax_g, amax_x,
+                       (const float*)nullptr, (const float*)nullptr);
     return check_launch(who);
   }
   int rc = allow_lds(conv3d_bww_split_kernel<false>, LDS_BYTES, who);
   if (rc != MODE_OK) return rc;
-  hipLaunchKernelGGL(conv3d_bww_split_kernel<false>, dim3(d.S, d.MTo, d.MTc), dim3(NT), LDS_BYTES, st, gy, x, part, d, nullptr, nullptr);
+  hipLaunchKernelGGL(conv3d_bww_split_kernel<false>, dim3(d.S, d.MTo, d.MTc), dim3(NT), LDS_BYTES, st, gy, x, part, d, (const float*)nullptr,
+                     (const float*)nullptr, (const float*)nullptr, (const float*)nullptr);
   return check_launch(who);
 }
 
diff --git a/mode-2022_amd/csrc/split_arith.h b/mode-2022_amd/csrc/split_arith.h
--- a/mode-2022_amd/csrc/split_arith.h
+++ b/mode-2022_amd/csrc/split_arith.h
@@ -83,6 +83,11 @@
   return m == 0.f ? 1.f : __builtin_bit_cast(float, (268u - e) << 23);
 }
 
+__device__ __forceinline__ float bnrelu_scaled(float y, float scale, float shift, float half_s) {
+  const float v = __builtin_fmaf(y, scale, shift);
+  return (v + __builtin_fabsf(v)) * half_s;
+}
+
 __device__ __forceinline__ f32x16 mfma_bf16(uint4 a, uint4 b, f32x16 c) {
   return __builtin_amdgcn_mfma_f32_32x32x16_bf16(__builtin_bit_cast(bf16x8, a), __builtin_bit_cast(bf16x8, b), c, 0, 0, 0);
 }
diff --git a/mode-2022_amd/mode_hip/__init__.py b/mode-2022_amd/mode_hip/__init__.py
--- a/mode-2022_amd/mode_hip/__init__.py
+++ b/mode-2022_amd/mode_hip/__init__.py
@@ -110,6 +110,11 @@
     'mode_conv3d_fwd_split_f16_bn': (_c_int, [_c_ptr] * 7 + [_c_int] * 6 + [_c_ptr]),
     'mode_conv3d_bwd_data_split_f16': (_c_int, [_c_ptr] * 7 + [_c_int] * 6 + [_c_ptr]),
     'mode_conv3d_bwd_weight_split_f16': (_c_int, [_c_ptr] * 6 + [_c_int] * 7 + [_c_ptr]),
+    'mode_bn_coef_amax_workspace_bytes': (_c_size, [_c_int]),
+    'mode_bn_train_coef_amax': (_c_int, [_c_ptr] * 6 + [ctypes.c_float] * 2 + [_c_ptr] * 6 + [_c_int] * 2 + [ctypes.c_longlong, _c_int, _c_ptr]),
+    'mode_conv3d_bnrelu_prologue_supported': (_c_int, [_c_int] * 5),
+    'mode_conv3d_fwd_split_f16_bnrelu': (_c_int, [_c_ptr] * 8 + [_c_int] * 6 + [_c_ptr]),
+    'mode_conv3d_bwd_weight_split_f16_bnrelu': (_c_int, [_c_ptr] * 8 + [_c_int] * 7 + [_c_ptr]),
     'mode_conv3d_bwd_data_split_acc': (_c_int, [_c_ptr] * 5 + [_c_int] * 7 + [_c_ptr]),
     'mode_deconv3d_fwd_split_bn': (_c_int, [_c_ptr] * 5 + [_c_int] * 6 + [_c_ptr]),
     'mode_deconv3d_fwd_split_bn_amax': (_c_int, [_c_ptr] * 6 + [_c_int] * 6 + [_c_ptr]),
diff --git a/mode-2022_amd/mode_hip/functional.py b/mode-2022_amd/mode_hip/functional.py
--- a/mode-2022_amd/mode_hip/functional.py
+++ b/mode-2022_amd/mode_hip/functional.py
@@ -1981,33 +1981,9 @@
   @staticmethod
   def backward(ctx, gout):
     y, out, gamma, beta, mean, invstd, coef = ctx.saved_tensors
-    gout = gout.contiguous()
-    B, C, S = _bcs(y)
-    gy = torch.empty_like(y)
     need_gadd = ctx.has_add and ctx.relu and ctx.needs_input_grad[1]
-    gadd = torch.empty_like(y) if need_gadd else None
-    sink_g, sink_b = grad_sink(gamma), grad_sink(beta)
-    fused = sink_g is not None and sink_b is not None and ctx.needs_input_grad[2] and ctx.needs_input_grad[3]
-    ggamma = sink_g if fused else torch.empty_like(gamma)
-    gbeta = sink_b if fused else torch.empty_like(gamma)
-    if need_gadd and out is not None:
-      nbytes = 4 * y.numel() * 7
-    else:
-      nbytes = 4 * y.numel() * (2 * (2 + (1 if out is not None else 0)) + 1 + (1 if need_gadd else 0))
-    gy_amax = None
-    if CONV_ARITH == 'bf16x6' and ((CONV3D_S1_F16 and y.dim() == 5) or (SPHERE_BWD_F16 and y.dim() == 4 and C % 16 == 0)):
-      gy_amax = torch.empty(BN_ABSMAX_FLOATS, dtype=torch.float32, device=y.device)
-    with torch.cuda.device_of(y), profiling.region(_tag_bn('bn_train_bwd', y), nbytes, 0, y.device):
-      ws = _bn_ws(C * ctx.groups, y.device)
-      check(lib().mode_bn_train_bwd_amax(ptr(gout), ptr(y), ptr(out) if out is not None else None, ptr(gamma), ptr(mean), ptr(invstd),
-                                         ptr(coef[0]) if coef is not None else None, ptr(coef[1]) if coef is not None else None, int(ctx.relu),
-                                         ptr(gy), ptr(gadd) if gadd is not None else None, ptr(ggamma), ptr(gbeta),
-                                         int(fused), ptr(ws), B, C, S, ctx.groups, ptr(gy_amax) if gy_amax is not None else None,
-                                         stream_of(y)), 'mode_bn_train_bwd_amax')
-    if gy_amax is not None:
-      gy._mode_amax = (gy_amax, gy._version, gy.data_ptr())
-    if fused:
-      ggamma = gbeta = None
+    gy, gadd, ggamma, gbeta = _bn_train_bwd(gout, y, out, gamma, beta, mean, invstd, coef, ctx.relu, ctx.groups, need_gadd,
+                                            ctx.needs_input_grad[2] and ctx.needs_input_grad[3])
     if ctx.has_add and not ctx.relu:
       gadd = gout
     if gadd is not None and ctx.add_carrier is not None:
@@ -2017,6 +1993,36 @@
       elif ctx.add_carrier.leave(gadd, ctx):
         gadd = None
     return gy, gadd, ggamma, gbeta, None, None, None, None, None, None, None, None, None
+
+
+def _bn_train_bwd(gout, y, out, gamma, beta, mean, invstd, coef, relu, groups, need_gadd, affine_grads):
+  gout = gout.contiguous()
+  B, C, S = _bcs(y)
+  gy = torch.empty_like(y)
+  gadd = torch.empty_like(y) if need_gadd else None
+  sink_g, sink_b = grad_sink(gamma), grad_sink(beta)
+  fused = bool(sink_g is not None and sink_b is not None and affine_grads)
+  ggamma = sink_g if fused else torch.empty_like(gamma)
+  gbeta = sink_b if fused else torch.empty_like(gamma)
+  if need_gadd and out is not None:
+    nbytes = 4 * y.numel() * 7
+  else:
+    nbytes = 4 * y.numel() * (2 * (2 + (1 if out is not None else 0)) + 1 + (1 if need_gadd else 0))
+  gy_amax = None
+  if CONV_ARITH == 'bf16x6' and ((CONV3D_S1_F16 and y.dim() == 5) or (SPHERE_BWD_F16 and y.dim() == 4 and C % 16 == 0)):
+    gy_amax = torch.empty(BN_ABSMAX_FLOATS, dtype=torch.float32, device=y.device)
+  with torch.cuda.device_of(y), profiling.region(_tag_bn('bn_train_bwd', y), nbytes, 0, y.device):
+    ws = _bn_ws(C * groups, y.device)
+    check(lib().mode_bn_train_bwd_amax(ptr(gout), ptr(y), ptr(out) if out is not None else None, ptr(gamma), ptr(mean), ptr(invstd),
+                                       ptr(coef[0]) if coef is not None else None, ptr(coef[1]) if coef is not None else None, int(relu),
+                                       ptr(gy), ptr(gadd) if gadd is not None else None, ptr(ggamma), ptr(gbeta),
+                                       int(fused), ptr(ws), B, C, S, groups, ptr(gy_amax) if gy_amax is not None else None,
+                                       stream_of(y)), 'mode_bn_train_bwd_amax')
+  if gy_amax is not None:
+    gy._mode_amax = (gy_amax, gy._version, gy.data_ptr())
+  if fused:
+    ggamma = gbeta = None
+  return gy, gadd, ggamma, gbeta
 
 
 def bn_eval(y, add, gamma, beta, running_mean, running_var, eps, relu):
@@ -2060,6 +2066,103 @@
     out = out + add if add is not None else out
     return torch.relu(out) if relu else out
   return bn_eval(y, add, bn.weight, bn.bias, bn.running_mean, bn.running_var, bn.eps, relu)
+
+
+BN_DEFER = True
+BN_DEFER_MIN_NUMEL = 1 << 23
+
+
+class DeferredAct(object):
+  __slots__ = ('y', 'bn')
+
+  def __init__(self, y, bn):
+    self.y, self.bn = y, bn
+
+  def materialize(self):
+    return bn_act(self.bn, self.y, None, True)
+
+
+def bn_defer_supported(y, bn, groups=1):
+  return (BN_DEFER and CONV_ARITH == 'bf16x6' and CONV3D_S1_F16 and y.dim() == 5 and bn_supported(y) and torch.is_grad_enabled() and
+          bn.training and bn.momentum is not None and bn.weight is not None and bn.bias is not None and groups == 1 and
+          y.numel() >= BN_DEFER_MIN_NUMEL)
+
+
+def conv3d_bnrelu_supported(y, w):
+  Ci, Co = int(y.shape[1]), int(w.shape[0])
+  return (CONV_ARITH == 'bf16x6' and CONV3D_S1_F16 and tuple(w.shape[1:]) == (Ci, 3, 3, 3) and w.is_cuda and w.dtype == torch.float32 and
+          lib().mode_conv3d_bnrelu_prologue_supported(Ci, Co, int(y.shape[2]), int(y.shape[3]), int(y.shape[4])) == 1)
+
+
+class Conv3dBnReluFunction(torch.autograd.Function):
+
+  @staticmethod
+  def forward(ctx, y, w, gamma, beta, running_mean, running_var, momentum, eps, num_batches_tracked):
+    require_gpu(y, w, gamma, beta)
+    y, w = y.contiguous(), w.contiguous()
+    require_f32c(y, w, gamma, beta)
+    B, C, S = _bcs(y)
+    D, H, W = y.shape[2:]
+    Co = w.shape[0]
+    saved = torch.empty((4, C), dtype=torch.float32, device=y.device)
+    a_amax = torch.empty(BN_ABSMAX_FLOATS, dtype=torch.float32, device=y.device)
+    with torch.cuda.device_of(y), profiling.region(_tag_bn('bn_train_fwd', y), 4 * y.numel(), 0, y.device):
+      ws = torch.empty(lib().mode_bn_coef_amax_workspace_bytes(C) // 4, dtype=torch.float32, device=y.device)
+      check(lib().mode_bn_train_coef_amax(ptr(y), ptr(gamma), ptr(beta), ptr(running_mean) if running_mean is not None else None,
+                                          ptr(running_var) if running_var is not None else None,
+                                          ptr(num_batches_tracked) if num_batches_tracked is not None else None, float(momentum), float(eps),
+                                          ptr(saved[0]), ptr(saved[1]), ptr(saved[2]), ptr(saved[3]), ptr(a_amax), ptr(ws), B, C, S, 1,
+                                          stream_of(y)), 'mode_bn_train_coef_amax')
+    _written_by_kernel(running_mean, running_var, num_batches_tracked)
+    w_amax = _weight_abs_max(w)
+    z = torch.empty((B, Co, D, H, W), dtype=y.dtype, device=y.device)
+    with torch.cuda.device_of(y), profiling.region(_tag3('conv3d_fwd', C, Co, 1, D, H, W), 4 * (y.numel() + z.numel() + w.numel()),
+                                                   2 * z.numel() * C * 27, y.device):
+      wp = _wpack3d(C, Co, y.device)
+      check(lib().mode_conv3d_fwd_split_f16_bnrelu(ptr(y), ptr(saved[2]), ptr(saved[3]), ptr(w), ptr(a_amax), ptr(w_amax), ptr(z), ptr(wp),
+                                                   B, C, D, H, W, Co, stream_of(y)), 'mode_conv3d_fwd_split_f16_bnrelu')
+    ctx.save_for_backward(y, w, gamma, beta, saved, a_amax, w_amax)
+    return z
+
+  @staticmethod
+  def backward(ctx, gz):
+    y, w, gamma, beta, saved, a_amax, w_amax = ctx.saved_tensors
+    B, C, D, H, W = y.shape
+    Co = w.shape[0]
+    ag = known_abs_max(gz)
+    gz = gz.contiguous()
+    if ag is None:
+      ag = abs_max(gz)
+    need_ga = ctx.needs_input_grad[0] or ctx.needs_input_grad[2] or ctx.needs_input_grad[3]
+    ga = conv3d_bwd_data(gz, w, y.shape, 1, amax=(ag, w_amax)) if need_ga else None
+    gw = None
+    if ctx.needs_input_grad[1]:
+      sink = grad_sink(w)
+      gw = sink if sink is not None else torch.empty((Co, C, 3, 3, 3), dtype=gz.dtype, device=gz.device)
+      with torch.cuda.device_of(gz), profiling.region(_tag3('conv3d_bwd_weight', C, Co, 1, D, H, W), 4 * (y.numel() + gz.numel() + gw.numel()),
+                                                      2 * gz.numel() * C * 27, gz.device):
+        ws = torch.empty(max(lib().mode_conv3d_bwd_weight_workspace_bytes(B, C, D, H, W, Co, 1) // 4, 1), dtype=torch.float32, device=gz.device)
+        check(lib().mode_conv3d_bwd_weight_split_f16_bnrelu(ptr(gz), ptr(y), ptr(saved[2]), ptr(saved[3]), ptr(ag), ptr(a_amax), ptr(gw), ptr(ws),
+                                                            B, C, D, H, W, Co, int(sink is not None), stream_of(gz)),
+              'mode_conv3d_bwd_weight_split_f16_bnrelu')
+      if sink is not None:
+        gw = None
+    gy = ggamma = gbeta = None
+    if ga is not None:
+      gy, _, ggamma, gbeta = _bn_train_bwd(ga, y, None, gamma, beta, saved[0], saved[1], saved[2:4], True, 1, False,
+                                           ctx.needs_input_grad[2] and ctx.needs_input_grad[3])
+    return gy, gw, ggamma, gbeta, None, None, None, None, None
+
+
+def conv3d_bnrelu(deferred, w):
+  bn, y = deferred.bn, deferred.y
+  update = bn.training and bn.track_running_stats
+  nbt = bn.num_batches_tracked if update else None
+  if nbt is not None and not (nbt.is_cuda and nbt.dtype == torch.int64):
+    nbt.add_(1)
+    nbt = None
+  return Conv3dBnReluFunction.apply(y, w, bn.weight, bn.bias, bn.running_mean if update else None, bn.running_var if update else None,
+                                    bn.momentum, bn.eps, nbt)
 
 
 CLASSIF_FUSED = True
diff --git a/mode-2022_amd/models/mode_disparity.py b/mode-2022_amd/models/mode_disparity.py
--- a/mode-2022_amd/models/mode_disparity.py
+++ b/mode-2022_amd/models/mode_disparity.py
@@ -27,11 +27,12 @@
                                nn.BatchNorm3d(inplanes))
 
   def forward(self, x, presqu, postsqu, *, residual=None, pre_consumers=1, x_carrier=None):
-    out = stage3d.conv_bn(self.conv1[0], x, relu=True) if x_carrier is None else stage3d.conv_bn(self.conv1[0], x, relu=True, x_carrier=x_carrier)
+    out = stage3d.conv_bn(self.conv1[0], x, relu=True, defer=True) if x_carrier is None else \
+        stage3d.conv_bn(self.conv1[0], x, relu=True, x_carrier=x_carrier, defer=True)
     pre = stage3d.conv_bn(self.conv2, out, relu=True, add=postsqu)
     inner = 1 + (1 if presqu is None else 0)
     alias = HF.fan_out(pre, inner + pre_consumers) if inner + pre_consumers > 2 else (pre,) * (inner + pre_consumers)
-    out = stage3d.conv_bn(self.conv3[0], alias[0], relu=True)
+    out = stage3d.conv_bn(self.conv3[0], alias[0], relu=True, defer=True)
     out = stage3d.conv_bn(self.conv4[0], out, relu=True)
     post = stage3d.conv_bn(self.conv5, out, relu=True, add=presqu if presqu is not None else alias[1])
     out = stage3d.conv_bn(self.conv6, post, add=residual)
@@ -135,17 +136,17 @@
         cost0 = HF.cost_conv_bn_eval(ref_fea, tgt_fea, conv0.weight, self.maxdisp // 4, self.dres0[0][1], relu=True)
       else:
         y0 = HF.cost_conv(ref_fea, tgt_fea, conv0.weight, self.maxdisp // 4)
-        cost0 = stage3d.bn_act(self.dres0[0][1], y0, None, True)
+        cost0 = stage3d.bn_relu(self.dres0[0][1], y0, defer=True)
     else:
       cost = HF.cost_volume(ref_fea, tgt_fea, self.maxdisp // 4)
-      cost0 = stage3d.conv_bn(self.dres0[0], cost, relu=True)
+      cost0 = stage3d.conv_bn(self.dres0[0], cost, relu=True, defer=True)
     cost0 = stage3d.conv_bn(self.dres0[2], cost0, relu=True)
     car = HF.grad_carrier(cost0)
     if car is None:
-      t = stage3d.conv_bn(self.dres1[0], cost0, relu=True)
+      t = stage3d.conv_bn(self.dres1[0], cost0, relu=True, defer=True)
       cost0 = stage3d.conv_bn(self.dres1[2], t, add=cost0)
     else:
-      t = stage3d.conv_bn(self.dres1[0], cost0, relu=True, x_carrier=car)
+      t = stage3d.conv_bn(self.dres1[0], cost0, relu=True, x_carrier=car, defer=True)
       cost0 = stage3d.conv_bn(self.dres1[2], t, add=cost0, add_carrier=car)
 
     c0 = HF.fan_out(cost0, 4)
diff --git a/mode-2022_amd/models/stage3d.py b/mode-2022_amd/models/stage3d.py
--- a/mode-2022_amd/models/stage3d.py
+++ b/mode-2022_amd/models/stage3d.py
@@ -52,16 +52,28 @@
   return conv(x)
 
 
-def conv_bn(seq, x, relu=False, add=None, x_carrier=None, add_carrier=None):
+def conv_bn(seq, x, relu=False, add=None, x_carrier=None, add_carrier=None, defer=False):
   conv, bn = seq[0], seq[1]
-  if x.is_cuda and x.dtype == torch.float32 and HF.bn_foldable(bn):
-    y = _conv_bn_folded(conv, bn, x, add, relu)
-    if y is not None:
-      return y
-  if (x.is_cuda and bn.training and current_bn_groups() == 1 and _hip_kind(conv, x) == 'conv1' and conv.out_channels > 1 and
-      torch.is_grad_enabled() and HF.conv3d_stats_supported(x, conv.weight, bn)):
-    return HF.conv3d_bn_train(x, conv.weight, bn, add, relu)
-  y = conv3(conv, x) if x_carrier is None else conv3(conv, x, x_carrier)
+  deferred = None
+  if isinstance(x, HF.DeferredAct):
+    if (x_carrier is None and _hip_kind(conv, x.y) == 'conv1' and conv.out_channels > 1 and bn.training and torch.is_grad_enabled() and
+        HF.conv3d_bnrelu_supported(x.y, conv.weight)):
+      deferred = x
+    else:
+      x = x.materialize()
+  if deferred is None:
+    if x.is_cuda and x.dtype == torch.float32 and HF.bn_foldable(bn):
+      y = _conv_bn_folded(conv, bn, x, add, relu)
+      if y is not None:
+        return y
+    if (x.is_cuda and bn.training and current_bn_groups() == 1 and _hip_kind(conv, x) == 'conv1' and conv.out_channels > 1 and
+        torch.is_grad_enabled() and HF.conv3d_stats_supported(x, conv.weight, bn)):
+      return HF.conv3d_bn_train(x, conv.weight, bn, add, relu)
+    y = conv3(conv, x) if x_carrier is None else conv3(conv, x, x_carrier)
+  else:
+    y = HF.conv3d_bnrelu(deferred, conv.weight)
+  if defer and relu and add is None and y.is_cuda and HF.bn_defer_supported(y, bn, current_bn_groups()):
+    return HF.DeferredAct(y, bn)
   return bn_act(bn, y, add, relu) if add_carrier is None else bn_act(bn, y, add, relu, add_carrier)
 
 
@@ -113,6 +125,12 @@
   return HF.bn_act(bn, y, add, relu, groups=current_bn_groups() if bn.training else 1, add_carrier=add_carrier)
 
 
+def bn_relu(bn, y, defer=False):
+  if defer and y.is_cuda and HF.bn_defer_supported(y, bn, current_bn_groups()):
+    return HF.DeferredAct(y, bn)
+  return bn_act(bn, y, None, True)
+
+
 def bn_act_torch(bn, y, add=None, relu=False, add_carrier=None):
   groups = current_bn_groups()
   if groups > 1 and bn.training:
```

Result: no change. 38.25 pairs/s (median of 6 runs) (+0.5%).
